# benjiebob/SMALify

Hardware: AMD Instinct MI355X
Metric: fitter iterations/sec (higher is better)
Workload: dtype f32

## Files before the change

### smalify_amd/csrc/kernels_lbs_backward.inc

```

__global__ void __launch_bounds__(256)
vertex_bwd_kernel(ModelDev m, int M, const float* __restrict__ proj, const float* __restrict__ dface,
                  const float* __restrict__ dJ41 ,
                  const float* __restrict__ dverts_ext ,
                  const float* __restrict__ Am, float* __restrict__ dvert ,
                  float* __restrict__ dvp , float* __restrict__ dtr_part ) {
  __shared__ float As[420];
  __shared__ float dJs[123];
  __shared__ float red[16];
  const int Vp = m.Vp;
  PHASE_MARK(pv0);
  int n, vblock;
  xcd_block(Vp / 256, n, vblock);
  if (n >= M) return;
  const int v = vblock * 256 + threadIdx.x;
  constexpr int kPre = 8;
  const int vc = min(v, m.V - 1);
  const int vf0 = m.vf_off[vc], vf1 = (v < m.V) ? m.vf_off[vc + 1] : vf0;
  int vfi[kPre];
#pragma unroll
  for (int q = 0; q < kPre; ++q) vfi[q] = m.vf_idx[min(vf0 + q, max(vf1 - 1, vf0))];
  for (int i = threadIdx.x; i < 420; i += 256) As[i] = Am[(size_t)n * 420 + i];
  for (int i = threadIdx.x; i < 123; i += 256) dJs[i] = dJ41 ? dJ41[(size_t)n * 123 + i] : 0.f;
  __syncthreads();
  int lm = -1;
#pragma unroll
  for (int i = 0; i < 6; ++i) if (v == m.landmarks[i]) lm = i;
  const bool live = v < m.V;
  float g[3] = {0.f, 0.f, 0.f};
  if (live && dface) {
    float gxn = 0.f, gyn = 0.f;
    const float2* df = reinterpret_cast<const float2*>(dface + (size_t)n * m.F * 6);
    float2 gq[kPre];
#pragma unroll
    for (int q = 0; q < kPre; ++q) gq[q] = df[vfi[q]];
#pragma unroll
    for (int q = 0; q < kPre; ++q)
      if (vf0 + q < vf1) { gxn += gq[q].x; gyn += gq[q].y; }
    for (int i = vf0 + kPre; i < vf1; ++i) {
      const float2 g2 = df[m.vf_idx[i]];
      gxn += g2.x;
      gyn += g2.y;
    }
    const float* pv = proj + (size_t)n * 3 * Vp;
    world_to_ndc_bwd(pv[v], pv[Vp + v], pv[2 * Vp + v], gxn, gyn, g[0], g[1], g[2]);
  }
  if (live && dverts_ext) {
#pragma unroll
    for (int a = 0; a < 3; ++a) g[a] += dverts_ext[((size_t)n * 3 + a) * Vp + v];
  }
  {
    const float s0 = wave_sum(live ? g[0] : 0.f), s1 = wave_sum(live ? g[1] : 0.f), s2 = wave_sum(live ? g[2] : 0.f);
    if ((threadIdx.x & 63) == 0) { float* q = &red[(threadIdx.x >> 6) * 4]; q[0] = s0; q[1] = s1; q[2] = s2; }
    __syncthreads();
    if (threadIdx.x < 3)
      dtr_part[((size_t)vblock * M + n) * 3 + threadIdx.x] =
          ((red[threadIdx.x] + red[4 + threadIdx.x]) + red[8 + threadIdx.x]) + red[12 + threadIdx.x];
  }
  float dv[3] = {g[0], g[1], g[2]};
  if (live) {
#pragma unroll 4
    for (int e = 0; e < m.Kj; ++e) {
      const int j = m.jrv_j[e * Vp + v];
      const float c = m.jrv_val[e * Vp + v];
#pragma unroll
      for (int a = 0; a < 3; ++a) dv[a] = fmaf(c, dJs[j * 3 + a], dv[a]);
    }
    if (lm >= 0) {
#pragma unroll
      for (int a = 0; a < 3; ++a) dv[a] += dJs[(35 + lm) * 3 + a];
    }
  }
  float T[9];
#pragma unroll
  for (int e = 0; e < 9; ++e) T[e] = 0.f;
  if (live) {
#pragma unroll 4
    for (int e = 0; e < m.Kw; ++e) {
      const int j = m.w_j[e * Vp + v];
      const float wv = m.w_val[e * Vp + v];
      const float* A = &As[j * 12];
#pragma unroll
      for (int a = 0; a < 3; ++a)
#pragma unroll
        for (int b = 0; b < 3; ++b) T[a * 3 + b] = fmaf(wv, A[a * 4 + b], T[a * 3 + b]);
    }
  }
#pragma unroll
  for (int b = 0; b < 3; ++b) {
    const float o = T[b] * dv[0] + T[3 + b] * dv[1] + T[6 + b] * dv[2];
    if (v < Vp) {
      dvp[((size_t)n * 3 + b) * Vp + v] = live ? o : 0.f;
      dvert[((size_t)n * 3 + b) * Vp + v] = live ? dv[b] : 0.f;
    }
  }
  PHASE_MARK(pv1);
  PHASE_END(PH_VERTEX_BWD, pv0, pv1);
}

__device__ __forceinline__ void
dA_block(const ModelDev& m, int j, int n, const float* __restrict__ dvert, const float* __restrict__ vposed,
         float* __restrict__ dA , float (*part)[32]) {
  const int Vp = m.Vp;
  const float* dv = dvert + (size_t)n * 3 * Vp;
  const float* vp = vposed + (size_t)n * 3 * Vp;
  float acc[16];
#pragma unroll
  for (int e = 0; e < 16; ++e) acc[e] = 0.f;
#pragma unroll 2
  for (int i = m.wc_off[j] + threadIdx.x; i < m.wc_off[j + 1]; i += 256) {
    const int v = m.wc_v[i];
    const float wv = m.wc_val[i];
    const float p[4] = {vp[v], vp[Vp + v], vp[2 * Vp + v], 1.0f};
#pragma unroll
    for (int a = 0; a < 3; ++a) {
      const float d = wv * dv[a * Vp + v];
#pragma unroll
      for (int b = 0; b < 4; ++b) acc[a * 4 + b] = fmaf(d, p[b], acc[a * 4 + b]);
    }
  }
  const int lane = threadIdx.x & 63, w = threadIdx.x >> 6;
  const float tot = wave_sums<16>(acc, lane);
  if ((lane & 3) == 0) part[w][lane >> 2] = tot;
  __syncthreads();
  if (threadIdx.x < 12)
    dA[((size_t)n * 35 + j) * 12 + threadIdx.x] = ((part[0][threadIdx.x] + part[1][threadIdx.x]) + part[2][threadIdx.x]) + part[3][threadIdx.x];
}

constexpr int kAsmElem = 4, kAsmLoss = 16;

__device__ __forceinline__ void
dbeta_block(const ModelDev& m, int M, int nb, int shared, int bx, int by, int bz, int gx, int gzn,
            const float* __restrict__ dvp, float* __restrict__ dbeta_part , float (*part)[32]) {
  const int ncol = 3 * m.Vp;
  const int c = bx * 256 + threadIdx.x;
  float g = 0.f;
  if (c < ncol) {
    if (shared) {
      const int per = (M + gzn - 1) / gzn;
      const int n0 = bz * per, n1 = min(M, n0 + per);
      double gd = 0.0;
#pragma unroll 8
      for (int n = n0; n < n1; ++n) gd += (double)dvp[(size_t)n * ncol + c];
      g = (float)gd;
    } else {
      g = dvp[(size_t)by * ncol + c];
    }
  }
  const size_t pidx = (size_t)by * gzn * gx + (size_t)bz * gx + bx;
  const int lane = threadIdx.x & 63, w = threadIdx.x >> 6;
  for (int b0 = 0; b0 < nb; b0 += 32) {
    float val[32];
    const int cc = min(c, ncol - 1);
#pragma unroll
    for (int b = 0; b < 32; ++b) val[b] = m.sd[(size_t)min(b0 + b, nb - 1) * ncol + cc];
#pragma unroll
    for (int b = 0; b < 32; ++b) val[b] = (c < ncol && b0 + b < nb) ? g * val[b] : 0.f;
    const float tot = wave_sums<32>(val, lane);
    __syncthreads();
    if ((lane & 1) == 0) part[w][lane >> 1] = tot;
    __syncthreads();
    if (threadIdx.x < 32 && b0 + threadIdx.x < nb)
      dbeta_part[pidx * nb + b0 + threadIdx.x] = ((part[0][threadIdx.x] + part[1][threadIdx.x]) + part[2][threadIdx.x]) + part[3][threadIdx.x];
  }
}

constexpr int PBM_SPLITS = 24, PBM_U = 2, PBM_TILES = 4;
static_assert(PBM_SPLITS % 8 == 0, "the blocks of a column split are placed on one XCD (ids in chunks of 8 splits)");
__device__ __forceinline__ void
poseblend_bwd_mfma_block(const ModelDev& m, int M, int tchunk, int kpair, int split, const float* __restrict__ dvp,
                         float* __restrict__ dpf_part , float (*red)[8][64]) {
  const int lane = threadIdx.x & 63, w = threadIdx.x >> 6;
  const int ncol = 3 * m.Vp, nsteps = ncol / 16;
  const int per = (nsteps + PBM_SPLITS * 4 - 1) / (PBM_SPLITS * 4);
  const int s_beg = (split * 4 + w) * per, s_end = min(nsteps, s_beg + per);
  const int nft = (M + 15) / 16, t0 = tchunk * PBM_TILES, nt = min(PBM_TILES, nft - t0);
  const int k0 = kpair * 32;
  const int row = lane & 15, cq = (lane >> 4) * 4;
  const float4* pa[PBM_TILES];
#pragma unroll
  for (int t = 0; t < PBM_TILES; ++t)
    pa[t] = reinterpret_cast<const float4*>(dvp + (size_t)min((t0 + t) * 16 + row, M - 1) * ncol + cq);
  const float4* pb0 = reinterpret_cast<const float4*>(m.pd + (size_t)min(k0 + row, 305) * ncol + cq);
  const float4* pb1 = reinterpret_cast<const float4*>(m.pd + (size_t)min(k0 + 16 + row, 305) * ncol + cq);
  f32x4 acc0[PBM_TILES], acc1[PBM_TILES];
#pragma unroll
  for (int t = 0; t < PBM_TILES; ++t) { acc0[t] = f32x4{0.f, 0.f, 0.f, 0.f}; acc1[t] = acc0[t]; }
  for (int st0 = s_beg; st0 < s_end; st0 += PBM_U) {
    float4 B0[PBM_U], B1[PBM_U], A[PBM_TILES][PBM_U];
#pragma unroll
    for (int u = 0; u < PBM_U; ++u) {
      const int st = min(st0 + u, nsteps - 1);
      B0[u] = pb0[st * 4]; B1[u] = pb1[st * 4];
#pragma unroll
      for (int t = 0; t < PBM_TILES; ++t) {
        A[t][u] = make_float4(0.f, 0.f, 0.f, 0.f);
        if (t < nt && st0 + u < s_end) A[t][u] = pa[t][st * 4];
      }
    }
    __builtin_amdgcn_sched_barrier(0);
#pragma unroll
    for (int u = 0; u < PBM_U; ++u) {
#pragma unroll
      for (int t = 0; t < PBM_TILES; ++t) {
        if (t < nt) {
          acc0[t] = __builtin_amdgcn_mfma_f32_16x16x4f32(A[t][u].x, B0[u].x, acc0[t], 0, 0, 0);
          acc1[t] = __builtin_amdgcn_mfma_f32_16x16x4f32(A[t][u].x, B1[u].x, acc1[t], 0, 0, 0);
          acc0[t] = __builtin_amdgcn_mfma_f32_16x16x4f32(A[t][u].y, B0[u].y, acc0[t], 0, 0, 0);
          acc1[t] = __builtin_amdgcn_mfma_f32_16x16x4f32(A[t][u].y, B1[u].y, acc1[t], 0, 0, 0);
          acc0[t] = __builtin_amdgcn_mfma_f32_16x16x4f32(A[t][u].z, B0[u].z, acc0[t], 0, 0, 0);
          acc1[t] = __builtin_amdgcn_mfma_f32_16x16x4f32(A[t][u].z, B1[u].z, acc1[t], 0, 0, 0);
          acc0[t] = __builtin_amdgcn_mfma_f32_16x16x4f32(A[t][u].w, B0[u].w, acc0[t], 0, 0, 0);
          acc1[t] = __builtin_amdgcn_mfma_f32_16x16x4f32(A[t][u].w, B1[u].w, acc1[t], 0, 0, 0);
        }
      }
    }
    __builtin_amdgcn_sched_barrier(0);
  }
#pragma unroll
  for (int t = 0; t < PBM_TILES; ++t) {
    if (t < nt) {
#pragma unroll
      for (int r = 0; r < 4; ++r) { red[w][r][lane] = acc0[t][r]; red[w][4 + r][lane] = acc1[t][r]; }
      __syncthreads();
#pragma unroll
      for (int q = 0; q < 2; ++q) {
        const int reg = w * 2 + q, r = reg & 3, tile = reg >> 2;
        const float tot = ((red[0][reg][lane] + red[1][reg][lane]) + red[2][reg][lane]) + red[3][reg][lane];
        const int n = (t0 + t) * 16 + 4 * (lane >> 4) + r, k = k0 + tile * 16 + (lane & 15);
        if (n < M && k < 306) dpf_part[((size_t)split * M + n) * 308 + k] = tot;
      }
      __syncthreads();
    }
  }
}

__host__ __device__ inline int mid_pb_ids(int M) { return 10 * PBM_SPLITS * (((M + 15) / 16 + PBM_TILES - 1) / PBM_TILES); }
__host__ __device__ inline int mid_da_ids(int M) { return xcd_grid(35, M); }
__host__ __device__ inline int mid_grid(int M, int nPB) { return (nPB ? mid_pb_ids(M) : 0) + mid_da_ids(M); }
__global__ void __launch_bounds__(256, 4)
lbs_bwd_mid_kernel(ModelDev m, int M, int nPB, const float* __restrict__ dvert, const float* __restrict__ vposed,
                   const float* __restrict__ dvp, float* __restrict__ dA, float* __restrict__ dpf_part) {
  __shared__ float part[4][32];
  __shared__ float tile_red[4][8][64];
  int blk = blockIdx.x;
  if (nPB > 0) {
    const int ids = mid_pb_ids(M);
    if (blk < ids) {
      PHASE_MARK(pm0);
      const int tchunk = blk / (10 * PBM_SPLITS), r = blk - tchunk * (10 * PBM_SPLITS);
      const int chunk = r / 80, q = r - chunk * 80;
      poseblend_bwd_mfma_block(m, M, tchunk, q >> 3, chunk * 8 + (q & 7), dvp, dpf_part, tile_red);
      PHASE_MARK(pm1);
      PHASE_END(PH_MID_PB, pm0, pm1);
      return;
    }
    blk -= ids;
  }
  PHASE_MARK(pd0);
  int n, j;
  xcd_block_of(blk, 35, n, j);
  if (n >= M) return;
  dA_block(m, j, n, dvert, vposed, dA, part);
  PHASE_MARK(pd1); PHASE_END(PH_MID_DA, pd0, pd1);
}

__global__ void __launch_bounds__(256)
chain_bwd_kernel(ModelDev m, int M, const float* __restrict__ theta, const float* __restrict__ Rm,
                 const float* __restrict__ Gm, const float* __restrict__ scm,
                 const float* __restrict__ Jrest, int j_stride, const float* __restrict__ dA,
                 const float* __restrict__ dpf_part, int CS, const float* __restrict__ dth_direct,
                 float* __restrict__ dtheta , float* __restrict__ dls ,
                 float* __restrict__ dJrest , float* __restrict__ dbetaJ ,
                 float* __restrict__ dRs_out ,
                 int nb, int betas_shared, int nDB_x, int nDB_y, int nDB_z, const float* __restrict__ dvp,
                 float* __restrict__ dbeta_part ) {
  PHASE_MARK(pc0);
  if ((int)blockIdx.x >= M) {
    __shared__ float rpart[4][32];
    const int blk = (int)blockIdx.x - M;
    dbeta_block(m, M, nb, betas_shared, blk % nDB_x, (blk / nDB_x) % nDB_y, blk / (nDB_x * nDB_y), nDB_x, nDB_z, dvp, dbeta_part, rpart);
    PHASE_MARK(pcr);
    PHASE_END(PH_CHAIN_RIDER, pc0, pcr);
    return;
  }
  __shared__ float R[35][9], G[35][12], sc[35][3], J[35][3];
  __shared__ float dG[35][12], dR[35][9], dJ[35][3];
  __shared__ float cG[35][12], cJ[35][3], cS[35][3], sOwn[35][3];
  __shared__ float dRp[35][9], djv[35][3];
  __shared__ int sidx[105];
  __shared__ float psum[4][320];
  __shared__ float isc[35][3];
  __shared__ float sJS[105 * 48];
  __shared__ float dAs[35][12];
  __shared__ unsigned char t_lvl_off[36], t_lvl_joint[36], t_child_off[36], t_child_idx[36], t_par[36];
  __shared__ uint2 t_sch[kTreeMaxPass][8];
  const int n = blockIdx.x, l = threadIdx.x;
  const TreeLevels& tl = m.tree;
  if (l < 36) {
    t_lvl_off[l] = tl.lvl_off[l]; t_child_off[l] = tl.child_off[l];
    if (l < 35) { t_lvl_joint[l] = tl.lvl_joint[l]; t_child_idx[l] = tl.child_idx[l]; t_par[l] = (unsigned char)max(m.parents[l], 0); }
  }
  if (l >= 128 && l < 128 + kTreeMaxPass * 8) {
    const int q = l - 128;
    const unsigned char* ch = tl.pass_child[q >> 3][q & 7];
    t_sch[q >> 3][q & 7] = make_uint2((unsigned)tl.pass_joint[q >> 3][q & 7] | ((unsigned)tl.pass_parent[q >> 3][q & 7] << 8) | ((unsigned)tl.pass_nchild[q >> 3][q & 7] << 16),
                                      (unsigned)ch[0] | ((unsigned)ch[1] << 8) | ((unsigned)ch[2] << 16) | ((unsigned)ch[3] << 24));
  }
  const int lth = min(l, 34);
  const float th_pre[3] = {theta[((size_t)n * 35 + lth) * 3], theta[((size_t)n * 35 + lth) * 3 + 1], theta[((size_t)n * 35 + lth) * 3 + 2]};
  float dthd_pre[3] = {0.f, 0.f, 0.f};
  if (dth_direct) {
#pragma unroll
    for (int a = 0; a < 3; ++a) dthd_pre[a] = dth_direct[(size_t)n * 105 + lth * 3 + a];
  }
  const int nlev = tl.nlev;
  const bool js_lds = dbetaJ && m.NBall <= 48;
  const int njs = js_lds ? 105 * m.NBall : 1;
  float js_tmp[20];
  const float* js_src = js_lds ? m.JS : Rm + (size_t)n * 315;
#pragma unroll
  for (int r = 0; r < 20; ++r) js_tmp[r] = js_src[min(l + 256 * r, njs - 1)];
  {
    const int l2 = l + 256;
    const float r0v = Rm[(size_t)n * 315 + l], r1v = Rm[(size_t)n * 315 + min(l2, 314)];
    const float g0v = Gm[(size_t)n * 420 + l], g1v = Gm[(size_t)n * 420 + min(l2, 419)];
    const float a0v = dA[(size_t)n * 420 + l], a1v = dA[(size_t)n * 420 + min(l2, 419)];
    const int lc = min(l, 104);
    const float sv = scm[(size_t)n * 105 + lc], jv = Jrest[(size_t)n * j_stride + lc];
    const int siv = m.scale_idx[lc];
    constexpr int kMaxPer = (PBM_SPLITS + 3) / 4;
    const int per = (CS + 3) / 4, qd = l >> 6, c0 = qd * per, c1 = min(CS, c0 + per);
    const size_t stride = (size_t)M * 308;
    float pv[5][kMaxPer];
    const bool fast = dpf_part != nullptr && per <= kMaxPer;
    if (fast) {
#pragma unroll
      for (int r = 0; r < 5; ++r) {
        const float* src = dpf_part + (size_t)n * 308 + min((l & 63) + 64 * r, 305);
#pragma unroll
        for (int c = 0; c < kMaxPer; ++c) pv[r][c] = src[(size_t)min(c0 + c, CS - 1) * stride];
      }
    }
    if (js_lds) {
#pragma unroll
      for (int r = 0; r < 20; ++r) { const int i = l + 256 * r; if (i < njs) sJS[i] = js_tmp[r]; }
    }
    R[l / 9][l % 9] = r0v;
    if (l2 < 315) R[l2 / 9][l2 % 9] = r1v;
    G[l / 12][l % 12] = g0v; dAs[l / 12][l % 12] = a0v;
    if (l2 < 420) { G[l2 / 12][l2 % 12] = g1v; dAs[l2 / 12][l2 % 12] = a1v; }
    if (l < 105) {
      sc[l / 3][l % 3] = sv; isc[l / 3][l % 3] = 1.0f / sv;
      J[l / 3][l % 3] = jv;
      sOwn[l / 3][l % 3] = 0.f; cS[l / 3][l % 3] = 0.f; cJ[l / 3][l % 3] = 0.f;
      sidx[l] = siv;
    }
    if (dpf_part) {
#pragma unroll
      for (int r = 0; r < 5; ++r) {
        const int el = (l & 63) + 64 * r;
        if (el < 306) {
          float sacc = 0.f;
          if (fast) {
            if (c0 < c1) sacc = pv[r][0];
#pragma unroll
            for (int c = 1; c < kMaxPer; ++c)
              if (c0 + c < c1) sacc += pv[r][c];
          } else {
            const float* src = dpf_part + (size_t)n * 308 + el;
            for (int c = c0; c < c1; ++c) sacc += src[c * stride];
          }
          psum[qd][el] = sacc;
        }
      }
    }
  }
  __syncthreads();
  PHASE_MARK(pc1);
  for (int i = l; i < 315; i += 256)
    dR[i / 9][i % 9] = (i >= 9 && dpf_part) ? ((psum[0][i - 9] + psum[1][i - 9]) + psum[2][i - 9]) + psum[3][i - 9] : 0.f;
  for (int i = l; i < 420; i += 256) {
    const int j = i / 12, e = i % 12, a = e >> 2, b = e & 3;
    const float* da = dAs[j];
    dG[j][e] = (b < 3) ? da[e] - da[a * 4 + 3] * J[j][b] : da[e];
  }
  for (int i = l; i < 105; i += 256) {
    const int j = i / 3, c = i % 3;
    const float* da = dAs[j];
    dJ[j][c] = -(G[j][0 * 4 + c] * da[3] + G[j][1 * 4 + c] * da[7] + G[j][2 * 4 + c] * da[11]);
  }
  __syncthreads();
  PHASE_MARK(pc2);
  const int slot = l / 12, e = l % 12;
  if (l < 64 && tl.fast) {
    const int npass = tl.npass;
    const int slot_c = min(slot, 7);
    uint2 sch_n = t_sch[max(npass - 1, 0)][slot_c];
#pragma unroll 1
    for (int k = npass - 1; k >= 0; --k) {
      const uint2 sch = sch_n;
      sch_n = t_sch[max(k - 1, 0)][slot_c];
      const bool live = (sch.x & 255u) != 255u;
      const int i = live ? (int)(sch.x & 255u) : 0, p = live ? (int)((sch.x >> 8) & 255u) : 0, nch = live ? (int)(sch.x >> 16) : 0;
      const unsigned chil_k = sch.y;
      if (live) {
        float acc = dG[i][e];
        float cv[kTreeMaxChildren];
#pragma unroll
        for (int q = 0; q < kTreeMaxChildren; ++q) cv[q] = cG[(chil_k >> (8 * q)) & 255u][e];
#pragma unroll
        for (int q = 0; q < kTreeMaxChildren; ++q) acc += (q < nch) ? cv[q] : 0.f;
        dG[i][e] = acc;
      }
      __builtin_amdgcn_fence(__ATOMIC_ACQ_REL, "wavefront");
      __builtin_amdgcn_wave_barrier();
      if (live) {
        if (e < 9) {
          const int a = e / 3, b = e % 3;
          dRp[i][e] = G[p][0 * 4 + a] * dG[i][0 * 4 + b] + G[p][1 * 4 + a] * dG[i][1 * 4 + b] + G[p][2 * 4 + a] * dG[i][2 * 4 + b];
        } else {
          const int a = e - 9;
          djv[i][a] = G[p][0 * 4 + a] * dG[i][3] + G[p][1 * 4 + a] * dG[i][7] + G[p][2 * 4 + a] * dG[i][11];
        }
      }
      __builtin_amdgcn_fence(__ATOMIC_ACQ_REL, "wavefront");
      __builtin_amdgcn_wave_barrier();
      if (live) {
        if (e < 9) {
          const int a = e / 3, c = e % 3;
          float acc = dG[i][a * 4 + 3] * (J[i][c] - J[p][c]);
#pragma unroll
          for (int b = 0; b < 3; ++b) acc = fmaf(dG[i][a * 4 + b], R[i][c * 3 + b] * sc[i][b] * isc[p][c], acc);
          cG[i][a * 4 + c] = acc;
          dR[i][a * 3 + c] += dRp[i][a * 3 + c] * sc[i][c] * isc[p][a];
        } else {
          const int a = e - 9;
          cG[i][a * 4 + 3] = dG[i][a * 4 + 3];
          cJ[i][a] = djv[i][a];
          {
            const int b = a;
            float acc = 0.f;
#pragma unroll
            for (int r = 0; r < 3; ++r) acc = fmaf(dRp[i][r * 3 + b], R[i][r * 3 + b] * isc[p][r], acc);
            sOwn[i][b] = acc;
          }
          {
            float acc = 0.f;
#pragma unroll
            for (int b = 0; b < 3; ++b) acc = fmaf(dRp[i][a * 3 + b], R[i][a * 3 + b] * sc[i][b] * isc[p][a], acc);
            cS[i][a] = acc * isc[p][a];
          }
        }
      }
      __builtin_amdgcn_fence(__ATOMIC_ACQ_REL, "wavefront");
      __builtin_amdgcn_wave_barrier();
    }
  } else if (l < 64)
  for (int L = nlev - 1; L >= 1; --L) {
    const int j0 = t_lvl_off[L], nj = t_lvl_off[L + 1] - j0;
    for (int base = 0; base < nj; base += 5) {
      const bool live = (slot < 5) && (base + slot < nj);
      const int i = live ? t_lvl_joint[j0 + base + slot] : 0;
      const int p = live ? t_par[i] : 0;
      if (live) {
        float acc = dG[i][e];
        for (int q = t_child_off[i]; q < t_child_off[i + 1]; ++q) acc += cG[t_child_idx[q]][e];
        dG[i][e] = acc;
      }
      __builtin_amdgcn_fence(__ATOMIC_ACQ_REL, "workgroup");
      __builtin_amdgcn_wave_barrier();
      if (live) {
        if (e < 9) {
          const int a = e / 3, b = e % 3;
          dRp[i][e] = G[p][0 * 4 + a] * dG[i][0 * 4 + b] + G[p][1 * 4 + a] * dG[i][1 * 4 + b] + G[p][2 * 4 + a] * dG[i][2 * 4 + b];
        } else {
          const int a = e - 9;
          djv[i][a] = G[p][0 * 4 + a] * dG[i][3] + G[p][1 * 4 + a] * dG[i][7] + G[p][2 * 4 + a] * dG[i][11];
        }
      }
      __builtin_amdgcn_fence(__ATOMIC_ACQ_REL, "workgroup");
      __builtin_amdgcn_wave_barrier();
      if (live) {
        if (e < 9) {
          const int a = e / 3, c = e % 3;
          float acc = dG[i][a * 4 + 3] * (J[i][c] - J[p][c]);
#pragma unroll
          for (int b = 0; b < 3; ++b) acc = fmaf(dG[i][a * 4 + b], R[i][c * 3 + b] * sc[i][b] * isc[p][c], acc);
          cG[i][a * 4 + c] = acc;
          dR[i][a * 3 + c] += dRp[i][a * 3 + c] * sc[i][c] * isc[p][a];
        } else {
          const int a = e - 9;
          cG[i][a * 4 + 3] = dG[i][a * 4 + 3];
          cJ[i][a] = djv[i][a];
          {
            const int b = a;
            float acc = 0.f;
#pragma unroll
            for (int r = 0; r < 3; ++r) acc = fmaf(dRp[i][r * 3 + b], R[i][r * 3 + b] * isc[p][r], acc);
            sOwn[i][b] = acc;
          }
          {
            float acc = 0.f;
#pragma unroll
            for (int b = 0; b < 3; ++b) acc = fmaf(dRp[i][a * 3 + b], R[i][a * 3 + b] * sc[i][b] * isc[p][a], acc);
            cS[i][a] = acc * isc[p][a];
          }
        }
      }
      __builtin_amdgcn_fence(__ATOMIC_ACQ_REL, "workgroup");
      __builtin_amdgcn_wave_barrier();
    }
  }
  __syncthreads();
  PHASE_MARK(pc3);
  if (l < 12) {
    float acc = dG[0][l];
    for (int q = t_child_off[0]; q < t_child_off[1]; ++q) acc += cG[t_child_idx[q]][l];
    dG[0][l] = acc;
  }
  __syncthreads();
  if (l < 9) dR[0][l] += dG[0][(l / 3) * 4 + (l % 3)];
  for (int i = l; i < 105; i += 256) {
    const int j = i / 3, a = i % 3;
    float aj = dJ[j][a], as = 0.f;
    for (int q = t_child_off[j]; q < t_child_off[j + 1]; ++q) { aj -= cJ[t_child_idx[q]][a]; as -= cS[t_child_idx[q]][a]; }
    if (j > 0) { aj += cJ[j][a]; as += sOwn[j][a]; }
    else aj += dG[0][a * 4 + 3];
    dJ[j][a] = aj;
    sOwn[j][a] = as;
  }
  __syncthreads();
  PHASE_MARK(pc4);
  if (l < 35) {
    const float th[3] = {th_pre[0], th_pre[1], th_pre[2]};
    float g[9], d[3];
#pragma unroll
    for (int q = 0; q < 9; ++q) g[q] = dR[l][q];
    if (dRs_out) {
#pragma unroll
      for (int q = 0; q < 9; ++q) dRs_out[((size_t)n * 35 + l) * 9 + q] = g[q];
    }
    rodrigues_bwd(th, g, d);
#pragma unroll
    for (int a = 0; a < 3; ++a)
      dtheta[(size_t)n * 105 + l * 3 + a] = d[a] + (dth_direct ? dthd_pre[a] : 0.f);
  }
  if (dls) {
    const int w = l >> 6, lane = l & 63;
    for (int sidx_l = w; sidx_l < 6; sidx_l += 4) {
      float v = 0.f;
      if (sidx[lane] == sidx_l) v = sOwn[lane / 3][lane % 3] * sc[lane / 3][lane % 3];
      if (lane + 64 < 105 && sidx[lane + 64] == sidx_l) v += sOwn[(lane + 64) / 3][(lane + 64) % 3] * sc[(lane + 64) / 3][(lane + 64) % 3];
      v = wave_sum(v);
      if (lane == 0) dls[(size_t)n * 6 + sidx_l] = v;
    }
  }
  for (int i = l; i < 105; i += 256) dJrest[(size_t)n * 105 + i] = dJ[i / 3][i % 3];
  if (dbetaJ) {
    const int w = l >> 6, b = l & 63;
    if (b < m.NBall) {
      float acc = 0.f;
      if (js_lds) {
#pragma unroll 9
        for (int r = 0; r < 27; ++r) { const int i = w * 27 + r; if (i < 105) acc = fmaf(dJ[i / 3][i % 3], sJS[i * m.NBall + b], acc); }
      } else {
        for (int i = w * 27; i < min(105, w * 27 + 27); ++i) acc = fmaf(dJ[i / 3][i % 3], m.JS[i * m.NBall + b], acc);
      }
      psum[w][b] = acc;
    }
    __syncthreads();
    if (l < m.NBall) dbetaJ[(size_t)n * m.NBall + l] = ((psum[0][l] + psum[1][l]) + psum[2][l]) + psum[3][l];
  }
  PHASE_MARK(pc5);
  PHASE_ADD(PH_CHAIN, 0, pc0, pc1); PHASE_ADD(PH_CHAIN, 1, pc1, pc2); PHASE_ADD(PH_CHAIN, 2, pc2, pc3); PHASE_ADD(PH_CHAIN, 3, pc3, pc4); PHASE_ADD(PH_CHAIN, 4, pc4, pc5);
  PHASE_END(PH_CHAIN, pc0, pc5);
}

__global__ void __launch_bounds__(256)
assemble_kernel(AssembleArgs a) {
  __shared__ float red[16];
  __shared__ double bsum[12][32];
  __shared__ float part[32][8];
  __shared__ double dpart[32][8];
  __shared__ int is_last;
  const int t = threadIdx.x;
  PHASE_MARK(pa0);
  const int M = a.M;
  const int nbs = a.betas_shared ? 1 : M;
  int role = blockIdx.x;
  const int ph_role = (role < nbs) ? PH_ASM_BETA : PH_ASM_ELEM;
  if (role < nbs) {
    if (a.g_betas) {
      const int s = role;
      const int bl = t % 20, slice = t / 20;
      auto beta_pass = [&](int b0) {
        const int b = b0 + bl;
        if (slice < 12 && b < a.nb) {
          double acc = 0.0;
          const int nlo = a.betas_shared ? 0 : s, nhi = a.betas_shared ? M : s + 1;
          for (int n = nlo + slice; n < nhi; n += 12) acc += (double)a.dbetaJ[(size_t)n * a.NBall + b];
          const int nparts = a.nblk_beta * a.ngrp_beta;
#pragma unroll 8
          for (int blk = slice; blk < nparts; blk += 12) acc += (double)a.dbeta_part[((size_t)s * nparts + blk) * a.nb + b];
          bsum[slice][bl] = acc;
        }
        __syncthreads();
        if (t < 20 && b0 + t < a.nb) {
          double tot = 0.0;
          for (int sl = 0; sl < 12; ++sl) tot += bsum[sl][t];
          if (a.gb_prior && s == 0) tot += (double)a.gb_prior[b0 + t];
          a.g_betas[s * a.nb + b0 + t] = (float)tot;
        }
      };
      beta_pass(0);
      for (int b0 = 20; b0 < a.nb; b0 += 20) {
        __syncthreads();
        beta_pass(b0);
      }
    }
  } else if ((role -= nbs) == 0) {
    if (a.g_ls) {
      if (a.ls_shared) {
        const int e = t & 7, sl = t >> 3;
        double acc = 0.0;
        if (e < 6) for (int n = sl; n < M; n += 32) acc += (double)a.dls[(size_t)n * 6 + e];
        dpart[sl][e] = acc;
        __syncthreads();
        if (t < 6) {
          double tot = 0.0;
          for (int i = 0; i < 32; ++i) tot += dpart[i][t];
          if (a.gls_prior) tot += (double)a.gls_prior[t];
          a.g_ls[t] = (float)tot;
        }
      } else {
        for (int i = t; i < M * 6; i += 256) a.g_ls[i] = a.dls[i];
      }
    }
  } else if ((role -= 1) < kAsmElem) {
    const int gt = role * 256 + t, gs = kAsmElem * 256;
    for (int i = gt; i < M * 3; i += gs) {
      const int n = i / 3, e = i % 3;
      if (a.g_grot) a.g_grot[i] = a.dtheta[(size_t)n * 105 + e] * a.gmask[e];
      if (a.g_trans) {
        double acc = a.dtr_direct ? (double)a.dtr_direct[i] : 0.0;
#pragma unroll 16
        for (int vt = 0; vt < a.nvt; ++vt) acc += (double)a.dtr_part[((size_t)vt * M + n) * 3 + e];
        a.g_trans[i] = (float)acc;
      }
    }
    if (a.g_jrot) {
      const int total = M * 102;
      for (int i0 = gt; i0 < total; i0 += 8 * gs) {
        float v[8];
#pragma unroll
        for (int u = 0; u < 8; ++u) {
          const int i = min(i0 + u * gs, total - 1), n = i / 102, e = i % 102;
          v[u] = a.dtheta[(size_t)n * 105 + 3 + e] * a.rmask[e];
        }
#pragma unroll
        for (int u = 0; u < 8; ++u)
          if (i0 + u * gs < total) a.g_jrot[i0 + u * gs] = v[u];
      }
    }
  } else if (a.losses) {
    role -= kAsmElem;
    float lsil = 0.f;
    if (a.tile_loss) {
      for (int k = role * 256 + t; k < M * a.T; k += kAsmLoss * 256) {
        const int n = k / a.T;
        const int Bn = frame_window_size(n, a.win);
        lsil += a.tile_loss[k] * (a.w_sil / ((float)Bn * (float)a.S * (float)a.S));
      }
    }
    long long qs = 0;
    if (a.qloss) for (int k = role * 256 + t; k < a.nqblk; k += kAsmLoss * 256) qs += a.qloss[k];
    qs = wave_sum_i64(qs);
    __shared__ long long qred[4];
    if ((t & 63) == 0) qred[t >> 6] = qs;
    lsil = block_sum(lsil, red);
    if (t == 0) { a.lpart[role] = lsil; a.qpart[role] = (qred[0] + qred[1]) + (qred[2] + qred[3]); }
  }
  PHASE_MARK(pa1);
  PHASE_END(ph_role, pa0, pa1);
  (void)ph_role;
  if (!a.losses) return;
  __threadfence();
  __syncthreads();
  if (t == 0) is_last = (atomicAdd(a.counter, 1) == (int)gridDim.x - 1);
  __syncthreads();
  if (!is_last) return;
  __threadfence();
  static_assert(kAsmLoss == 16, "butterfly below");
  float lsil = 0.f;
  if (t < 64) {
    const volatile float* lp = a.lpart;
    lsil = (t < kAsmLoss) ? lp[t] : 0.f;
#pragma unroll
    for (int o = 8; o > 0; o >>= 1) lsil += __shfl_xor(lsil, o, 64);
    const volatile long long* qp = a.qpart;
    long long qtot = (t < kAsmLoss) ? qp[t] : 0ll;
    qtot = wave_sum_i64(qtot);
    lsil += (float)((double)qtot * (1.0 / (double)kLossFix));
  }
  {
    const int k = t & 7, sl = t >> 3;
    float acc = 0.f;
    if (a.loss_part) for (int n = sl; n < M; n += 32) acc += a.loss_part[n * 8 + k];
    part[sl][k] = acc;
  }
  __syncthreads();
  if (t < 8) {
    float acc = 0.f;
    if (t == 3) acc = a.loss_betas ? *a.loss_betas : 0.f;
    else if (t == 4) acc = lsil;
    else for (int i = 0; i < 32; ++i) acc += part[i][t];
    a.losses[t] = acc;
  }
  if (t == 8) {
    float acc = 0.f;
    for (int i = 0; i < 32; ++i) acc += part[i][3];
    a.losses[8] = acc;
  }
  if (t == 0) *a.counter = 0;
  PHASE_MARK(pa2);
  PHASE_END(PH_ASM_LAST, pa1, pa2);
}

__global__ void offset_grad_kernel(ModelDev m, int M, const float* __restrict__ dvp ,
                                   const float* __restrict__ dJrest , float* __restrict__ doff ) {
  const int v = blockIdx.x * blockDim.x + threadIdx.x, n = blockIdx.y;
  if (v >= m.V) return;
  float g[3];
#pragma unroll
  for (int c = 0; c < 3; ++c) g[c] = dvp[((size_t)n * 3 + c) * m.Vp + v];
  for (int k = 0; k < m.Kj; ++k) {
    const float w = m.jrv_val[(size_t)k * m.Vp + v];
    const int j = m.jrv_j[(size_t)k * m.Vp + v];
#pragma unroll
    for (int c = 0; c < 3; ++c) g[c] = fmaf(w, dJrest[(size_t)n * 105 + j * 3 + c], g[c]);
  }
  float* o = doff + ((size_t)n * m.V + v) * 3;
  o[0] = g[0]; o[1] = g[1]; o[2] = g[2];
}

struct AdamSegments {
  int nseg;
  int beg[4];
  int off[5];
};
__device__ __forceinline__ void adam_segments_element(const AdamSegments& sg, int j, float* p, const float* g, float* mm,
                                                      float* vv, float step_size, float b1, float b2, float eps,
                                                      float bc2_sqrt, bool fresh) {
  int sgi = 0;
#pragma unroll
  for (int k = 1; k < 4; ++k) sgi += (k < sg.nseg && j >= sg.off[k]) ? 1 : 0;
  const int i = sg.beg[sgi] + (j - sg.off[sgi]);
  const float gi = g[i];
  adam_update(gi, fresh ? 0.f : mm[i], fresh ? 0.f : vv[i], b1, b2, eps, step_size, bc2_sqrt, mm[i], vv[i], p[i]);
}
__global__ void adam_segments_kernel(AdamSegments sg, float* __restrict__ p, const float* __restrict__ g,
                                     float* __restrict__ mm, float* __restrict__ vv,
                                     float step_size, float b1, float b2, float eps, float bc2_sqrt, int fresh) {
  PHASE_MARK(pz0);
  const int j = blockIdx.x * blockDim.x + threadIdx.x;
  if (j >= sg.off[sg.nseg]) return;
  adam_segments_element(sg, j, p, g, mm, vv, step_size, b1, b2, eps, bc2_sqrt, fresh != 0);
  PHASE_MARK(pz1);
  PHASE_END(PH_ADAM, pz0, pz1);
}

__global__ void tick_kernel(int* counter) { *counter += 1; }
__global__ void set_counter_kernel(int* counter, int value) { *counter = value; }
__global__ void adam_segments_graph_kernel(AdamSegments sg, float* __restrict__ p, const float* __restrict__ g,
                                           float* __restrict__ mm, float* __restrict__ vv, const int* __restrict__ step_counter,
                                           float lr, float b1, float b2, float eps) {
  const int j = blockIdx.x * blockDim.x + threadIdx.x;
  if (j >= sg.off[sg.nseg]) return;
  const int t = *step_counter;
  float step_size, bc2_sqrt;
  adam_bias_terms(lr, b1, b2, t, step_size, bc2_sqrt);
  adam_segments_element(sg, j, p, g, mm, vv, step_size, b1, b2, eps, bc2_sqrt, t == 1);
}

__global__ void shard_record_kernel(int ns, const float* __restrict__ shared_grad, int M, const float* __restrict__ grot,
                                    const float* __restrict__ jrot, const float* __restrict__ trans,
                                    const float* __restrict__ gmask, const float* __restrict__ rmask, float* __restrict__ out) {
  const int t = blockIdx.x * blockDim.x + threadIdx.x;
  if (t < ns) { out[t] = shared_grad[t]; return; }
  const int u = t - ns;
  if (u >= 216) return;
  const int which = u / 108, c = u - which * 108;
  const int n = which ? M - 1 : 0;
  float v;
  if (c < 3) v = grot[n * 3 + c] * gmask[c];
  else if (c < 105) v = jrot[n * 102 + (c - 3)] * rmask[c - 3];
  else v = trans[n * 3 + (c - 105)];
  out[t] = v;
}

__global__ void shard_reduce_adam_kernel(int world, int stride, const float* __restrict__ gathered, int ns, int ns_train,
                                         float* __restrict__ p, float* __restrict__ g, float* __restrict__ mm, float* __restrict__ vv,
                                         float step_size, float b1, float b2, float eps, float bc2_sqrt, int fresh) {
  const int i = blockIdx.x * blockDim.x + threadIdx.x;
  if (i >= ns) return;
  float gi = 0.f;
  for (int r = 0; r < world; ++r) gi += gathered[(size_t)r * stride + i];
  g[i] = gi;
  if (i >= ns_train) return;
  adam_update(gi, fresh ? 0.f : mm[i], fresh ? 0.f : vv[i], b1, b2, eps, step_size, bc2_sqrt, mm[i], vv[i], p[i]);
}

__global__ void __launch_bounds__(128)
temporal_kernel(int M, float w_temp, const float* __restrict__ theta, const float* __restrict__ trans,
                float* __restrict__ losses , float* __restrict__ dtheta ,
                float* __restrict__ dtrans ) {
  __shared__ float red[16];
  const int t = threadIdx.x;
  float lj = 0.f, lg = 0.f, lt = 0.f;
  for (int idx = t; idx < M * 108; idx += 128) {
    const int n = idx / 108, e = idx % 108;
    const bool is_tr = e >= 105;
    const int k = is_tr ? e - 105 : e;
    const float D = is_tr ? 3.0f : (k < 3 ? 3.0f : 102.0f);
    const float cur = is_tr ? trans[n * 3 + k] : theta[n * 105 + k];
    float g = 0.f;
    if (n + 1 < M) {
      const float d = cur - (is_tr ? trans[(n + 1) * 3 + k] : theta[(n + 1) * 105 + k]);
      const float term = d * d * (w_temp / D);
      if (is_tr) lt += term; else if (k < 3) lg += term; else lj += term;
      g += d;
    }
    if (n > 0) g += cur - (is_tr ? trans[(n - 1) * 3 + k] : theta[(n - 1) * 105 + k]);
    g *= 2.0f * w_temp / D;
    if (is_tr) dtrans[n * 3 + k] = g; else dtheta[n * 105 + k] = g;
  }
  lj = block_sum(lj, red); lg = block_sum(lg, red); lt = block_sum(lt, red);
  if (t == 0) { losses[0] = lj; losses[1] = lg; losses[2] = lt; }
}

__global__ void split_theta_grad_kernel(int M, const float* __restrict__ dtheta, const float* __restrict__ gmask,
                                        const float* __restrict__ rmask, float* __restrict__ g_grot,
                                        float* __restrict__ g_jrot) {
  const int i = blockIdx.x * blockDim.x + threadIdx.x;
  if (i >= M * 105) return;
  const int n = i / 105, e = i % 105;
  if (e < 3) { if (g_grot) g_grot[n * 3 + e] = dtheta[i] * (gmask ? gmask[e] : 1.f); }
  else if (g_jrot) g_jrot[n * 102 + e - 3] = dtheta[i] * (rmask ? rmask[e - 3] : 1.f);
}

__global__ void project_points_kernel(int count, int S, const float* __restrict__ pts, float* __restrict__ out) {
  const int i = blockIdx.x * blockDim.x + threadIdx.x;
  if (i >= count) return;
  float xn, yn, zv;
  world_to_ndc(pts[i * 3], pts[i * 3 + 1], pts[i * 3 + 2], xn, yn, zv);
  const float half = 0.5f * (float)(S - 1);
  out[i * 2] = half * (1.0f - yn);
  out[i * 2 + 1] = half * (1.0f - xn);
}
__global__ void project_points_bwd_kernel(int count, int S, const float* __restrict__ pts,
                                          const float* __restrict__ dout, float* __restrict__ dpts) {
  const int i = blockIdx.x * blockDim.x + threadIdx.x;
  if (i >= count) return;
  float xn, yn, zv;
  world_to_ndc(pts[i * 3], pts[i * 3 + 1], pts[i * 3 + 2], xn, yn, zv);
  const float half = 0.5f * (float)(S - 1);
  world_to_ndc_bwd(xn, yn, zv, -half * dout[i * 2 + 1], -half * dout[i * 2], dpts[i * 3], dpts[i * 3 + 1], dpts[i * 3 + 2]);
}

__global__ void rodrigues_kernel(int count, const float* __restrict__ th, float* __restrict__ R) {
  const int i = blockIdx.x * blockDim.x + threadIdx.x;
  if (i >= count) return;
  float r[9];
  const float t[3] = {th[i * 3], th[i * 3 + 1], th[i * 3 + 2]};
  rodrigues_fwd(t, r);
#pragma unroll
  for (int e = 0; e < 9; ++e) R[i * 9 + e] = r[e];
}
__global__ void rodrigues_bwd_kernel(int count, const float* __restrict__ th, const float* __restrict__ dR,
                                     float* __restrict__ dth) {
  const int i = blockIdx.x * blockDim.x + threadIdx.x;
  if (i >= count) return;
  const float t[3] = {th[i * 3], th[i * 3 + 1], th[i * 3 + 2]};
  float g[9], d[3];
#pragma unroll
  for (int e = 0; e < 9; ++e) g[e] = dR[i * 9 + e];
  rodrigues_bwd(t, g, d);
  dth[i * 3] = d[0]; dth[i * 3 + 1] = d[1]; dth[i * 3 + 2] = d[2];
}

__global__ void __launch_bounds__(128)
pose_prior_kernel(const float* __restrict__ x, const float* __restrict__ prec, const float* __restrict__ mean,
                  const float* __restrict__ mask, float* __restrict__ out ) {
  __shared__ float xs[105];
  const int n = blockIdx.x, t = threadIdx.x;
  if (t < 105) xs[t] = x[n * 105 + t] - mean[t];
  __syncthreads();
  if (t < 105) {
    float acc = 0.f;
    for (int r = 0; r < 105; ++r) acc = fmaf(xs[r], prec[r * 105 + t], acc);
    acc *= mask[t];
    out[n * 105 + t] = acc * acc;
  }
}
__global__ void __launch_bounds__(128)
pose_prior_bwd_kernel(const float* __restrict__ x, const float* __restrict__ prec, const float* __restrict__ mean,
                      const float* __restrict__ mask, const float* __restrict__ dout, float* __restrict__ dx) {
  __shared__ float xs[105], g[105];
  const int n = blockIdx.x, t = threadIdx.x;
  if (t < 105) xs[t] = x[n * 105 + t] - mean[t];
  __syncthreads();
  if (t < 105) {
    float acc = 0.f;
    for (int r = 0; r < 105; ++r) acc = fmaf(xs[r], prec[r * 105 + t], acc);
    g[t] = 2.0f * acc * mask[t] * mask[t] * dout[n * 105 + t];
  }
  __syncthreads();
  if (t < 105) {
    float acc = 0.f;
    for (int c = 0; c < 105; ++c) acc = fmaf(g[c], prec[t * 105 + c], acc);
    dx[n * 105 + t] = acc;
  }
}
```

### smalify_amd/csrc/kernels_lbs_forward.inc

```


struct HeadArgs {
  int M, Mp, nb, betas_stride, ls_stride, nshape_x, nshape, prior_D, prior_use_ls;
  const float* betas;
  const float* theta_in;
  const float* grot;
  const float* jrot;
  const float* gmask;
  const float* rmask;
  const float* logscale;
  float* theta;
  float* Jrest;
  float* v_shaped;
  float *Rm, *Gm, *scm, *Am, *pfT;
  const float* prior_prec;
  const float* prior_mean;
  float prior_w;
  float *prior_loss, *prior_gb, *prior_gls;
  const float* Rs_in;
  const float* joff;
  int joff_stride;
  const float* voff;
};

__device__ __forceinline__ void
pose_block(const ModelDev& m, const HeadArgs& a, int n) {
  __shared__ float th[105];
  __shared__ float R[35][9];
  __shared__ float sc[35][3], isc[35][3];
  __shared__ __attribute__((aligned(16))) float G[35][12];
  __shared__ float J[35][3];
  __shared__ unsigned char t_lvl_off[36], t_lvl_joint[36], t_par[36];
  __shared__ unsigned char t_pj[kTreeMaxPass][8], t_pp[kTreeMaxPass][8];
  const int l = threadIdx.x, M = a.M;
  PHASE_MARK(ph0);
  const TreeLevels& tl = m.tree;
  if (l < 36) {
    t_lvl_off[l] = tl.lvl_off[l];
    if (l < 35) { t_lvl_joint[l] = tl.lvl_joint[l]; t_par[l] = (unsigned char)max(m.parents[l], 0); }
  }
  if (l >= 128 && l < 128 + kTreeMaxPass * 8) { const int q = l - 128; t_pj[q >> 3][q & 7] = tl.pass_joint[q >> 3][q & 7]; t_pp[q >> 3][q & 7] = tl.pass_parent[q >> 3][q & 7]; }
  const int nlev = tl.nlev;
  if (l < 105) {
    const int lj = max(l - 3, 0);
    const float* tsrc = a.theta_in ? a.theta_in + (size_t)n * 105 + l : ((l < 3) ? a.grot + n * 3 + l : a.jrot + (size_t)n * 102 + lj);
    const float* msrc = a.theta_in ? tsrc : ((l < 3) ? a.gmask + l : a.rmask + lj);
    const int idx = m.scale_idx[l];
    const float tv0 = *tsrc, mv = *msrc;
    float acc = m.Jt[l];
    const float lsv = a.logscale ? a.logscale[(size_t)n * a.ls_stride + max(idx, 0)] : 0.f;
    const float tv = a.theta_in ? tv0 : tv0 * mv;
    th[l] = tv;
    a.theta[(size_t)n * 105 + l] = tv;
    const float* beta = a.betas + (size_t)(a.betas_stride ? n : 0) * a.betas_stride;
#pragma unroll 10
    for (int b = 0; b < a.nb; ++b) acc = fmaf(m.JS[l * m.NBall + b], beta[b], acc);
    if (a.joff) acc += a.joff[(size_t)n * a.joff_stride + l];
    J[l / 3][l % 3] = acc;
    if (a.betas_stride || n == 0) a.Jrest[(size_t)(a.betas_stride ? n : 0) * 105 + l] = acc;
    const float sv = (a.logscale != nullptr && idx >= 0) ? expf(lsv) : 1.0f;
    sc[l / 3][l % 3] = sv; isc[l / 3][l % 3] = 1.0f / sv;
    a.scm[(size_t)n * 105 + l] = sv;
  }
  __syncthreads();
  PHASE_MARK(ph1);
  if (l < 35) {
    const float t3[3] = {th[l * 3], th[l * 3 + 1], th[l * 3 + 2]};
    float r[9];
    if (a.Rs_in) {
#pragma unroll
      for (int e = 0; e < 9; ++e) r[e] = a.Rs_in[((size_t)n * 35 + l) * 9 + e];
    } else {
      rodrigues_fwd(t3, r);
    }
#pragma unroll
    for (int e = 0; e < 9; ++e) { R[l][e] = r[e]; a.Rm[((size_t)n * 35 + l) * 9 + e] = r[e]; }
  }
  __syncthreads();
  PHASE_MARK(ph2);
  for (int idx = l; idx < 306; idx += 256) {
    const int j = idx / 9 + 1, e = idx % 9;
    a.pfT[(size_t)idx * a.Mp + n] = R[j][e] - ((e & 3) == 0 ? 1.0f : 0.0f);
  }
  if (l < 12) {
    const int r = l >> 2, c = l & 3;
    G[0][l] = (c < 3) ? R[0][r * 3 + c] : J[0][r];
  }
  if (l < 64 && tl.fast) {
    const int slot_c = min(l / 12, 7), e = l % 12, r = e >> 2, c = e & 3, cc = min(c, 2);
    const int npass = tl.npass;
    auto fetch = [&](int k, int& ijp, float (&kc)[3]) {
      const int i = t_pj[k][slot_c], p = t_pp[k][slot_c];
      const bool live = i != 255;
      ijp = live ? (i | (p << 8)) : -1;
      const int ii = live ? i : 0;
#pragma unroll
      for (int q = 0; q < 3; ++q) {
        const float rot = R[ii][q * 3 + cc] * sc[ii][cc] * isc[p][q], dj = J[ii][q] - J[p][q];
        kc[q] = (c < 3) ? rot : dj;
      }
    };
    int ijp_n;
    float kc_n[3];
    fetch(0, ijp_n, kc_n);
#pragma unroll 1
    for (int k = 0; k < npass; ++k) {
      const int ijp = ijp_n;
      const float k0 = kc_n[0], k1 = kc_n[1], k2 = kc_n[2];
      fetch(min(k + 1, kTreeMaxPass - 1), ijp_n, kc_n);
      __builtin_amdgcn_fence(__ATOMIC_ACQ_REL, "wavefront");
      __builtin_amdgcn_wave_barrier();
      if (ijp >= 0) {
        const int i = ijp & 255, p = ijp >> 8;
        const float4 g = *reinterpret_cast<const float4*>(&G[p][r * 4]);
        float acc = (c < 3) ? 0.f : g.w;
        acc = fmaf(g.x, k0, acc);
        acc = fmaf(g.y, k1, acc);
        acc = fmaf(g.z, k2, acc);
        G[i][e] = acc;
      }
    }
  } else if (l < 64) {
    const int slot = l / 12, e = l % 12;
    for (int L = 1; L < nlev; ++L) {
      const int j0 = t_lvl_off[L], nj = t_lvl_off[L + 1] - j0;
      for (int base = 0; base < nj; base += 5) {
        __builtin_amdgcn_fence(__ATOMIC_ACQ_REL, "workgroup");
        __builtin_amdgcn_wave_barrier();
        if (slot < 5 && base + slot < nj) {
          const int i = t_lvl_joint[j0 + base + slot], p = t_par[i];
          const int r = e >> 2, c = e & 3;
          float acc;
          if (c < 3) {
            acc = 0.f;
#pragma unroll
            for (int q = 0; q < 3; ++q) acc = fmaf(G[p][r * 4 + q], R[i][q * 3 + c] * sc[i][c] * isc[p][q], acc);
          } else {
            acc = G[p][r * 4 + 3];
#pragma unroll
            for (int q = 0; q < 3; ++q) acc = fmaf(G[p][r * 4 + q], J[i][q] - J[p][q], acc);
          }
          G[i][e] = acc;
        }
      }
    }
  }
  __syncthreads();
  PHASE_MARK(ph3);
  for (int idx = l; idx < 35 * 12; idx += 256) {
    const int j = idx / 12, e = idx % 12, r = e >> 2, c = e & 3;
    float val = G[j][e];
    if (c == 3) {
#pragma unroll
      for (int q = 0; q < 3; ++q) val = fmaf(-G[j][r * 4 + q], J[j][q], val);
    }
    a.Am[(size_t)n * 420 + idx] = val;
    a.Gm[(size_t)n * 420 + idx] = G[j][e];
  }
  (void)M;
  PHASE_MARK(ph4);
  PHASE_ADD(PH_HEAD_POSE, 0, ph0, ph1); PHASE_ADD(PH_HEAD_POSE, 1, ph1, ph2); PHASE_ADD(PH_HEAD_POSE, 2, ph2, ph3); PHASE_ADD(PH_HEAD_POSE, 3, ph3, ph4);
  PHASE_END(PH_HEAD_POSE, ph0, ph4);
}

__global__ void __launch_bounds__(256)
lbs_head_kernel(ModelDev m, HeadArgs a) {
  int blk = blockIdx.x;
  if (blk < a.M) { pose_block(m, a, blk); return; }
  blk -= a.M;
  if (blk < a.nshape) {
    PHASE_MARK(ps0);
    const int s = blk / a.nshape_x;
    const float* beta = a.betas + (size_t)s * a.betas_stride;
    const int v = (blk % a.nshape_x) * 256 + threadIdx.x;
    const int Vp = m.Vp;
    if (v < Vp) {
#pragma unroll
      for (int c = 0; c < 3; ++c) {
        float acc = m.vt[c * Vp + v];
#pragma unroll 10
        for (int b = 0; b < a.nb; ++b) acc = fmaf(beta[b], m.sd[((size_t)b * 3 + c) * Vp + v], acc);
        if (a.voff) acc += a.voff[((size_t)s * 3 + c) * Vp + v];
        a.v_shaped[((size_t)s * 3 + c) * Vp + v] = acc;
      }
    }
    PHASE_MARK(ps1);
    PHASE_END(PH_HEAD_SHAPE, ps0, ps1);
    return;
  }
  if (a.prior_prec && threadIdx.x < 64) {
    __shared__ float x[32], res[32];
    const int t = threadIdx.x, D = a.prior_D;
    if (t < D) x[t] = ((t < 20) ? a.betas[t] : a.logscale[t - 20]) - a.prior_mean[t];
    __builtin_amdgcn_fence(__ATOMIC_ACQ_REL, "workgroup");
    __builtin_amdgcn_wave_barrier();
    float lv = 0.f;
    if (t < D) {
      float acc = 0.f;
      for (int r = 0; r < D; ++r) acc = fmaf(x[r], a.prior_prec[r * D + t], acc);
      res[t] = acc;
      lv = acc * acc;
    }
    __builtin_amdgcn_fence(__ATOMIC_ACQ_REL, "workgroup");
    __builtin_amdgcn_wave_barrier();
    lv = wave_sum(lv);
    if (t == 0) *a.prior_loss = a.prior_w * lv / (float)D;
    if (t < D) {
      float acc = 0.f;
      for (int c = 0; c < D; ++c) acc = fmaf(res[c], a.prior_prec[t * D + c], acc);
      acc *= 2.0f * a.prior_w / (float)D;
      if (t < 20) a.prior_gb[t] = acc; else if (a.prior_use_ls) a.prior_gls[t - 20] = acc;
    }
  }
}

__global__ void build_theta_kernel(int M, const float* __restrict__ grot, const float* __restrict__ jrot,
                                   const float* __restrict__ gmask, const float* __restrict__ rmask,
                                   float* __restrict__ theta) {
  const int i = blockIdx.x * blockDim.x + threadIdx.x;
  if (i >= M * 105) return;
  const int n = i / 105, e = i % 105;
  theta[i] = (e < 3) ? grot[n * 3 + e] * gmask[e] : jrot[n * 102 + (e - 3)] * rmask[e - 3];
}

typedef float f32x4 __attribute__((ext_vector_type(4)));
constexpr int kSkinGroups = 2;
constexpr int kSkinVerts = 16 * kSkinGroups;
constexpr int kSkinThreads = 256 * kSkinGroups;
constexpr int kSkinStage = (16 * 105 + kSkinThreads - 1) / kSkinThreads;
__global__ void __launch_bounds__(kSkinThreads)
skin_mfma_split_kernel(ModelDev m, int M, int Mp, const float* __restrict__ v_shaped, int vs_stride ,
                 const float* __restrict__ pfT, const float* __restrict__ Am, const float* __restrict__ trans,
                 float* __restrict__ vposed, float* __restrict__ verts, float* __restrict__ proj) {
  __shared__ __attribute__((aligned(16))) float As[16][420];
  __shared__ float red[4 * kSkinGroups][12][64];
  const int Vp = m.Vp;
  PHASE_MARK(pk0);
  const int lane = threadIdx.x & 63, wid = threadIdx.x >> 6, w = wid & 3, grp = wid >> 2;
  const int n0 = blockIdx.y * 16;
  const int v = blockIdx.x * kSkinVerts + grp * 16 + (lane & 15);
  const int kq = lane >> 4;
  const int nvalid = min(16, M - n0) * 105;
  float4 a_stage[kSkinStage];
  {
    const float4* src = reinterpret_cast<const float4*>(Am + (size_t)n0 * 420);
#pragma unroll
    for (int r = 0; r < kSkinStage; ++r) a_stage[r] = src[min((int)threadIdx.x + kSkinThreads * r, nvalid - 1)];
  }
  int wj[8];
  float wv[8];
  const int Kw = min(m.Kw, 8);
#pragma unroll
  for (int e = 0; e < 8; ++e) {
    const int ee = max(min(e, Kw - 1), 0);
    wj[e] = m.w_j[ee * Vp + v];
    wv[e] = m.w_val[ee * Vp + v];
  }
  const int f = 4 * kq + w, n = n0 + f, nn = min(n, M - 1);
  float vs_r[3], tr_r[3];
  {
    const float* vs = v_shaped + (size_t)nn * vs_stride;
#pragma unroll
    for (int a = 0; a < 3; ++a) { vs_r[a] = vs[a * Vp + v]; tr_r[a] = trans[nn * 3 + a]; }
  }
  constexpr int U = 20;
  const int st0 = w * U;
  const float* pa = pfT + (size_t)kq * Mp + n0 + (lane & 15);
  const float* pb = m.pd + (size_t)kq * 3 * Vp + v;
  float xa[U], x0[U], x1[U], x2[U];
#pragma unroll
  for (int u = 0; u < U; ++u) {
    const int st = min(st0 + u, 76);
    xa[u] = pa[(size_t)st * 4 * Mp];
    const float* b = pb + (size_t)(min(st * 4 + kq, 305) - kq) * 3 * Vp;
    x0[u] = b[0]; x1[u] = b[Vp]; x2[u] = b[2 * Vp];
  }
  {
    float4* dst = reinterpret_cast<float4*>(&As[0][0]);
#pragma unroll
    for (int r = 0; r < kSkinStage; ++r) {
      const int i4 = threadIdx.x + kSkinThreads * r;
      if (i4 < 16 * 105) dst[i4] = (i4 < nvalid) ? a_stage[r] : make_float4(0.f, 0.f, 0.f, 0.f);
    }
  }
  PHASE_MARK(pk1);
  f32x4 acc0 = {0.f, 0.f, 0.f, 0.f}, acc1 = acc0, acc2 = acc0;
#pragma unroll
  for (int u = 0; u < U; ++u) {
    if (st0 + u < 77) {
      acc0 = __builtin_amdgcn_mfma_f32_16x16x4f32(xa[u], x0[u], acc0, 0, 0, 0);
      acc1 = __builtin_amdgcn_mfma_f32_16x16x4f32(xa[u], x1[u], acc1, 0, 0, 0);
      acc2 = __builtin_amdgcn_mfma_f32_16x16x4f32(xa[u], x2[u], acc2, 0, 0, 0);
    }
  }
#pragma unroll
  for (int r = 0; r < 4; ++r) { red[wid][r][lane] = acc0[r]; red[wid][4 + r][lane] = acc1[r]; red[wid][8 + r][lane] = acc2[r]; }
  __syncthreads();
  PHASE_MARK(pk2);
  if (n < M) {
    float bl[3];
#pragma unroll
    for (int a = 0; a < 3; ++a) bl[a] = ((red[grp * 4][a * 4 + w][lane] + red[grp * 4 + 1][a * 4 + w][lane]) + red[grp * 4 + 2][a * 4 + w][lane]) + red[grp * 4 + 3][a * 4 + w][lane];
    const float vp[3] = {vs_r[0] + bl[0], vs_r[1] + bl[1], vs_r[2] + bl[2]};
#pragma unroll
    for (int a = 0; a < 3; ++a) vposed[((size_t)n * 3 + a) * Vp + v] = vp[a];
    float T[12];
#pragma unroll
    for (int e = 0; e < 12; ++e) T[e] = 0.f;
#pragma unroll
    for (int e = 0; e < 8; ++e) {
      if (e < Kw) {
        const float* A = &As[f][wj[e] * 12];
#pragma unroll
        for (int c = 0; c < 12; ++c) T[c] = fmaf(wv[e], A[c], T[c]);
      }
    }
    for (int e = 8; e < m.Kw; ++e) {
      const int j = m.w_j[e * Vp + v];
      const float wx = m.w_val[e * Vp + v];
      const float* A = &As[f][j * 12];
#pragma unroll
      for (int c = 0; c < 12; ++c) T[c] = fmaf(wx, A[c], T[c]);
    }
    float o[3];
#pragma unroll
    for (int a = 0; a < 3; ++a) {
      o[a] = fmaf(T[a * 4], vp[0], fmaf(T[a * 4 + 1], vp[1], fmaf(T[a * 4 + 2], vp[2], T[a * 4 + 3])));
      verts[((size_t)n * 3 + a) * Vp + v] = o[a];
    }
    float xn, yn, zv;
    world_to_ndc(o[0] + tr_r[0], o[1] + tr_r[1], o[2] + tr_r[2], xn, yn, zv);
    proj[((size_t)n * 3 + 0) * Vp + v] = xn;
    proj[((size_t)n * 3 + 1) * Vp + v] = yn;
    proj[((size_t)n * 3 + 2) * Vp + v] = zv;
  }
  PHASE_MARK(pk3);
  PHASE_ADD(PH_SKIN, 0, pk0, pk1); PHASE_ADD(PH_SKIN, 1, pk1, pk2); PHASE_ADD(PH_SKIN, 2, pk2, pk3);
  PHASE_END(PH_SKIN, pk0, pk3);
}

__global__ void __launch_bounds__(256)
skin_mfma_kernel(ModelDev m, int M, int Mp, const float* __restrict__ v_shaped, int vs_stride ,
                 const float* __restrict__ pfT, const float* __restrict__ Am, const float* __restrict__ trans,
                 float* __restrict__ vposed, float* __restrict__ verts, float* __restrict__ proj) {
  __shared__ __attribute__((aligned(16))) float As[16][420];
  const int Vp = m.Vp;
  PHASE_MARK(pk0);
  const int lane = threadIdx.x & 63, w = threadIdx.x >> 6;
  const int n0 = blockIdx.y * 16;
  const int v = blockIdx.x * 64 + w * 16 + (lane & 15);
  const int kq = lane >> 4;
  const int nvalid = min(16, M - n0) * 105;
  float4 a_stage[7];
  {
    const float4* src = reinterpret_cast<const float4*>(Am + (size_t)n0 * 420);
#pragma unroll
    for (int r = 0; r < 7; ++r) a_stage[r] = src[min((int)threadIdx.x + 256 * r, nvalid - 1)];
  }
  int wj[8];
  float wv[8];
  const int Kw = min(m.Kw, 8);
#pragma unroll
  for (int e = 0; e < 8; ++e) {
    const int ee = max(min(e, Kw - 1), 0);
    wj[e] = m.w_j[ee * Vp + v];
    wv[e] = m.w_val[ee * Vp + v];
  }
  float vs_r[4][3], tr_r[4][3];
#pragma unroll
  for (int r = 0; r < 4; ++r) {
    const int nn = min(n0 + 4 * kq + r, M - 1);
    const float* vs = v_shaped + (size_t)nn * vs_stride;
#pragma unroll
    for (int a = 0; a < 3; ++a) { vs_r[r][a] = vs[a * Vp + v]; tr_r[r][a] = trans[nn * 3 + a]; }
  }
  {
    float4* dst = reinterpret_cast<float4*>(&As[0][0]);
#pragma unroll
    for (int r = 0; r < 7; ++r) {
      const int i4 = threadIdx.x + 256 * r;
      if (i4 < 16 * 105) dst[i4] = (i4 < nvalid) ? a_stage[r] : make_float4(0.f, 0.f, 0.f, 0.f);
    }
  }
  f32x4 acc0 = {0.f, 0.f, 0.f, 0.f}, acc1 = acc0, acc2 = acc0;
  const float* pa = pfT + (size_t)kq * Mp + n0 + (lane & 15);
  const float* pb = m.pd + (size_t)kq * 3 * Vp + v;
  constexpr int U = 11, NBATCH = 7;
  static_assert(U * NBATCH == 77, "306 pose features in steps of 4");
  float xa[U], x0[U], x1[U], x2[U], ya[U], y0[U], y1[U], y2[U];
  auto load_batch = [&](int bt, float* A, float* B0, float* B1, float* B2) {
#pragma unroll
    for (int u = 0; u < U; ++u) {
      const int st = bt * U + u;
      A[u] = pa[(size_t)st * 4 * Mp];
      const float* b = pb + (size_t)(min(st * 4 + kq, 305) - kq) * 3 * Vp;
      B0[u] = b[0]; B1[u] = b[Vp]; B2[u] = b[2 * Vp];
    }
  };
  auto mfma_batch = [&](const float* A, const float* B0, const float* B1, const float* B2) {
#pragma unroll
    for (int u = 0; u < U; ++u) {
      acc0 = __builtin_amdgcn_mfma_f32_16x16x4f32(A[u], B0[u], acc0, 0, 0, 0);
      acc1 = __builtin_amdgcn_mfma_f32_16x16x4f32(A[u], B1[u], acc1, 0, 0, 0);
      acc2 = __builtin_amdgcn_mfma_f32_16x16x4f32(A[u], B2[u], acc2, 0, 0, 0);
    }
  };
  PHASE_MARK(pk1);
  load_batch(0, xa, x0, x1, x2);
  for (int bt = 0; bt < NBATCH - 1; bt += 2) {
    load_batch(bt + 1, ya, y0, y1, y2);
    __builtin_amdgcn_sched_barrier(0);
    mfma_batch(xa, x0, x1, x2);
    __builtin_amdgcn_sched_barrier(0);
    load_batch(bt + 2, xa, x0, x1, x2);
    __builtin_amdgcn_sched_barrier(0);
    mfma_batch(ya, y0, y1, y2);
    __builtin_amdgcn_sched_barrier(0);
  }
  mfma_batch(xa, x0, x1, x2);
  __syncthreads();
  PHASE_MARK(pk2);
#pragma unroll
  for (int r = 0; r < 4; ++r) {
    const int f = 4 * kq + r, n = n0 + f;
    if (n >= M) break;
    const float vp[3] = {vs_r[r][0] + acc0[r], vs_r[r][1] + acc1[r], vs_r[r][2] + acc2[r]};
#pragma unroll
    for (int a = 0; a < 3; ++a) vposed[((size_t)n * 3 + a) * Vp + v] = vp[a];
    float T[12];
#pragma unroll
    for (int e = 0; e < 12; ++e) T[e] = 0.f;
#pragma unroll
    for (int e = 0; e < 8; ++e) {
      if (e < Kw) {
        const float* A = &As[f][wj[e] * 12];
#pragma unroll
        for (int c = 0; c < 12; ++c) T[c] = fmaf(wv[e], A[c], T[c]);
      }
    }
    for (int e = 8; e < m.Kw; ++e) {
      const int j = m.w_j[e * Vp + v];
      const float wx = m.w_val[e * Vp + v];
      const float* A = &As[f][j * 12];
#pragma unroll
      for (int c = 0; c < 12; ++c) T[c] = fmaf(wx, A[c], T[c]);
    }
    float o[3];
#pragma unroll
    for (int a = 0; a < 3; ++a) {
      o[a] = fmaf(T[a * 4], vp[0], fmaf(T[a * 4 + 1], vp[1], fmaf(T[a * 4 + 2], vp[2], T[a * 4 + 3])));
      verts[((size_t)n * 3 + a) * Vp + v] = o[a];
    }
    float xn, yn, zv;
    world_to_ndc(o[0] + tr_r[r][0], o[1] + tr_r[r][1], o[2] + tr_r[r][2], xn, yn, zv);
    proj[((size_t)n * 3 + 0) * Vp + v] = xn;
    proj[((size_t)n * 3 + 1) * Vp + v] = yn;
    proj[((size_t)n * 3 + 2) * Vp + v] = zv;
  }
  PHASE_MARK(pk3);
  PHASE_ADD(PH_SKIN, 0, pk0, pk1); PHASE_ADD(PH_SKIN, 1, pk1, pk2); PHASE_ADD(PH_SKIN, 2, pk2, pk3);
  PHASE_END(PH_SKIN, pk0, pk3);
}

template <int FR>
__global__ void __launch_bounds__(256)
skin_kernel(ModelDev m, int M, int Mp, const float* __restrict__ v_shaped, int vs_stride ,
            const float* __restrict__ pfT, const float* __restrict__ Am, const float* __restrict__ trans,
            float* __restrict__ vposed, float* __restrict__ verts, float* __restrict__ proj) {
  __shared__ float red[4][FR * 3][64];
  __shared__ float As[FR][420];
  const int Vp = m.Vp;
  const int lane = threadIdx.x & 63, w = __builtin_amdgcn_readfirstlane(threadIdx.x >> 6);
  const int v = blockIdx.x * 64 + lane;
  const int n0 = blockIdx.y * FR;
  for (int i = threadIdx.x; i < FR * 420; i += 256) {
    const int f = i / 420;
    As[f][i % 420] = (n0 + f < M) ? Am[(size_t)(n0 + f) * 420 + (i % 420)] : 0.f;
  }
  float acc[FR][3];
#pragma unroll
  for (int f = 0; f < FR; ++f) acc[f][0] = acc[f][1] = acc[f][2] = 0.f;
  const int k0 = (w * 306) / 4, k1 = ((w + 1) * 306) / 4;
  for (int k = k0; k < k1; ++k) {
    const float p0 = m.pd[((size_t)k * 3 + 0) * Vp + v];
    const float p1 = m.pd[((size_t)k * 3 + 1) * Vp + v];
    const float p2 = m.pd[((size_t)k * 3 + 2) * Vp + v];
    const float* pf = pfT + (size_t)k * Mp + n0;
#pragma unroll
    for (int f = 0; f < FR; ++f) {
      const float c = pf[f];
      acc[f][0] = fmaf(c, p0, acc[f][0]);
      acc[f][1] = fmaf(c, p1, acc[f][1]);
      acc[f][2] = fmaf(c, p2, acc[f][2]);
    }
  }
#pragma unroll
  for (int f = 0; f < FR; ++f) {
    red[w][f * 3 + 0][lane] = acc[f][0];
    red[w][f * 3 + 1][lane] = acc[f][1];
    red[w][f * 3 + 2][lane] = acc[f][2];
  }
  __syncthreads();
  for (int f = w; f < FR; f += 4) {
    const int n = n0 + f;
    if (n >= M) break;
    const float* vs = v_shaped + (size_t)n * vs_stride;
    float vp[3];
#pragma unroll
    for (int a = 0; a < 3; ++a) {
      vp[a] = vs[a * Vp + v] + ((red[0][f * 3 + a][lane] + red[1][f * 3 + a][lane]) +
                                (red[2][f * 3 + a][lane] + red[3][f * 3 + a][lane]));
      vposed[((size_t)n * 3 + a) * Vp + v] = vp[a];
    }
    float T[12];
#pragma unroll
    for (int e = 0; e < 12; ++e) T[e] = 0.f;
    for (int e = 0; e < m.Kw; ++e) {
      const int j = m.w_j[e * Vp + v];
      const float wv = m.w_val[e * Vp + v];
      const float* A = &As[f][j * 12];
#pragma unroll
      for (int c = 0; c < 12; ++c) T[c] = fmaf(wv, A[c], T[c]);
    }
    float o[3];
#pragma unroll
    for (int a = 0; a < 3; ++a) {
      o[a] = fmaf(T[a * 4], vp[0], fmaf(T[a * 4 + 1], vp[1], fmaf(T[a * 4 + 2], vp[2], T[a * 4 + 3])));
      verts[((size_t)n * 3 + a) * Vp + v] = o[a];
    }
    float xn, yn, zv;
    world_to_ndc(o[0] + trans[n * 3], o[1] + trans[n * 3 + 1], o[2] + trans[n * 3 + 2], xn, yn, zv);
    proj[((size_t)n * 3 + 0) * Vp + v] = xn;
    proj[((size_t)n * 3 + 1) * Vp + v] = yn;
    proj[((size_t)n * 3 + 2) * Vp + v] = zv;
  }
}

__global__ void project_verts_kernel(int M, int V, int Vp, const float* __restrict__ vin,
                                     float* __restrict__ proj) {
  const int v = blockIdx.x * blockDim.x + threadIdx.x, n = blockIdx.y;
  if (v >= Vp) return;
  float xn = 0.f, yn = 0.f, zv = 1.f;
  if (v < V) {
    const float* p = vin + ((size_t)n * V + v) * 3;
    world_to_ndc(p[0], p[1], p[2], xn, yn, zv);
  }
  proj[((size_t)n * 3 + 0) * Vp + v] = xn;
  proj[((size_t)n * 3 + 1) * Vp + v] = yn;
  proj[((size_t)n * 3 + 2) * Vp + v] = zv;
}

__global__ void planar_to_interleaved_kernel(int M, int V, int Vp, const float* __restrict__ src, int src_stride,
                                             const float* __restrict__ offs, float* __restrict__ dst) {
  const int i = blockIdx.x * blockDim.x + threadIdx.x, n = blockIdx.y;
  if (i >= V * 3) return;
  const int v = i / 3, a = i % 3;
  float val = src[(size_t)n * src_stride + a * Vp + v];
  if (offs) val += offs[n * 3 + a];
  dst[(size_t)n * V * 3 + i] = val;
}

__global__ void interleaved_to_planar_kernel(int M, int V, int Vp, const float* __restrict__ src,
                                             float* __restrict__ dst) {
  const int v = blockIdx.x * blockDim.x + threadIdx.x, n = blockIdx.y;
  if (v >= Vp) return;
#pragma unroll
  for (int a = 0; a < 3; ++a)
    dst[((size_t)n * 3 + a) * Vp + v] = (v < V) ? src[((size_t)n * V + v) * 3 + a] : 0.f;
}

struct Parents35 {
  int p[kJoints];
};

__global__ void global_rigid_kernel(int count, const float* __restrict__ Rs, const float* __restrict__ Js, Parents35 parents,
                                    const float* __restrict__ logscale ,
                                    float* __restrict__ newJ, float* __restrict__ A) {
  const int n = blockIdx.x * blockDim.x + threadIdx.x;
  if (n >= count) return;
  global_rigid_frame(Rs + (size_t)n * 315, Js + (size_t)n * 105, parents.p, logscale ? logscale + (size_t)n * 6 : nullptr,
                     newJ + (size_t)n * 105, A + (size_t)n * 560);
}

__global__ void global_rigid_bwd_kernel(int count, const float* __restrict__ Rs, const float* __restrict__ Js, Parents35 parents,
                                        const float* __restrict__ logscale, const float* __restrict__ dnewJ,
                                        const float* __restrict__ dA, float* __restrict__ scratch, float* __restrict__ dRs,
                                        float* __restrict__ dJs, float* __restrict__ dlogscale) {
  const int n = blockIdx.x * blockDim.x + threadIdx.x;
  if (n >= count) return;
  global_rigid_frame_bwd(Rs + (size_t)n * 315, Js + (size_t)n * 105, parents.p, logscale ? logscale + (size_t)n * 6 : nullptr,
                         dnewJ + (size_t)n * 105, dA + (size_t)n * 560, scratch + (size_t)n * 840, scratch + (size_t)n * 840 + 420,
                         dRs + (size_t)n * 315, dJs + (size_t)n * 105, dlogscale ? dlogscale + (size_t)n * 6 : nullptr);
}

__device__ __forceinline__ void joints_block(const ModelDev& m, const float* __restrict__ verts, float* __restrict__ joints ,
                                             int j, int n, float* red ) {
  const int Vp = m.Vp;
  const float* vx = verts + (size_t)n * 3 * Vp;
  if (j >= 35) {
    if (threadIdx.x < 3) joints[((size_t)n * 41 + j) * 3 + threadIdx.x] = vx[threadIdx.x * Vp + m.landmarks[j - 35]];
    return;
  }
  float a0 = 0.f, a1 = 0.f, a2 = 0.f;
  if (threadIdx.x < 128) {
#pragma unroll 4
    for (int i = m.jr_off[j] + threadIdx.x; i < m.jr_off[j + 1]; i += 128) {
      const int v = m.jr_v[i];
      const float c = m.jr_val[i];
      a0 = fmaf(c, vx[v], a0);
      a1 = fmaf(c, vx[Vp + v], a1);
      a2 = fmaf(c, vx[2 * Vp + v], a2);
    }
  }
  a0 = block_sum(a0, red);
  a1 = block_sum(a1, red);
  a2 = block_sum(a2, red);
  if (threadIdx.x == 0) {
    float* o = joints + ((size_t)n * 41 + j) * 3;
    o[0] = a0; o[1] = a1; o[2] = a2;
  }
}

__global__ void __launch_bounds__(128)
joints_kernel(ModelDev m, const float* __restrict__ verts, float* __restrict__ joints ) {
  __shared__ float red[16];
  joints_block(m, verts, joints, blockIdx.x, blockIdx.y, red);
}

__device__ __forceinline__ void loss_block(const LossArgs& a, int n) {
  __shared__ float th[105], x[105], res[105], dth[105];
  __shared__ float dJ[41 * 3];
  __shared__ float red[16];
  const int t = threadIdx.x;
  const int Bn = frame_window_size(n, a.win);
  for (int i = t; i < 105; i += 128) { th[i] = a.theta[n * 105 + i]; dth[i] = 0.f; }
  for (int i = t; i < 123; i += 128) dJ[i] = 0.f;
  __syncthreads();
  const float tx = a.trans[n * 3], ty = a.trans[n * 3 + 1], tz = a.trans[n * 3 + 2];
  float l_joint = 0.f, l_pose = 0.f, l_splay = 0.f, l_tj = 0.f, l_tg = 0.f, l_tt = 0.f, l_limit = 0.f;
  if (t < 25) {
    const int cj = a.canon[t];
    const float* jp = a.joints + ((size_t)n * 41 + cj) * 3;
    float xn, yn, zv;
    world_to_ndc(jp[0] + tx, jp[1] + ty, jp[2] + tz, xn, yn, zv);
    const float half = 0.5f * (float)(a.S - 1);
    const float row = half * (1.0f - yn), col = half * (1.0f - xn);
    if (a.proj_out) { a.proj_out[(n * 25 + t) * 2] = row; a.proj_out[(n * 25 + t) * 2 + 1] = col; }
    if (a.w_j2d > 0.f && a.vis[n * 25 + t] != 0.f) {
      const float dr = row - a.tj[(n * 25 + t) * 2], dc = col - a.tj[(n * 25 + t) * 2 + 1];
      l_joint = dr * dr + dc * dc;
      const float k = 2.0f * a.w_j2d / (50.0f * (float)Bn);
      float gx, gy, gz;
      world_to_ndc_bwd(xn, yn, zv, -half * k * dc, -half * k * dr, gx, gy, gz);
      atomicAdd(&dJ[cj * 3 + 0], gx);
      atomicAdd(&dJ[cj * 3 + 1], gy);
      atomicAdd(&dJ[cj * 3 + 2], gz);
    }
  }
  if (a.w_pose > 0.f) {
    if (t < 105) x[t] = th[t] - a.pose_mean[t];
    __syncthreads();
    if (t < 105) {
      float acc = 0.f;
#pragma unroll 15
      for (int r = 0; r < 105; ++r) acc = fmaf(x[r], a.pose_prec[r * 105 + t], acc);
      acc *= a.pose_mask[t];
      res[t] = acc * a.pose_mask[t];
      l_pose = acc * acc;
    }
    __syncthreads();
    if (t < 105) {
      float acc = 0.f;
#pragma unroll 15
      for (int c = 0; c < 105; ++c) acc = fmaf(res[c], a.pose_prec[t * 105 + c], acc);
      dth[t] += acc * (2.0f * a.w_pose / (105.0f * (float)Bn));
    }
  }
  if (a.w_limit > 0.f && t >= 3 && t < 105) {
    const float x = th[t], hi = a.lim_max[t - 3], lo = a.lim_min[t - 3];
    l_limit = fmaxf(x - hi, 0.f) + fmaxf(lo - x, 0.f);
    const float slope = (x > hi) ? 1.0f : ((x < lo) ? -1.0f : 0.0f);
    dth[t] += slope * (a.w_limit / (102.0f * (float)Bn));
  }
  if (a.w_splay > 0.f && t >= 3 && t < 105 && ((t % 3) != 1)) {
    l_splay = th[t] * th[t];
    dth[t] += 2.0f * a.w_splay * th[t];
  }
  float dtr = 0.f;
  if (a.w_temp > 0.f && t < 108) {
    const bool is_tr = t >= 105;
    const int e = is_tr ? t - 105 : t;
    const float D = is_tr ? 3.0f : (e < 3 ? 3.0f : 102.0f);
    const float cur = is_tr ? a.trans[n * 3 + e] : th[e];
    float g = 0.f;
    bool has_next = (n + 1 < a.M) || (a.halo_next != nullptr);
    if (has_next) {
      const float nxt = (n + 1 < a.M) ? (is_tr ? a.trans[(n + 1) * 3 + e] : a.theta[(n + 1) * 105 + e])
                                      : a.halo_next[is_tr ? 105 + e : e];
      const float d = cur - nxt;
      const float term = d * d * (a.w_temp / D);
      if (is_tr) l_tt = term; else if (e < 3) l_tg = term; else l_tj = term;
      g += d;
    }
    bool has_prev = (n > 0) || (a.halo_prev != nullptr);
    if (has_prev) {
      const float prv = (n > 0) ? (is_tr ? a.trans[(n - 1) * 3 + e] : a.theta[(n - 1) * 105 + e])
                                : a.halo_prev[is_tr ? 105 + e : e];
      g += cur - prv;
    }
    g *= 2.0f * a.w_temp / D;
    if (is_tr) dtr = g; else dth[e] += g;
  }
  __syncthreads();
  for (int i = t; i < 105; i += 128) a.dth_direct[n * 105 + i] = dth[i];
  for (int i = t; i < 123; i += 128) a.dJ41[n * 123 + i] = dJ[i];
  if (t >= 105 && t < 108) {
    float s = dtr;
    const int e = t - 105;
    for (int j = 0; j < 41; ++j) s += dJ[j * 3 + e];
    a.dtr_direct[n * 3 + e] = s;
  }
  const float nj = 1.0f / (50.0f * (float)Bn), np_ = 1.0f / (105.0f * (float)Bn);
  l_joint = block_sum(l_joint, red);
  l_pose = block_sum(l_pose, red);
  l_splay = block_sum(l_splay, red);
  l_tj = block_sum(l_tj, red);
  l_tg = block_sum(l_tg, red);
  l_tt = block_sum(l_tt, red);
  l_limit = block_sum(l_limit, red);
  if (t == 0) {
    float* o = a.loss_part + n * 8;
    o[0] = a.w_j2d * nj * l_joint;
    o[1] = a.w_pose * np_ * l_pose;
    o[2] = a.w_splay * l_splay;
    o[3] = a.w_limit * l_limit / (102.0f * (float)Bn);
    o[4] = 0.f;
    o[5] = l_tj; o[6] = l_tg; o[7] = l_tt;
  }
}

__global__ void __launch_bounds__(128)
loss_kernel(LossArgs a) { loss_block(a, blockIdx.x); }
```

### smalify_amd/csrc/smalfit_internal.h

```cpp
#pragma once
#include <hip/hip_runtime.h>

#include "smalfit_math.h"

#define SMALFIT_STATUS_BIN_OVERFLOW 1

namespace smalfit {

constexpr int kTreeMaxPass = 16, kTreeMaxChildren = 4;
struct TreeLevels {
  unsigned char nlev;
  unsigned char lvl_off[36];
  unsigned char lvl_joint[35];
  unsigned char child_off[36];
  unsigned char child_idx[35];
  unsigned char fast, npass;
  unsigned char pass_joint[kTreeMaxPass][8];
  unsigned char pass_parent[kTreeMaxPass][8];
  unsigned char pass_nchild[kTreeMaxPass][8];
  unsigned char pass_child[kTreeMaxPass][8][kTreeMaxChildren];
};

struct ModelDev {
  int V, Vp, F, NBall;
  const float* vt;
  const float* sd;
  const float* pd;
  int Kw;
  const int* w_j;
  const float* w_val;
  const int* wc_off;
  const int* wc_v;
  const float* wc_val;
  const int* jr_off;
  const int* jr_v;
  const float* jr_val;
  int Kj;
  const int* jrv_j;
  const float* jrv_val;
  const float* Jt;
  const float* JS;
  const int* parents;
  const int* faces;
  const int* vf_off;
  const int* vf_idx;
  const int* scale_idx;
  int landmarks[6];
  TreeLevels tree;
};

struct WinMap {
  int window;
  int offset;
  int total;
};

struct LossArgs {
  int M, S;
  WinMap win;
  const float* theta;
  const float* trans;
  const float* joints;
  const int* canon;
  const float* tj;
  const float* vis;
  float w_j2d, w_pose, w_splay, w_temp;
  float w_limit;
  const float* lim_min;
  const float* lim_max;
  const float* pose_prec;
  const float* pose_mean;
  const float* pose_mask;
  const float* halo_prev;
  const float* halo_next;
  float* proj_out;
  float* dth_direct;
  float* dJ41;
  float* dtr_direct;
  float* loss_part;
};

struct AssembleArgs {
  int M, S, T, nb, NBall, nblk_beta, nvt;
  WinMap win;
  int betas_shared, ls_shared;
  float w_sil;
  const float* dbeta_part;
  const float* dJrest;
  const float* dbetaJ;
  int ngrp_beta;
  const float* JS;
  const float* gb_prior;
  const float* gls_prior;
  const float* dls;
  const float* dtheta;
  const float* gmask;
  const float* rmask;
  const float* dtr_direct;
  const float* dtr_part;
  const float* loss_part;
  const float* loss_betas;
  const float* tile_loss;
  const long long* qloss;
  int nqblk;
  float* lpart;
  long long* qpart;
  int* counter;
  float* g_betas;
  float* g_ls;
  float* g_grot;
  float* g_jrot;
  float* g_trans;
  float* losses;
};

}
```

### smalify_amd/csrc/smalfit_launch.inc

```
#include <algorithm>
#include <cstdio>
#include <cstring>
#include <string>
#include <vector>

#include "../../include/smalfit.h"

namespace smalfit {

static thread_local std::string g_err;
static constexpr int kBetaGroups = 8;
static constexpr int kSelectBlocks = 1792;
static_assert(kSelectBlocks % (8 * kSelGroups) == 0, "every ticket group of every XCD needs the same number of selection workgroups (a group without one would leave its pixels undone)");
#ifdef SMALFIT_DEV_PROBES
static int g_dbg = 0;
#else
static constexpr int g_dbg = 0;
#endif

static int fail(const std::string& msg) {
  g_err = msg;
  return 1;
}

#define HIP_OK(expr)                                                                         \
  do {                                                                                       \
    hipError_t _e = (expr);                                                                  \
    if (_e != hipSuccess)                                                                    \
      return fail(std::string(#expr) + ": " + hipGetErrorString(_e));                        \
  } while (0)

#define LAUNCH_OK(what)                                                                      \
  do {                                                                                       \
    hipError_t _e = hipGetLastError();                                                       \
    if (_e != hipSuccess) return fail(std::string("launch ") + what + ": " + hipGetErrorString(_e)); \
  } while (0)

static inline size_t align_up(size_t x, size_t a) { return (x + a - 1) / a * a; }

struct Blob {
  std::vector<unsigned char> bytes;
  size_t add(const void* src, size_t n) {
    const size_t off = align_up(bytes.size(), 256);
    bytes.resize(off + n);
    if (src) std::memcpy(bytes.data() + off, src, n);
    return off;
  }
};

static const int kDefaultLandmarks[6] = {1863, 26, 2124, 150, 3055, 1097};
static const int kCanonical[25] = {10, 9, 8, 20, 19, 18, 14, 13, 12, 24, 23, 22, 25,
                                   31, 33, 34, 35, 36, 38, 37, 39, 40, 15, 15, 28};

}

using namespace smalfit;

struct smalfit_model {
  ModelDev dev;
  void* blob = nullptr;
  int V = 0, Vp = 0, F = 0, NBall = 0;
};

struct smalfit_engine {
  smalfit_model* model = nullptr;
  int maxM = 0, Mp = 0, S = 0, Tx = 0, T = 0, cap = 0, CS = PBM_SPLITS, nvt = 0, nblk_beta = 0;
  void* slab = nullptr;
  float *theta, *v_shaped, *Jrest, *Rm, *Gm, *scm, *Am, *pfT, *vposed, *verts, *proj, *joints;
  int2* fbox;
  int* status;
  float4* frec;
  int4* brect;
  unsigned long long* gacc;
  unsigned* bcnt;
  float2* zband;
  float2* blist;
  unsigned char* plist;
  unsigned char* pcount;
  unsigned long long* zbuf = nullptr;
  float* vnorm = nullptr;
  int *qcount, *frect, *queue, *bqueue;
  long long* qloss;
  int nrb = 0;
  float2* gz;
  float* zc;
  float* lpart;
  long long* qpart;
  int* asm_counter;
  float *silbuf, *tile_loss, *dface;
  float *dJ41, *dvert, *dvp, *dext, *dA, *dpf_part, *dbeta_part, *dtheta, *dls, *dJrest;
  float* dbetaJ;
  float *dth_direct, *dtr_direct, *dtr_part, *loss_part, *loss_betas, *gb_prior, *gls_prior;
  float *ones, *zeros;
  int* canon;
  float *pose_prec = nullptr, *pose_mean = nullptr, *pose_mask = nullptr;
  float *lim_min = nullptr, *lim_max = nullptr;
  bool has_joint_limits = false;
  float *shape_prec = nullptr, *shape_mean = nullptr;
  int shape_dim = 0;
  bool has_pose_prior = false;
  bool unclamped_edge_t = false;
  bool use_graph = false;
  hipGraphExec_t graph_exec = nullptr;
  std::vector<unsigned char> graph_key;
  unsigned config_epoch = 0;
  int* step_counter = nullptr;
  bool prof_on = false;
  int prof_iter = 0, prof_cap = 0, prof_stride = 1, prof_tick = 0;
  std::vector<hipEvent_t> prof_ev;
};

namespace smalfit {
struct Section {
  smalfit_engine* e; hipStream_t st; int id; bool on;
  Section(smalfit_engine* e_, hipStream_t st_, int id_) : e(e_), st(st_), id(id_) {
    on = e->prof_on && e->prof_iter < e->prof_cap && (e->prof_tick % e->prof_stride) == 0;
    if (on) (void)hipEventRecord(e->prof_ev[((size_t)e->prof_iter * SMALFIT_NUM_SECTIONS + id) * 2], st);
  }
  ~Section() {
    if (on) (void)hipEventRecord(e->prof_ev[((size_t)e->prof_iter * SMALFIT_NUM_SECTIONS + id) * 2 + 1], st);
  }
};
}

namespace smalfit {
static void launch_raster_bwd(smalfit_engine* e, hipStream_t st, int M) {
  const ModelDev& m = e->model->dev;
  const unsigned grid = (unsigned)xcd_grid((m.F + kBwdFaces - 1) / kBwdFaces, M), block = kBwdLanes * kBwdFaces;
  if (e->unclamped_edge_t)
    raster_bwd_kernel<true><<<grid, block, 0, st>>>(m.F, M, e->S, e->frec, e->fbox, e->zc, e->gz, e->plist, e->pcount, e->dface);
  else
    raster_bwd_kernel<false><<<grid, block, 0, st>>>(m.F, M, e->S, e->frec, e->fbox, e->zc, e->gz, e->plist, e->pcount, e->dface);
}
}

extern "C" {

int smalfit_version(void) { return SMALFIT_ABI_VERSION; }
#ifdef SMALFIT_DEV_PROBES
void smalfit_debug_set(int flags) { g_dbg = flags; }
int smalfit_debug_stats(smalfit_engine* e, int* out8) {
  (void)hipDeviceSynchronize();
  (void)hipMemcpy(out8, e->status, 8 * sizeof(int), hipMemcpyDeviceToHost);
  (void)hipMemset(e->status, 0, 8 * sizeof(int));
  return 0;
}
#endif
#ifdef SMALFIT_WORK_STATS
int smalfit_debug_work_stats(unsigned long long* out32) {
  (void)hipDeviceSynchronize();
  (void)hipMemcpyFromSymbol(out32, HIP_SYMBOL(smalfit::g_work), 32 * sizeof(unsigned long long));
  static const unsigned long long z[32] = {0};
  (void)hipMemcpyToSymbol(HIP_SYMBOL(smalfit::g_work), z, sizeof(z));
  return 0;
}
#endif
#ifdef SMALFIT_PHASES
int smalfit_debug_phase_stats(unsigned long long* out192) {
  (void)hipDeviceSynchronize();
  (void)hipMemcpyFromSymbol(out192, HIP_SYMBOL(smalfit::g_phase), 12 * 16 * sizeof(unsigned long long));
  static const unsigned long long z[12 * 16] = {0};
  (void)hipMemcpyToSymbol(HIP_SYMBOL(smalfit::g_phase), z, sizeof(z));
  return 0;
}
#endif
const char* smalfit_last_error(void) { return g_err.c_str(); }

int smalfit_model_create(const smalfit_model_desc* d, smalfit_model** out) {
  if (!d || !out) return fail("smalfit_model_create: null argument");
  const int V = d->num_verts, F = d->num_faces, NB = d->num_betas;
  if (V <= 0 || F <= 0 || NB <= 0) return fail("smalfit_model_create: bad dimensions");
  for (int i = 1; i < 35; ++i)
    if (!(d->parents[i] >= 0 && d->parents[i] < i)) return fail("smalfit_model_create: parents must satisfy 0 <= parents[i] < i");
  for (int i = 0; i < F * 3; ++i)
    if (d->faces[i] < 0 || d->faces[i] >= V) return fail("smalfit_model_create: face index out of range");
  const int* lms = kDefaultLandmarks;
  for (int i = 0; i < 6; ++i)
    if (lms[i] >= V) return fail("smalfit_model_create: model has fewer vertices than the SMAL landmark ids");
  const int Vp = (int)align_up((size_t)V, 256);
  Blob b;
  std::vector<float> vt((size_t)3 * Vp, 0.f), sd((size_t)NB * 3 * Vp, 0.f), pd((size_t)306 * 3 * Vp, 0.f);
  for (int v = 0; v < V; ++v)
    for (int a = 0; a < 3; ++a) vt[(size_t)a * Vp + v] = d->v_template[v * 3 + a];
  for (int k = 0; k < NB; ++k)
    for (int v = 0; v < V; ++v)
      for (int a = 0; a < 3; ++a) sd[((size_t)k * 3 + a) * Vp + v] = d->shapedirs[(size_t)k * 3 * V + 3 * v + a];
  for (int k = 0; k < 306; ++k)
    for (int v = 0; v < V; ++v)
      for (int a = 0; a < 3; ++a) pd[((size_t)k * 3 + a) * Vp + v] = d->posedirs[(size_t)k * 3 * V + 3 * v + a];
  auto build = [&](const float* dense, int& K, std::vector<int>& ell_j, std::vector<float>& ell_v,
                   std::vector<int>& off, std::vector<int>& cv, std::vector<float>& cval) {
    K = 1;
    for (int v = 0; v < V; ++v) {
      int c = 0;
      for (int j = 0; j < 35; ++j) c += dense[v * 35 + j] != 0.f;
      K = std::max(K, c);
    }
    ell_j.assign((size_t)K * Vp, 0);
    ell_v.assign((size_t)K * Vp, 0.f);
    for (int v = 0; v < V; ++v) {
      int c = 0;
      for (int j = 0; j < 35; ++j)
        if (dense[v * 35 + j] != 0.f) { ell_j[(size_t)c * Vp + v] = j; ell_v[(size_t)c * Vp + v] = dense[v * 35 + j]; ++c; }
    }
    off.assign(36, 0);
    cv.clear(); cval.clear();
    for (int j = 0; j < 35; ++j) {
      for (int v = 0; v < V; ++v)
        if (dense[v * 35 + j] != 0.f) { cv.push_back(v); cval.push_back(dense[v * 35 + j]); }
      off[j + 1] = (int)cv.size();
    }
    if (cv.empty()) { cv.push_back(0); cval.push_back(0.f); }
  };
  int Kw, Kj;
  std::vector<int> w_j, wc_off, wc_v, jrv_j, jr_off, jr_v;
  std::vector<float> w_val, wc_val, jrv_val, jr_val;
  build(d->weights, Kw, w_j, w_val, wc_off, wc_v, wc_val);
  build(d->J_regressor, Kj, jrv_j, jrv_val, jr_off, jr_v, jr_val);
  std::vector<double> Jt64(105, 0.0), JS64((size_t)105 * NB, 0.0);
  for (int j = 0; j < 35; ++j)
    for (int i = jr_off[j]; i < jr_off[j + 1]; ++i) {
      const int v = jr_v[i];
      const double c = jr_val[i];
      for (int a = 0; a < 3; ++a) {
        Jt64[j * 3 + a] += c * d->v_template[v * 3 + a];
        for (int k = 0; k < NB; ++k) JS64[(size_t)(j * 3 + a) * NB + k] += c * d->shapedirs[(size_t)k * 3 * V + 3 * v + a];
      }
    }
  std::vector<float> Jt(105), JS((size_t)105 * NB);
  for (int i = 0; i < 105; ++i) Jt[i] = (float)Jt64[i];
  for (size_t i = 0; i < JS.size(); ++i) JS[i] = (float)JS64[i];
  std::vector<int> faces_int((size_t)F * 3);
  {
    float lo[3] = {1e30f, 1e30f, 1e30f}, hi[3] = {-1e30f, -1e30f, -1e30f};
    std::vector<float> cen((size_t)F * 3);
    for (int f = 0; f < F; ++f)
      for (int a = 0; a < 3; ++a) {
        const float c = (d->v_template[d->faces[f * 3] * 3 + a] + d->v_template[d->faces[f * 3 + 1] * 3 + a] +
                         d->v_template[d->faces[f * 3 + 2] * 3 + a]) / 3.0f;
        cen[(size_t)f * 3 + a] = c;
        lo[a] = std::min(lo[a], c); hi[a] = std::max(hi[a], c);
      }
    std::vector<std::pair<unsigned long long, int>> keyed(F);
    for (int f = 0; f < F; ++f) {
      unsigned long long code = 0;
      for (int a = 0; a < 3; ++a) {
        const float span = hi[a] - lo[a];
        const unsigned q = span > 0.f ? (unsigned)std::min(1023.0f, (cen[(size_t)f * 3 + a] - lo[a]) / span * 1023.0f) : 0u;
        for (int bit = 0; bit < 10; ++bit) code |= (unsigned long long)((q >> bit) & 1u) << (3 * bit + a);
      }
      keyed[f] = {code, f};
    }
    std::stable_sort(keyed.begin(), keyed.end());
    for (int f = 0; f < F; ++f)
      for (int k = 0; k < 3; ++k) faces_int[(size_t)f * 3 + k] = d->faces[keyed[f].second * 3 + k];
  }
  std::vector<int> vf_off(V + 1, 0), vf_idx((size_t)F * 3 + 1, 0);
  for (int i = 0; i < F * 3; ++i) vf_off[faces_int[i] + 1]++;
  for (int v = 0; v < V; ++v) vf_off[v + 1] += vf_off[v];
  {
    std::vector<int> cur(vf_off.begin(), vf_off.end() - 1);
    for (int i = 0; i < F * 3; ++i) vf_idx[cur[faces_int[i]]++] = i;
  }
  std::vector<int> sidx(105, -1);
  auto set = [&](int j, int a, int c) { sidx[j * 3 + a] = c; };
  for (int j = 7; j < 25; ++j) {
    if (j == 15 || j == 16) continue;
    set(j, 2, 0); set(j, 0, 1); set(j, 1, 1);
  }
  for (int j = 25; j < 32; ++j) { set(j, 0, 2); set(j, 1, 3); set(j, 2, 3); }
  for (int j = 33; j < 35; ++j) { set(j, 1, 4); set(j, 2, 5); }

  const size_t o_vt = b.add(vt.data(), vt.size() * 4), o_sd = b.add(sd.data(), sd.size() * 4);
  const size_t o_pd = b.add(pd.data(), pd.size() * 4);
  const size_t o_wj = b.add(w_j.data(), w_j.size() * 4), o_wv = b.add(w_val.data(), w_val.size() * 4);
  const size_t o_wco = b.add(wc_off.data(), 36 * 4), o_wcv = b.add(wc_v.data(), wc_v.size() * 4);
  const size_t o_wcl = b.add(wc_val.data(), wc_val.size() * 4);
  const size_t o_jro = b.add(jr_off.data(), 36 * 4), o_jrv = b.add(jr_v.data(), jr_v.size() * 4);
  const size_t o_jrl = b.add(jr_val.data(), jr_val.size() * 4);
  const size_t o_jvj = b.add(jrv_j.data(), jrv_j.size() * 4), o_jvv = b.add(jrv_val.data(), jrv_val.size() * 4);
  const size_t o_jt = b.add(Jt.data(), 105 * 4), o_js = b.add(JS.data(), JS.size() * 4);
  const size_t o_par = b.add(d->parents, 35 * 4), o_f = b.add(faces_int.data(), (size_t)F * 3 * 4);
  const size_t o_vfo = b.add(vf_off.data(), vf_off.size() * 4), o_vfi = b.add(vf_idx.data(), vf_idx.size() * 4);
  const size_t o_si = b.add(sidx.data(), 105 * 4);

  smalfit_model* m = new smalfit_model();
  if (hipMalloc(&m->blob, b.bytes.size()) != hipSuccess) { delete m; return fail("smalfit_model_create: hipMalloc failed (no HIP device?)"); }
  if (hipMemcpy(m->blob, b.bytes.data(), b.bytes.size(), hipMemcpyHostToDevice) != hipSuccess) {
    (void)hipFree(m->blob); delete m; return fail("smalfit_model_create: hipMemcpy failed");
  }
  unsigned char* base = (unsigned char*)m->blob;
  ModelDev& g = m->dev;
  g.V = V; g.Vp = Vp; g.F = F; g.NBall = NB;
  g.vt = (const float*)(base + o_vt); g.sd = (const float*)(base + o_sd); g.pd = (const float*)(base + o_pd);
  g.Kw = Kw; g.w_j = (const int*)(base + o_wj); g.w_val = (const float*)(base + o_wv);
  g.wc_off = (const int*)(base + o_wco); g.wc_v = (const int*)(base + o_wcv); g.wc_val = (const float*)(base + o_wcl);
  g.jr_off = (const int*)(base + o_jro); g.jr_v = (const int*)(base + o_jrv); g.jr_val = (const float*)(base + o_jrl);
  g.Kj = Kj; g.jrv_j = (const int*)(base + o_jvj); g.jrv_val = (const float*)(base + o_jvv);
  g.Jt = (const float*)(base + o_jt); g.JS = (const float*)(base + o_js);
  g.parents = (const int*)(base + o_par); g.faces = (const int*)(base + o_f);
  g.vf_off = (const int*)(base + o_vfo); g.vf_idx = (const int*)(base + o_vfi);
  g.scale_idx = (const int*)(base + o_si);
  for (int i = 0; i < 6; ++i) g.landmarks[i] = lms[i];
  {
    TreeLevels& tl = g.tree;
    int depth[35] = {0}, maxd = 0;
    for (int i = 1; i < 35; ++i) { depth[i] = depth[d->parents[i]] + 1; maxd = std::max(maxd, depth[i]); }
    tl.nlev = (unsigned char)(maxd + 1);
    int pos = 0;
    for (int L = 0; L <= maxd; ++L) {
      tl.lvl_off[L] = (unsigned char)pos;
      for (int i = 0; i < 35; ++i) if (depth[i] == L) tl.lvl_joint[pos++] = (unsigned char)i;
    }
    for (int L = maxd + 1; L < 36; ++L) tl.lvl_off[L] = (unsigned char)pos;
    pos = 0;
    for (int j = 0; j < 35; ++j) {
      tl.child_off[j] = (unsigned char)pos;
      for (int c = 34; c >= 1; --c) if (d->parents[c] == j) tl.child_idx[pos++] = (unsigned char)c;
    }
    tl.child_off[35] = (unsigned char)pos;
    memset(tl.pass_joint, 255, sizeof(tl.pass_joint));
    memset(tl.pass_parent, 0, sizeof(tl.pass_parent));
    memset(tl.pass_nchild, 0, sizeof(tl.pass_nchild));
    memset(tl.pass_child, 0, sizeof(tl.pass_child));
    int np = 0;
    bool fits = true;
    for (int L = 1; L <= maxd; ++L) {
      const int j0 = tl.lvl_off[L], nj = tl.lvl_off[L + 1] - j0;
      for (int base = 0; base < nj; base += 5, ++np) {
        if (np >= kTreeMaxPass) { fits = false; continue; }
        for (int s = 0; s < 5 && base + s < nj; ++s) {
          const int i = tl.lvl_joint[j0 + base + s];
          tl.pass_joint[np][s] = (unsigned char)i;
          tl.pass_parent[np][s] = (unsigned char)d->parents[i];
          const int nc = tl.child_off[i + 1] - tl.child_off[i];
          if (nc > kTreeMaxChildren) fits = false;
          tl.pass_nchild[np][s] = (unsigned char)std::min(nc, kTreeMaxChildren);
          for (int q = 0; q < std::min(nc, kTreeMaxChildren); ++q) tl.pass_child[np][s][q] = tl.child_idx[tl.child_off[i] + q];
        }
      }
    }
    if (tl.child_off[1] - tl.child_off[0] > 35) fits = false;
    tl.npass = (unsigned char)std::min(np, kTreeMaxPass);
    tl.fast = fits ? 1 : 0;
  }
  m->V = V; m->Vp = Vp; m->F = F; m->NBall = NB;
  *out = m;
  return 0;
}

void smalfit_model_destroy(smalfit_model* m) {
  if (!m) return;
  if (m->blob) (void)hipFree(m->blob);
  delete m;
}

int smalfit_engine_create(smalfit_model* model, int max_frames, int image_size, smalfit_engine** out) {
  if (!model || !out || max_frames <= 0 || image_size <= 0) return fail("smalfit_engine_create: bad argument");
  if (image_size > 1024) return fail("smalfit_engine_create: image_size above 1024 is not supported (float32 pixel walk, see kernels_raster.inc)");
  smalfit_engine* e = new smalfit_engine();
  e->model = model;
  e->maxM = max_frames;
  e->Mp = (int)align_up((size_t)max_frames, 16);
  e->S = image_size;
  e->Tx = (image_size + 15) / 16;
  e->T = e->Tx * e->Tx;
  e->nrb = ((image_size + kResEdge - 1) / kResEdge) * ((image_size + kResEdge - 1) / kResEdge);
  e->nvt = model->Vp / 256;
  e->nblk_beta = (3 * model->Vp + 255) / 256;
  const size_t M = max_frames, Vp = model->Vp, F = model->F, S = image_size, T = e->T;
  size_t off = 0;
  auto carve = [&](size_t bytes) { size_t o = off; off = align_up(off + bytes, 256); return o; };
  struct Item { void** ptr; size_t off; };
  std::vector<Item> items;
#define CARVE(field, count, type) items.push_back({(void**)&e->field, carve((size_t)(count) * sizeof(type))})
  CARVE(theta, M * 105, float);
  CARVE(v_shaped, M * 3 * Vp, float);
  CARVE(Jrest, M * 105, float);
  CARVE(Rm, M * 315, float);
  CARVE(Gm, M * 420, float);
  CARVE(scm, M * 105, float);
  CARVE(Am, M * 420, float);
  CARVE(pfT, (size_t)308 * e->Mp, float);
  CARVE(vposed, M * 3 * Vp, float);
  CARVE(verts, M * 3 * Vp, float);
  CARVE(proj, M * 3 * Vp, float);
  CARVE(joints, M * 123, float);
  CARVE(fbox, M * F, int2);
  CARVE(frec, M * F * kRecVecs, float4);
  CARVE(brect, M * ((F + kRectFaces - 1) / kRectFaces), int4);
  CARVE(plist, M * F * kListCap, unsigned char);
  CARVE(pcount, M * F, unsigned char);
  CARVE(gacc, M * S * S, unsigned long long);
  CARVE(bcnt, M * S * S, unsigned);
  CARVE(zband, M * S * S, float2);
  CARVE(qcount, kQCountInts, int);
  CARVE(frect, M * 4, int);
  CARVE(queue, M * S * S, int);
  CARVE(bqueue, M * S * S, int);
  CARVE(qloss, kSelectBlocks + kBandBlocks, long long);
  CARVE(status, 8, int);
  CARVE(gz, M * S * S, float2);
  CARVE(silbuf, M * S * S, float);
  CARVE(tile_loss, M * (size_t)e->nrb, float);
  CARVE(dface, M * F * 6, float);
  CARVE(dJ41, M * 123, float);
  CARVE(dvert, M * 3 * Vp, float);
  CARVE(dvp, M * 3 * Vp, float);
  CARVE(dext, M * 3 * Vp, float);
  CARVE(dA, M * 420, float);
  CARVE(dpf_part, (size_t)e->CS * M * 308, float);
  CARVE(dbeta_part, (M + kBetaGroups) * (size_t)e->nblk_beta * model->NBall, float);
  CARVE(dtheta, M * 105, float);
  CARVE(dls, M * 6, float);
  CARVE(dJrest, M * 105, float);
  CARVE(dbetaJ, M * (size_t)model->NBall, float);
  CARVE(dth_direct, M * 105, float);
  CARVE(dtr_direct, M * 3, float);
  CARVE(dtr_part, (size_t)e->nvt * M * 3, float);
  CARVE(loss_part, M * 8, float);
  CARVE(loss_betas, 4, float);
  CARVE(lpart, 64, float);
  CARVE(qpart, 64, long long);
  CARVE(zc, M, float);
  CARVE(asm_counter, 4, int);
  CARVE(step_counter, 4, int);
  CARVE(gb_prior, 64, float);
  CARVE(gls_prior, 16, float);
  CARVE(ones, 128, float);
  CARVE(zeros, M * 128, float);
  CARVE(canon, 32, int);
  CARVE(pose_prec, 105 * 105, float);
  CARVE(pose_mean, 105, float);
  CARVE(pose_mask, 105, float);
  CARVE(lim_min, 102, float);
  CARVE(lim_max, 102, float);
  CARVE(shape_prec, 41 * 41, float);
  CARVE(shape_mean, 41, float);
#undef CARVE
  if (hipMalloc(&e->slab, off) != hipSuccess) { delete e; return fail("smalfit_engine_create: hipMalloc of workspace failed"); }
  for (auto& it : items) *it.ptr = (unsigned char*)e->slab + it.off;
  if (hipMemset(e->slab, 0, off) != hipSuccess) { (void)hipFree(e->slab); delete e; return fail("smalfit_engine_create: hipMemset failed"); }
  if (hipMemsetD32((hipDeviceptr_t)e->zband, 0x7f800000, (size_t)M * S * S * 2) != hipSuccess ||
      hipMalloc(&e->blist, (size_t)M * S * S * kBandCap * sizeof(float2)) != hipSuccess) {
    (void)hipFree(e->slab); delete e; return fail("smalfit_engine_create: allocation of the band lists failed");
  }
  std::vector<float> ones(128, 1.0f);
  (void)hipMemcpy(e->ones, ones.data(), 128 * 4, hipMemcpyHostToDevice);
  (void)hipMemcpy(e->canon, kCanonical, 25 * 4, hipMemcpyHostToDevice);
  *out = e;
  return 0;
}

void smalfit_engine_destroy(smalfit_engine* e) {
  if (!e) return;
  for (auto ev : e->prof_ev) (void)hipEventDestroy(ev);
  if (e->graph_exec) (void)hipGraphExecDestroy(e->graph_exec);
  if (e->slab) (void)hipFree(e->slab);
  if (e->blist) (void)hipFree(e->blist);
  if (e->zbuf) (void)hipFree(e->zbuf);
  if (e->vnorm) (void)hipFree(e->vnorm);
  delete e;
}

int smalfit_engine_status(smalfit_engine* e, void* stream, int* bits) {
  if (!e || !bits) return fail("smalfit_engine_status: null argument");
  hipStream_t st = (hipStream_t)stream;
  HIP_OK(hipStreamSynchronize(st));
  HIP_OK(hipMemcpy(bits, e->status, sizeof(int), hipMemcpyDeviceToHost));
  HIP_OK(hipMemset(e->status, 0, sizeof(int)));
  return 0;
}

int smalfit_engine_reset_raster_cache(smalfit_engine* e, void* stream) {
  if (!e) return fail("smalfit_engine_reset_raster_cache: null argument");
  HIP_OK(hipMemsetD32Async((hipDeviceptr_t)e->zband, 0x7f800000, (size_t)e->maxM * e->S * e->S * 2, (hipStream_t)stream));
  return 0;
}

int smalfit_engine_set_pose_prior(smalfit_engine* e, const float* prec, const float* mean, const float* mask) {
  if (!e || !prec || !mean || !mask) return fail("smalfit_engine_set_pose_prior: null argument");
  HIP_OK(hipMemcpy(e->pose_prec, prec, 105 * 105 * 4, hipMemcpyHostToDevice));
  HIP_OK(hipMemcpy(e->pose_mean, mean, 105 * 4, hipMemcpyHostToDevice));
  HIP_OK(hipMemcpy(e->pose_mask, mask, 105 * 4, hipMemcpyHostToDevice));
  e->has_pose_prior = true;
  e->config_epoch++;
  return 0;
}

int smalfit_engine_set_joint_limits(smalfit_engine* e, const float* min_values, const float* max_values) {
  if (!e || !min_values || !max_values) return fail("smalfit_engine_set_joint_limits: null argument");
  for (int i = 0; i < 102; ++i)
    if (!(min_values[i] <= max_values[i])) return fail("smalfit_engine_set_joint_limits: min must not exceed max");
  HIP_OK(hipMemcpy(e->lim_min, min_values, 102 * 4, hipMemcpyHostToDevice));
  HIP_OK(hipMemcpy(e->lim_max, max_values, 102 * 4, hipMemcpyHostToDevice));
  e->has_joint_limits = true;
  e->config_epoch++;
  return 0;
}

int smalfit_engine_clear_joint_limits(smalfit_engine* e) {
  if (!e) return fail("smalfit_engine_clear_joint_limits: null argument");
  e->has_joint_limits = false;
  e->config_epoch++;
  return 0;
}

int smalfit_engine_set_option(smalfit_engine* e, int option, int value) {
  if (!e) return fail("smalfit_engine_set_option: null argument");
  switch (option) {
    case SMALFIT_OPT_UNCLAMPED_EDGE_T:
      if (value != 0 && value != 1) return fail("smalfit_engine_set_option: SMALFIT_OPT_UNCLAMPED_EDGE_T takes 0 or 1");
      e->unclamped_edge_t = value != 0;
      break;
    default:
      return fail("smalfit_engine_set_option: unknown option");
  }
  e->config_epoch++;
  return 0;
}

int smalfit_engine_set_shape_prior(smalfit_engine* e, const float* prec, const float* mean, int dim) {
  if (!e || !prec || !mean || dim <= 0 || dim > 26) return fail("smalfit_engine_set_shape_prior: bad argument (dim must be 1..26)");
  HIP_OK(hipMemcpy(e->shape_prec, prec, (size_t)dim * dim * 4, hipMemcpyHostToDevice));
  HIP_OK(hipMemcpy(e->shape_mean, mean, (size_t)dim * 4, hipMemcpyHostToDevice));
  e->shape_dim = dim;
  e->config_epoch++;
  return 0;
}

}

namespace smalfit {

struct HeadExtras {
  const float *grot = nullptr, *jrot = nullptr, *gmask = nullptr, *rmask = nullptr;
  const float *prior_prec = nullptr, *prior_mean = nullptr;
  int prior_D = 0, prior_use_ls = 0;
  float prior_w = 0.f;
  const float *Rs_in = nullptr, *joff = nullptr, *voff = nullptr;
  int joff_stride = 0;
};

static int run_lbs_forward(smalfit_engine* e, hipStream_t st, int M, const float* betas, int betas_stride,
                           int nb, const float* logscale, int ls_stride, const float* trans,
                           float* joints_out, const HeadExtras* ex = nullptr) {
  const ModelDev& m = e->model->dev;
  const int nbs = betas_stride ? M : 1;
  HeadArgs h;
  std::memset(&h, 0, sizeof(h));
  h.M = M; h.Mp = e->Mp; h.nb = nb; h.betas_stride = betas_stride; h.ls_stride = ls_stride;
  h.nshape_x = m.Vp / 256; h.nshape = h.nshape_x * nbs;
  h.betas = betas; h.logscale = logscale;
  h.theta_in = (ex && ex->grot) ? nullptr : e->theta;
  if (ex) { h.grot = ex->grot; h.jrot = ex->jrot; h.gmask = ex->gmask; h.rmask = ex->rmask;
            h.Rs_in = ex->Rs_in; h.joff = ex->joff; h.joff_stride = ex->joff_stride; h.voff = ex->voff; }
  h.theta = e->theta; h.Jrest = e->Jrest; h.v_shaped = e->v_shaped;
  h.Rm = e->Rm; h.Gm = e->Gm; h.scm = e->scm; h.Am = e->Am; h.pfT = e->pfT;
  const bool prior = ex && ex->prior_prec;
  if (prior) {
    h.prior_prec = ex->prior_prec; h.prior_mean = ex->prior_mean; h.prior_D = ex->prior_D; h.prior_use_ls = ex->prior_use_ls;
    h.prior_w = ex->prior_w; h.prior_loss = e->loss_betas; h.prior_gb = e->gb_prior; h.prior_gls = e->gls_prior;
  }
  lbs_head_kernel<<<M + h.nshape + (prior ? 1 : 0), 256, 0, st>>>(m, h);
  LAUNCH_OK("lbs_head_kernel");
  const int vs_stride = betas_stride ? 3 * m.Vp : 0;
  if (M > 4 && (m.Vp / 64) * ((M + 15) / 16) >= 256)
    skin_mfma_kernel<<<dim3(m.Vp / 64, (M + 15) / 16), 256, 0, st>>>(m, M, e->Mp, e->v_shaped, vs_stride, e->pfT, e->Am, trans,
                                                                    e->vposed, e->verts, e->proj);
  else if (M > 4)
    skin_mfma_split_kernel<<<dim3(m.Vp / kSkinVerts, (M + 15) / 16), kSkinThreads, 0, st>>>(m, M, e->Mp, e->v_shaped, vs_stride, e->pfT, e->Am, trans,
                                                                    e->vposed, e->verts, e->proj);
  else
    skin_kernel<8><<<dim3(m.Vp / 64, (M + 7) / 8), 256, 0, st>>>(m, M, e->Mp, e->v_shaped, vs_stride, e->pfT, e->Am,
                                                                 trans, e->vposed, e->verts, e->proj);
  LAUNCH_OK("skin_kernel");
  if (joints_out) {
    joints_kernel<<<dim3(41, M), 128, 0, st>>>(m, e->verts, joints_out);
    LAUNCH_OK("joints_kernel");
  }
  return 0;
}

static int run_raster_forward(smalfit_engine* e, hipStream_t st, int M, WinMap win, float w_sil,
                              SilTarget tsil, float* sil_out, float2* gz_unused, float* blk_loss,
                              float* joints_out = nullptr, const LossArgs* la = nullptr) {
  (void)gz_unused;
  float2* gz = e->gz;
  const ModelDev& m = e->model->dev;
  {
    Section sec(e, st, SMALFIT_SEC_RASTER_BBOX);
    face_bbox_kernel<<<((M + 7) / 8) * 8 + xcd_grid((m.F + 255) / 256, M) + (joints_out ? 41 * M : 0), 256, 0, st>>>(m, M, e->S, e->proj, e->fbox, e->frec, e->brect, e->zc, e->frect,
                                                                                                 e->qcount, e->verts, joints_out);
    LAUNCH_OK("face_bbox_kernel");
  }
  {
    Section sec(e, st, SMALFIT_SEC_RASTER_SWEEP);
    raster_sweep_kernel<<<xcd_grid((m.F + kSweepFaces - 1) / kSweepFaces, M), 256, 0, st>>>(m.F, M, e->S, e->frec, e->fbox, e->brect, e->zc, e->zband, e->gacc, e->bcnt, e->blist, e->plist, e->pcount);
    LAUNCH_OK("raster_sweep_kernel");
  }
  {
    Section sec(e, st, SMALFIT_SEC_RASTER_RESOLVE);
    LossArgs no_loss;
    std::memset(&no_loss, 0, sizeof(no_loss));
    raster_resolve_kernel<<<xcd_grid(e->nrb, M) + (la ? ((M + 7) / 8) * 8 : 0), 256, 0, st>>>(e->S, M, win, w_sil, e->gacc, e->bcnt, e->frect, e->zband, tsil, sil_out, gz,
                                                                         blk_loss, e->qcount, e->queue, e->bqueue, g_dbg ? e->status : nullptr,
                                                                         la ? *la : no_loss, la ? M : 0);
    LAUNCH_OK("raster_resolve_kernel");
    raster_band_kernel<<<kBandBlocks, 256, 0, st>>>(e->S, M, win, w_sil, e->gacc, e->bcnt, e->blist, tsil, sil_out, gz, e->zband,
                                                    e->qcount, e->queue, e->bqueue, tsil ? e->qloss + kSelectBlocks : nullptr);
    LAUNCH_OK("raster_band_kernel");
  }
  Section sec(e, st, SMALFIT_SEC_RASTER_SELECT);
  raster_select_kernel<<<kSelectBlocks, 64 * kSelWaves, 0, st>>>(m.F, e->S, M, win, w_sil, e->frec, e->zc, e->brect, e->fbox, e->qcount, e->queue,
                                                      tsil, sil_out, gz, e->zband, e->pcount, tsil ? e->qloss : nullptr, g_dbg);
  LAUNCH_OK("raster_select_kernel");
  return 0;
}

static int run_lbs_backward(smalfit_engine* e, hipStream_t st, int M, int nb, int betas_shared,
                            const float* dface, const float* dJ41, const float* dext, bool need_pose,
                            bool need_beta, bool need_ls, const float* dth_direct, int j_stride, float* dRs_out = nullptr) {
  const ModelDev& m = e->model->dev;
  vertex_bwd_kernel<<<xcd_grid(m.Vp / 256, M), 256, 0, st>>>(m, M, e->proj, dface, dJ41, dext, e->Am, e->dvert, e->dvp, e->dtr_part);
  LAUNCH_OK("vertex_bwd_kernel");
  {
    const int nPB = need_pose ? mid_pb_ids(M) : 0;
    const int dbx = need_beta ? e->nblk_beta : 0, dby = betas_shared ? 1 : M, dbz = betas_shared ? kBetaGroups : 1;
    lbs_bwd_mid_kernel<<<mid_grid(M, nPB), 256, 0, st>>>(m, M, nPB, e->dvert, e->vposed, e->dvp, e->dA, e->dpf_part);
    LAUNCH_OK("lbs_bwd_mid_kernel");
    chain_bwd_kernel<<<M + dbx * dby * dbz, 256, 0, st>>>(m, M, e->theta, e->Rm, e->Gm, e->scm, e->Jrest, j_stride, e->dA,
                                                   need_pose ? e->dpf_part : nullptr, e->CS, dth_direct, e->dtheta,
                                                   need_ls ? e->dls : nullptr, e->dJrest, need_beta ? e->dbetaJ : nullptr, dRs_out,
                                                   nb, betas_shared, dbx, dby, dbz, e->dvp, e->dbeta_part);
  }
  LAUNCH_OK("chain_bwd_kernel");
  return 0;
}

}

extern "C" {

int smalfit_fit_eval(smalfit_engine* e, void* stream, const smalfit_fit_args* a) {
  if (!e || !a) return fail("smalfit_fit_eval: null argument");
  if (a->struct_size != (unsigned)sizeof(smalfit_fit_args))
    return fail("smalfit_fit_eval: smalfit_fit_args.struct_size does not match this library (built against another smalfit.h?)");
  const int M = a->num_frames;
  if (M <= 0 || M > e->maxM) return fail("smalfit_fit_eval: num_frames exceeds the engine's max_frames");
  if (a->window <= 0) return fail("smalfit_fit_eval: window must be positive");
  if (a->frame_offset < 0) return fail("smalfit_fit_eval: frame_offset must be >= 0");
  if (a->total_frames != 0 && a->total_frames < a->frame_offset + M) return fail("smalfit_fit_eval: total_frames is smaller than frame_offset + num_frames");
  const WinMap win{a->window, a->frame_offset, a->total_frames > 0 ? a->total_frames : a->frame_offset + M};
  if (!a->betas || !a->global_rotation || !a->joint_rotations || !a->trans || !a->losses)
    return fail("smalfit_fit_eval: missing parameter / losses pointer");
  if (a->w_j2d > 0.f && (!a->target_joints || !a->target_visibility)) return fail("smalfit_fit_eval: keypoint targets missing");
  if (a->w_sil > 0.f && !a->target_sil && !a->target_sil_u8) return fail("smalfit_fit_eval: target_sil missing with w_sil > 0");
  if (a->w_pose > 0.f && !e->has_pose_prior) return fail("smalfit_fit_eval: pose prior not set");
  if (a->w_betas > 0.f && e->shape_dim <= 0) return fail("smalfit_fit_eval: shape prior not set");
  if (a->logscale_mode != 0 && !a->log_beta_scales) return fail("smalfit_fit_eval: log_beta_scales missing");
  hipStream_t st = (hipStream_t)stream;
  const ModelDev& m = e->model->dev;
  const float* gmask = a->global_mask ? a->global_mask : e->ones;
  const float* rmask = a->rotation_mask ? a->rotation_mask : e->ones;
  const float* ls = a->logscale_mode ? a->log_beta_scales : nullptr;
  const int ls_stride = a->logscale_mode == 2 ? 6 : 0;
  const int nb = 20;

  const bool sil_on = a->w_sil > 0.f;
  const bool fused_loss = sil_on || a->sil_out;
  const bool shape_prior = a->w_betas > 0.f;
  const int D = a->shape_prior_dim > 0 ? a->shape_prior_dim : e->shape_dim;
  const bool prior_uses_ls = shape_prior && D > 20;
  if (shape_prior && prior_uses_ls && a->logscale_mode != 1)
    return fail("smalfit_fit_eval: a 26-dim shape prior needs shared log_beta_scales");
  {
    Section sec(e, st, SMALFIT_SEC_LBS_FWD);
    HeadExtras ex;
    ex.grot = a->global_rotation; ex.jrot = a->joint_rotations; ex.gmask = gmask; ex.rmask = rmask;
    if (shape_prior) {
      ex.prior_prec = e->shape_prec; ex.prior_mean = e->shape_mean; ex.prior_D = D; ex.prior_use_ls = prior_uses_ls ? 1 : 0;
      const int w0 = (win.offset + win.window - 1) / win.window, w1 = (win.offset + M + win.window - 1) / win.window;
      ex.prior_w = a->w_betas * (float)(w1 - w0);
    }
    if (run_lbs_forward(e, st, M, a->betas, 0, nb, ls, ls_stride, a->trans, fused_loss ? nullptr : e->joints, &ex)) return 1;
  }

  LossArgs la;
  la.M = M; la.S = e->S; la.win = win;
  la.theta = e->theta; la.trans = a->trans; la.joints = e->joints; la.canon = e->canon;
  la.tj = a->target_joints; la.vis = a->target_visibility;
  la.w_j2d = a->w_j2d; la.w_pose = a->w_pose; la.w_splay = a->w_splay; la.w_temp = a->temporal ? a->w_temp : 0.f;
  la.w_limit = e->has_joint_limits ? a->w_limit : 0.f; la.lim_min = e->lim_min; la.lim_max = e->lim_max;
  la.pose_prec = e->pose_prec; la.pose_mean = e->pose_mean; la.pose_mask = e->pose_mask;
  la.halo_prev = a->temporal ? a->halo_prev : nullptr;
  la.halo_next = a->temporal ? a->halo_next : nullptr;
  la.proj_out = a->proj_out;
  la.dth_direct = e->dth_direct; la.dJ41 = e->dJ41; la.dtr_direct = e->dtr_direct; la.loss_part = e->loss_part;
  if (!fused_loss) {
    loss_kernel<<<M, 128, 0, st>>>(la);
    LAUNCH_OK("loss_kernel");
  } else {
    SilTarget tsil{nullptr, nullptr};
    if (sil_on) { if (a->target_sil_u8) tsil.b = a->target_sil_u8; else tsil.f = a->target_sil; }
    if (run_raster_forward(e, st, M, win, a->w_sil, tsil, a->sil_out,
                           sil_on ? e->gz : nullptr, sil_on ? e->tile_loss : nullptr, e->joints, &la)) return 1;
  }
  if (sil_on) {
    Section sec(e, st, SMALFIT_SEC_RASTER_BWD);
    launch_raster_bwd(e, st, M);
    LAUNCH_OK("raster_bwd_kernel");
  }
  if (a->verts_out) {
    planar_to_interleaved_kernel<<<dim3((m.V * 3 + 255) / 256, M), 256, 0, st>>>(M, m.V, m.Vp, e->verts, 3 * m.Vp, a->trans, a->verts_out);
    LAUNCH_OK("planar_to_interleaved_kernel");
  }

  const bool need_pose = a->g_joint_rotations != nullptr;
  const bool need_beta = a->g_betas != nullptr;
  const bool need_ls = a->g_log_beta_scales != nullptr && a->logscale_mode != 0;
  {
    Section sec(e, st, SMALFIT_SEC_LBS_BWD);
    if (run_lbs_backward(e, st, M, nb, 1, sil_on ? e->dface : nullptr, e->dJ41, nullptr, need_pose, need_beta, need_ls,
                         e->dth_direct, 0)) return 1;
  }

  AssembleArgs g;
  g.M = M; g.S = e->S; g.T = e->nrb; g.win = win; g.nb = nb; g.NBall = m.NBall;
  g.nblk_beta = e->nblk_beta; g.nvt = e->nvt; g.betas_shared = 1; g.ls_shared = a->logscale_mode == 1;
  g.w_sil = a->w_sil;
  g.dbeta_part = e->dbeta_part; g.dJrest = e->dJrest; g.JS = m.JS; g.dbetaJ = e->dbetaJ; g.ngrp_beta = kBetaGroups;
  g.gb_prior = shape_prior ? e->gb_prior : nullptr;
  g.gls_prior = prior_uses_ls ? e->gls_prior : nullptr;
  g.dls = e->dls; g.dtheta = e->dtheta; g.gmask = gmask; g.rmask = rmask;
  g.dtr_direct = e->dtr_direct; g.dtr_part = e->dtr_part; g.loss_part = e->loss_part;
  g.loss_betas = shape_prior ? e->loss_betas : nullptr;
  g.tile_loss = sil_on ? e->tile_loss : nullptr;
  g.qloss = sil_on ? e->qloss : nullptr;
  g.nqblk = kSelectBlocks + kBandBlocks;
  g.g_betas = need_beta ? a->g_betas : nullptr;
  g.g_ls = need_ls ? a->g_log_beta_scales : nullptr;
  g.g_grot = a->g_global_rotation; g.g_jrot = a->g_joint_rotations; g.g_trans = a->g_trans;
  g.losses = a->losses;
  g.lpart = e->lpart; g.qpart = e->qpart; g.counter = e->asm_counter;
  assemble_kernel<<<1 + 1 + kAsmElem + kAsmLoss, 256, 0, st>>>(g);
  LAUNCH_OK("assemble_kernel");
  if (e->prof_on) {
    if (e->prof_iter < e->prof_cap && (e->prof_tick % e->prof_stride) == 0) e->prof_iter++;
    e->prof_tick++;
  }
  return 0;
}

int smalfit_engine_profile_begin(smalfit_engine* e, int max_evals, int stride) {
  if (!e || max_evals <= 0 || stride <= 0) return fail("smalfit_engine_profile_begin: bad argument");
  for (auto ev : e->prof_ev) (void)hipEventDestroy(ev);
  e->prof_ev.assign((size_t)max_evals * SMALFIT_NUM_SECTIONS * 2, nullptr);
  for (auto& ev : e->prof_ev) HIP_OK(hipEventCreate(&ev));
  e->prof_cap = max_evals;
  e->prof_iter = 0;
  e->prof_stride = stride;
  e->prof_tick = 0;
  e->prof_on = true;
  return 0;
}

int smalfit_engine_profile_end(smalfit_engine* e, void* stream, float* ms_total, int* counts) {
  if (!e || !ms_total || !counts) return fail("smalfit_engine_profile_end: null argument");
  HIP_OK(hipStreamSynchronize((hipStream_t)stream));
  e->prof_on = false;
  for (int sct = 0; sct < SMALFIT_NUM_SECTIONS; ++sct) { ms_total[sct] = 0.f; counts[sct] = 0; }
  for (int it = 0; it < e->prof_iter; ++it)
    for (int sct = 0; sct < SMALFIT_NUM_SECTIONS; ++sct) {
      float ms = 0.f;
      hipEvent_t a = e->prof_ev[((size_t)it * SMALFIT_NUM_SECTIONS + sct) * 2];
      hipEvent_t b = e->prof_ev[((size_t)it * SMALFIT_NUM_SECTIONS + sct) * 2 + 1];
      if (hipEventElapsedTime(&ms, a, b) == hipSuccess) { ms_total[sct] += ms; counts[sct]++; }
    }
  (void)hipGetLastError();
  for (auto ev : e->prof_ev) (void)hipEventDestroy(ev);
  e->prof_ev.clear();
  e->prof_cap = e->prof_iter = 0;
  return 0;
}

namespace smalfit {
static int stage_vertex_offset(smalfit_engine* e, hipStream_t st, int M, const float* v_offset, HeadExtras& ex) {
  const ModelDev& m = e->model->dev;
  interleaved_to_planar_kernel<<<dim3(m.Vp / 256, M), 256, 0, st>>>(M, m.V, m.Vp, v_offset, e->dext);
  LAUNCH_OK("interleaved_to_planar_kernel");
  joints_kernel<<<dim3(41, M), 128, 0, st>>>(m, e->dext, e->dJ41);
  LAUNCH_OK("joints_kernel");
  ex.voff = e->dext; ex.joff = e->dJ41; ex.joff_stride = 123;
  return 0;
}
static int check_lbs_args(smalfit_engine* e, const smalfit_lbs_args* a, const char* who) {
  if (!e || !a) return fail(std::string(who) + ": null argument");
  if (a->num_frames <= 0 || a->num_frames > e->maxM) return fail(std::string(who) + ": num_frames exceeds the engine's max_frames");
  if (a->num_betas <= 0 || a->num_betas > e->model->dev.NBall) return fail(std::string(who) + ": num_betas out of range");
  if (!a->beta) return fail(std::string(who) + ": beta missing");
  if ((a->theta == nullptr) == (a->Rs == nullptr)) return fail(std::string(who) + ": give exactly one of theta (axis-angle) and Rs (rotation matrices)");
  return 0;
}
static int lbs_forward_common(smalfit_engine* e, hipStream_t st, const smalfit_lbs_args* a, float* joints_out) {
  const int M = a->num_frames, nb = a->num_betas;
  HeadExtras ex;
  if (a->theta) HIP_OK(hipMemcpyAsync(e->theta, a->theta, (size_t)M * 105 * 4, hipMemcpyDeviceToDevice, st));
  else HIP_OK(hipMemsetAsync(e->theta, 0, (size_t)M * 105 * 4, st));
  ex.Rs_in = a->Rs;
  if (a->v_offset && stage_vertex_offset(e, st, M, a->v_offset, ex)) return 1;
  return run_lbs_forward(e, st, M, a->beta, nb, nb, a->logscale, 6, e->zeros, joints_out, &ex);
}
}

int smalfit_lbs_forward_ex(smalfit_engine* e, void* stream, const smalfit_lbs_args* a) {
  if (check_lbs_args(e, a, "smalfit_lbs_forward_ex")) return 1;
  if (!a->verts || !a->joints) return fail("smalfit_lbs_forward_ex: verts / joints outputs missing");
  const ModelDev& m = e->model->dev;
  const int M = a->num_frames;
  hipStream_t st = (hipStream_t)stream;
  if (lbs_forward_common(e, st, a, a->joints)) return 1;
  const dim3 grid((m.V * 3 + 255) / 256, M);
  planar_to_interleaved_kernel<<<grid, 256, 0, st>>>(M, m.V, m.Vp, e->verts, 3 * m.Vp, nullptr, a->verts);
  if (a->v_shaped) planar_to_interleaved_kernel<<<grid, 256, 0, st>>>(M, m.V, m.Vp, e->v_shaped, 3 * m.Vp, nullptr, a->v_shaped);
  LAUNCH_OK("planar_to_interleaved_kernel");
  if (a->Rs_out) HIP_OK(hipMemcpyAsync(a->Rs_out, e->Rm, (size_t)M * 315 * 4, hipMemcpyDeviceToDevice, st));
  return 0;
}

int smalfit_lbs_backward_ex(smalfit_engine* e, void* stream, const smalfit_lbs_args* a) {
  if (check_lbs_args(e, a, "smalfit_lbs_backward_ex")) return 1;
  const ModelDev& m = e->model->dev;
  const int M = a->num_frames, nb = a->num_betas;
  hipStream_t st = (hipStream_t)stream;
  if (lbs_forward_common(e, st, a, e->joints)) return 1;
  const float* dext = nullptr;
  if (a->dverts) {
    interleaved_to_planar_kernel<<<dim3(m.Vp / 256, M), 256, 0, st>>>(M, m.V, m.Vp, a->dverts, e->dext);
    LAUNCH_OK("interleaved_to_planar_kernel");
    dext = e->dext;
  }
  const float* dj = a->djoints;
  if (a->v_offset) {
    if (dj) HIP_OK(hipMemcpyAsync(e->dJ41, dj, (size_t)M * 123 * 4, hipMemcpyDeviceToDevice, st));
    else HIP_OK(hipMemsetAsync(e->dJ41, 0, (size_t)M * 123 * 4, st));
    dj = e->dJ41;
  }
  if (run_lbs_backward(e, st, M, nb, 0, nullptr, dj, dext, true, a->dbeta != nullptr || a->dv_offset != nullptr,
                       a->logscale != nullptr && a->dlogscale != nullptr, nullptr, 105, a->Rs ? a->dRs : nullptr)) return 1;
  if (a->dtheta && a->theta) HIP_OK(hipMemcpyAsync(a->dtheta, e->dtheta, (size_t)M * 105 * 4, hipMemcpyDeviceToDevice, st));
  if (a->dlogscale) {
    if (a->logscale) HIP_OK(hipMemcpyAsync(a->dlogscale, e->dls, (size_t)M * 6 * 4, hipMemcpyDeviceToDevice, st));
    else HIP_OK(hipMemsetAsync(a->dlogscale, 0, (size_t)M * 6 * 4, st));
  }
  if (a->dbeta) {
    AssembleArgs g;
    std::memset(&g, 0, sizeof(g));
    g.M = M; g.nb = nb; g.NBall = m.NBall; g.nblk_beta = e->nblk_beta; g.betas_shared = 0;
    g.dbeta_part = e->dbeta_part; g.dJrest = e->dJrest; g.JS = m.JS; g.dbetaJ = e->dbetaJ; g.ngrp_beta = 1; g.g_betas = a->dbeta;
    g.win = WinMap{1, 0, M};
    assemble_kernel<<<M, 256, 0, st>>>(g);
    LAUNCH_OK("assemble_kernel");
  }
  if (a->dv_offset) {
    offset_grad_kernel<<<dim3((m.V + 255) / 256, M), 256, 0, st>>>(m, M, e->dvp, e->dJrest, a->dv_offset);
    LAUNCH_OK("offset_grad_kernel");
  }
  return 0;
}

int smalfit_lbs_forward(smalfit_engine* e, void* stream, int M, int nb, const float* beta, const float* theta,
                        const float* logscale, float* verts, float* joints, float* Rs, float* v_shaped) {
  if (!theta) return fail("smalfit_lbs_forward: null argument");
  smalfit_lbs_args a;
  std::memset(&a, 0, sizeof(a));
  a.num_frames = M; a.num_betas = nb; a.beta = beta; a.theta = theta; a.logscale = logscale;
  a.verts = verts; a.joints = joints; a.Rs_out = Rs; a.v_shaped = v_shaped;
  return smalfit_lbs_forward_ex(e, stream, &a);
}

int smalfit_lbs_backward(smalfit_engine* e, void* stream, int M, int nb, const float* beta, const float* theta,
                         const float* logscale, const float* dverts, const float* djoints, float* dbeta,
                         float* dtheta, float* dlogscale) {
  if (!theta) return fail("smalfit_lbs_backward: null argument");
  smalfit_lbs_args a;
  std::memset(&a, 0, sizeof(a));
  a.num_frames = M; a.num_betas = nb; a.beta = beta; a.theta = theta; a.logscale = logscale;
  a.dverts = dverts; a.djoints = djoints; a.dbeta = dbeta; a.dtheta = dtheta; a.dlogscale = dlogscale;
  return smalfit_lbs_backward_ex(e, stream, &a);
}

int smalfit_rodrigues(void* stream, int count, const float* theta, float* R) {
  if (count <= 0 || !theta || !R) return fail("smalfit_rodrigues: bad argument");
  rodrigues_kernel<<<(count + 255) / 256, 256, 0, (hipStream_t)stream>>>(count, theta, R);
  LAUNCH_OK("rodrigues_kernel");
  return 0;
}

int smalfit_global_rigid_transformation(void* stream, int count, const float* Rs, const float* Js, const int* parents,
                                        const float* logscale, float* new_J, float* A) {
  if (count <= 0 || !Rs || !Js || !parents || !new_J || !A) return fail("smalfit_global_rigid_transformation: bad argument");
  Parents35 par;
  par.p[0] = -1;
  for (int i = 1; i < 35; ++i) {
    if (!(parents[i] >= 0 && parents[i] < i)) return fail("smalfit_global_rigid_transformation: parents must satisfy 0 <= parents[i] < i");
    par.p[i] = parents[i];
  }
  global_rigid_kernel<<<(count + 63) / 64, 64, 0, (hipStream_t)stream>>>(count, Rs, Js, par, logscale, new_J, A);
  LAUNCH_OK("global_rigid_kernel");
  return 0;
}

int smalfit_global_rigid_transformation_backward(void* stream, int count, const float* Rs, const float* Js, const int* parents,
                                                 const float* logscale, const float* d_new_J, const float* d_A,
                                                 float* scratch, float* dRs, float* dJs, float* dlogscale) {
  if (count <= 0 || !Rs || !Js || !parents || !d_new_J || !d_A || !scratch || !dRs || !dJs)
    return fail("smalfit_global_rigid_transformation_backward: bad argument");
  Parents35 par;
  par.p[0] = -1;
  for (int i = 1; i < 35; ++i) {
    if (!(parents[i] >= 0 && parents[i] < i)) return fail("smalfit_global_rigid_transformation_backward: parents must satisfy 0 <= parents[i] < i");
    par.p[i] = parents[i];
  }
  global_rigid_bwd_kernel<<<(count + 63) / 64, 64, 0, (hipStream_t)stream>>>(count, Rs, Js, par, logscale, d_new_J, d_A, scratch, dRs, dJs,
                                                                            logscale ? dlogscale : nullptr);
  LAUNCH_OK("global_rigid_bwd_kernel");
  return 0;
}

int smalfit_rodrigues_backward(void* stream, int count, const float* theta, const float* dR, float* dtheta) {
  if (count <= 0 || !theta || !dR || !dtheta) return fail("smalfit_rodrigues_backward: bad argument");
  rodrigues_bwd_kernel<<<(count + 255) / 256, 256, 0, (hipStream_t)stream>>>(count, theta, dR, dtheta);
  LAUNCH_OK("rodrigues_bwd_kernel");
  return 0;
}

int smalfit_render_forward(smalfit_engine* e, void* stream, int M, const float* verts, const float* points, int P,
                           float* sil, float* proj_points) {
  if (!e || !verts) return fail("smalfit_render_forward: null argument");
  if (M <= 0 || M > e->maxM) return fail("smalfit_render_forward: M exceeds the engine's max_frames");
  hipStream_t st = (hipStream_t)stream;
  const ModelDev& m = e->model->dev;
  if (sil) {
    project_verts_kernel<<<dim3(m.Vp / 256, M), 256, 0, st>>>(M, m.V, m.Vp, verts, e->proj);
    LAUNCH_OK("project_verts_kernel");
    if (run_raster_forward(e, st, M, WinMap{1, 0, M}, 0.f, SilTarget{nullptr, nullptr}, sil, nullptr, nullptr)) return 1;
  }
  if (points && proj_points && P > 0) {
    project_points_kernel<<<(M * P + 255) / 256, 256, 0, st>>>(M * P, e->S, points, proj_points);
    LAUNCH_OK("project_points_kernel");
  }
  return 0;
}

}

namespace smalfit {
__global__ void raster_vertex_grad_kernel(ModelDev m, const float* __restrict__ proj, const float* __restrict__ dface,
                                          float* __restrict__ dverts) {
  const int v = blockIdx.x * blockDim.x + threadIdx.x, n = blockIdx.y;
  if (v >= m.V) return;
  float gxn = 0.f, gyn = 0.f;
  const float* df = dface + (size_t)n * m.F * 6;
  for (int i = m.vf_off[v]; i < m.vf_off[v + 1]; ++i) {
    gxn += df[m.vf_idx[i] * 2];
    gyn += df[m.vf_idx[i] * 2 + 1];
  }
  const float* pv = proj + (size_t)n * 3 * m.Vp;
  float g[3];
  world_to_ndc_bwd(pv[v], pv[m.Vp + v], pv[2 * m.Vp + v], gxn, gyn, g[0], g[1], g[2]);
  float* o = dverts + ((size_t)n * m.V + v) * 3;
  o[0] = g[0]; o[1] = g[1]; o[2] = g[2];
}
}

extern "C" {

int smalfit_render_color(smalfit_engine* e, void* stream, int M, const float* verts, const float* rgb, float* image) {
  if (!e || !verts || !rgb || !image) return fail("smalfit_render_color: null argument");
  if (M <= 0 || M > e->maxM) return fail("smalfit_render_color: M exceeds the engine's max_frames");
  hipStream_t st = (hipStream_t)stream;
  const ModelDev& m = e->model->dev;
  const size_t npx = (size_t)e->S * e->S;
  if (!e->zbuf && hipMalloc(&e->zbuf, (size_t)e->maxM * npx * sizeof(unsigned long long)) != hipSuccess)
    return fail("smalfit_render_color: hipMalloc of the z-buffer failed");
  if (!e->vnorm && hipMalloc(&e->vnorm, (size_t)e->maxM * 3 * m.Vp * sizeof(float)) != hipSuccess)
    return fail("smalfit_render_color: hipMalloc of the vertex normals failed");
  interleaved_to_planar_kernel<<<dim3(m.Vp / 256, M), 256, 0, st>>>(M, m.V, m.Vp, verts, e->verts);
  project_verts_kernel<<<dim3(m.Vp / 256, M), 256, 0, st>>>(M, m.V, m.Vp, verts, e->proj);
  vnormal_kernel<<<dim3(m.Vp / 256, M), 256, 0, st>>>(m, M, e->verts, e->vnorm);
  HIP_OK(hipMemsetAsync(e->zbuf, 0xff, (size_t)M * npx * sizeof(unsigned long long), st));
  color_zbuf_kernel<<<dim3((m.F + 15) / 16, M), 256, 0, st>>>(m, e->S, e->proj, e->zbuf);
  color_shade_kernel<<<dim3((unsigned)((npx + 255) / 256), M), 256, 0, st>>>(m, e->S, e->proj, e->verts, e->vnorm, e->zbuf, rgb[0], rgb[1],
                                                                            rgb[2], image);
  LAUNCH_OK("colour render kernels");
  return 0;
}

int smalfit_render_backward(smalfit_engine* e, void* stream, int M, const float* verts, const float* sil,
                            const float* dsil, float* dverts) {
  if (!e || !verts || !sil || !dsil || !dverts) return fail("smalfit_render_backward: null argument");
  if (M <= 0 || M > e->maxM) return fail("smalfit_render_backward: M exceeds the engine's max_frames");
  hipStream_t st = (hipStream_t)stream;
  const ModelDev& m = e->model->dev;
  project_verts_kernel<<<dim3(m.Vp / 256, M), 256, 0, st>>>(M, m.V, m.Vp, verts, e->proj);
  if (run_raster_forward(e, st, M, WinMap{1, 0, M}, 0.f, SilTarget{nullptr, nullptr}, e->silbuf, e->gz, nullptr)) return 1;
  const size_t total = (size_t)M * e->S * e->S;
  gpix_from_dsil_kernel<<<(unsigned)((total + 255) / 256), 256, 0, st>>>(total, sil, dsil, e->gz);
  launch_raster_bwd(e, st, M);
  raster_vertex_grad_kernel<<<dim3((m.V + 255) / 256, M), 256, 0, st>>>(m, e->proj, e->dface, dverts);
  LAUNCH_OK("render_backward kernels");
  return 0;
}

int smalfit_project_points_backward(void* stream, int count, int image_size, const float* points, const float* dproj,
                                    float* dpoints) {
  if (count <= 0 || !points || !dproj || !dpoints) return fail("smalfit_project_points_backward: bad argument");
  project_points_bwd_kernel<<<(count + 255) / 256, 256, 0, (hipStream_t)stream>>>(count, image_size, points, dproj, dpoints);
  LAUNCH_OK("project_points_bwd_kernel");
  return 0;
}

int smalfit_pose_prior(smalfit_engine* e, void* stream, int N, const float* x, float* out) {
  if (!e || !x || !out || N <= 0) return fail("smalfit_pose_prior: bad argument");
  if (!e->has_pose_prior) return fail("smalfit_pose_prior: pose prior not set");
  pose_prior_kernel<<<N, 128, 0, (hipStream_t)stream>>>(x, e->pose_prec, e->pose_mean, e->pose_mask, out);
  LAUNCH_OK("pose_prior_kernel");
  return 0;
}

int smalfit_pose_prior_backward(smalfit_engine* e, void* stream, int N, const float* x, const float* dout, float* dx) {
  if (!e || !x || !dout || !dx || N <= 0) return fail("smalfit_pose_prior_backward: bad argument");
  if (!e->has_pose_prior) return fail("smalfit_pose_prior_backward: pose prior not set");
  pose_prior_bwd_kernel<<<N, 128, 0, (hipStream_t)stream>>>(x, e->pose_prec, e->pose_mean, e->pose_mask, dout, dx);
  LAUNCH_OK("pose_prior_bwd_kernel");
  return 0;
}

int smalfit_temporal(smalfit_engine* e, void* stream, int N, float w_temp, const float* global_rotation,
                     const float* joint_rotations, const float* trans, const float* global_mask,
                     const float* rotation_mask, float* losses, float* g_global_rotation, float* g_joint_rotations,
                     float* g_trans) {
  if (!e || !global_rotation || !joint_rotations || !trans || !losses) return fail("smalfit_temporal: null argument");
  if (N <= 0 || N > e->maxM) return fail("smalfit_temporal: N exceeds the engine's max_frames");
  hipStream_t st = (hipStream_t)stream;
  const float* gmask = global_mask ? global_mask : e->ones;
  const float* rmask = rotation_mask ? rotation_mask : e->ones;
  build_theta_kernel<<<(N * 105 + 255) / 256, 256, 0, st>>>(N, global_rotation, joint_rotations, gmask, rmask, e->theta);
  temporal_kernel<<<1, 128, 0, st>>>(N, w_temp, e->theta, trans, losses, e->dtheta, g_trans ? g_trans : e->dtr_direct);
  split_theta_grad_kernel<<<(N * 105 + 255) / 256, 256, 0, st>>>(N, e->dtheta, gmask, rmask, g_global_rotation, g_joint_rotations);
  LAUNCH_OK("temporal kernels");
  return 0;
}

namespace smalfit {
static int pack_adam_segments(const smalfit_adam_args* o, AdamSegments& sg) {
  if (!o->param || !o->grad || !o->exp_avg || !o->exp_avg_sq) return fail("smalfit adam: null buffer");
  if (o->num_segments < 0 || o->num_segments > 4) return fail("smalfit adam: at most 4 segments");
  std::memset(&sg, 0, sizeof(sg));
  sg.nseg = o->num_segments;
  int total = 0;
  for (int k = 0; k < sg.nseg; ++k) {
    if (o->seg_begin[k] < 0 || o->seg_end[k] < o->seg_begin[k]) return fail("smalfit adam: bad segment");
    sg.beg[k] = o->seg_begin[k];
    sg.off[k] = total;
    total += o->seg_end[k] - o->seg_begin[k];
  }
  for (int k = sg.nseg; k <= 4; ++k) sg.off[k] = total;
  return 0;
}

static int launch_adam_segments(hipStream_t st, const AdamSegments& sg, const smalfit_adam_args* o, int t, bool fresh) {
  const int total = sg.off[sg.nseg];
  if (total == 0) return 0;
  float step_size, bc2_sqrt;
  adam_bias_terms(o->lr, o->beta1, o->beta2, t, step_size, bc2_sqrt);
  adam_segments_kernel<<<(total + 255) / 256, 256, 0, st>>>(sg, o->param, o->grad, o->exp_avg, o->exp_avg_sq, step_size,
                                                           o->beta1, o->beta2, o->eps, bc2_sqrt, fresh ? 1 : 0);
  LAUNCH_OK("adam_segments_kernel");
  return 0;
}

static int launch_adam_next_step(hipStream_t st, const smalfit_adam_args* o) {
  AdamSegments sg;
  if (pack_adam_segments(o, sg)) return 1;
  return launch_adam_segments(st, sg, o, o->step + 1, o->step == 0);
}
}

int smalfit_adam_segments(void* stream, const smalfit_adam_args* o) {
  if (!o) return fail("smalfit_adam_segments: null argument");
  if (o->step < 0) return fail("smalfit_adam_segments: step must be >= 0");
  return launch_adam_next_step((hipStream_t)stream, o);
}

int smalfit_engine_set_graph(smalfit_engine* e, int enable) {
  if (!e) return fail("smalfit_engine_set_graph: null argument");
  e->use_graph = enable != 0;
  if (!e->use_graph && e->graph_exec) { (void)hipGraphExecDestroy(e->graph_exec); e->graph_exec = nullptr; e->graph_key.clear(); }
  return 0;
}

namespace smalfit {
static int launch_adam_graph_node(smalfit_engine* e, hipStream_t st, const AdamSegments& sg, const smalfit_adam_args* o) {
  const int total = sg.off[sg.nseg];
  if (total == 0) return 0;
  adam_segments_graph_kernel<<<(total + 255) / 256, 256, 0, st>>>(sg, o->param, o->grad, o->exp_avg, o->exp_avg_sq, e->step_counter,
                                                                 o->lr, o->beta1, o->beta2, o->eps);
  LAUNCH_OK("adam_segments_graph_kernel");
  return 0;
}
}

int smalfit_fit_run(smalfit_engine* e, void* stream, const smalfit_fit_args* a, const smalfit_adam_args* o, int iterations) {
  if (!e || !a || !o) return fail("smalfit_fit_run: null argument");
  if (iterations <= 0) return fail("smalfit_fit_run: iterations must be positive");
  if (o->step < 0) return fail("smalfit_fit_run: step must be >= 0");
  AdamSegments sg;
  if (pack_adam_segments(o, sg)) return 1;
  hipStream_t st = (hipStream_t)stream;
  if (e->use_graph && !e->prof_on && iterations >= 2 && st != nullptr) {
    smalfit_adam_args okey = *o;
    okey.step = 0;
    const unsigned cfg[2] = {e->config_epoch, (unsigned)g_dbg};
    std::vector<unsigned char> key(sizeof(*a) + sizeof(okey) + sizeof(st) + sizeof(cfg));
    std::memcpy(key.data(), a, sizeof(*a));
    std::memcpy(key.data() + sizeof(*a), &okey, sizeof(okey));
    std::memcpy(key.data() + sizeof(*a) + sizeof(okey), &st, sizeof(st));
    std::memcpy(key.data() + sizeof(*a) + sizeof(okey) + sizeof(st), cfg, sizeof(cfg));
    if (!e->graph_exec || key != e->graph_key) {
      if (e->graph_exec) { (void)hipGraphExecDestroy(e->graph_exec); e->graph_exec = nullptr; }
      hipGraph_t graph = nullptr;
      HIP_OK(hipStreamBeginCapture(st, hipStreamCaptureModeThreadLocal));
      tick_kernel<<<1, 1, 0, st>>>(e->step_counter);
      int rc = smalfit_fit_eval(e, stream, a);
      if (!rc) rc = launch_adam_graph_node(e, st, sg, o);
      const hipError_t ce = hipStreamEndCapture(st, &graph);
      if (rc) { if (graph) (void)hipGraphDestroy(graph); return 1; }
      if (ce != hipSuccess) return fail(std::string("hipStreamEndCapture: ") + hipGetErrorString(ce));
      const hipError_t ie = hipGraphInstantiate(&e->graph_exec, graph, nullptr, nullptr, 0);
      (void)hipGraphDestroy(graph);
      if (ie != hipSuccess) { e->graph_exec = nullptr; return fail(std::string("hipGraphInstantiate: ") + hipGetErrorString(ie)); }
      e->graph_key = key;
    }
    set_counter_kernel<<<1, 1, 0, st>>>(e->step_counter, o->step);
    LAUNCH_OK("set_counter_kernel");
    for (int it = 0; it < iterations; ++it) HIP_OK(hipGraphLaunch(e->graph_exec, st));
    return 0;
  }
  for (int it = 0; it < iterations; ++it) {
    const int t = o->step + it + 1;
    if (smalfit_fit_eval(e, stream, a)) return 1;
    if (launch_adam_segments(st, sg, o, t, t == 1)) return 1;
  }
  return 0;
}

int smalfit_shard_record(void* stream, int num_shared, const float* shared_grad, int num_frames, const float* global_rotation,
                         const float* joint_rotations, const float* trans, const float* global_mask,
                         const float* rotation_mask, float* record) {
  if (num_shared < 0 || !shared_grad || num_frames <= 0 || !global_rotation || !joint_rotations || !trans || !global_mask ||
      !rotation_mask || !record) return fail("smalfit_shard_record: bad argument");
  shard_record_kernel<<<(num_shared + 216 + 255) / 256, 256, 0, (hipStream_t)stream>>>(num_shared, shared_grad, num_frames, global_rotation,
                                                                                    joint_rotations, trans, global_mask, rotation_mask, record);
  LAUNCH_OK("shard_record_kernel");
  return 0;
}

int smalfit_shard_local_step(smalfit_engine* e, void* stream, const smalfit_fit_args* a, const smalfit_adam_args* o, int num_shared,
                             const float* shared_grad, float* record) {
  if (!e || !a || !o || !record || !shared_grad) return fail("smalfit_shard_local_step: null argument");
  if (o->step < 0) return fail("smalfit_shard_local_step: step must be >= 0");
  if (smalfit_fit_eval(e, stream, a)) return 1;
  if (launch_adam_next_step((hipStream_t)stream, o)) return 1;
  return smalfit_shard_record(stream, num_shared, shared_grad, a->num_frames, a->global_rotation, a->joint_rotations, a->trans,
                              a->global_mask ? a->global_mask : e->ones, a->rotation_mask ? a->rotation_mask : e->ones, record);
}

int smalfit_shard_reduce_step(void* stream, int world_size, int record_stride, const float* gathered, int num_shared,
                              int num_trainable, const smalfit_adam_args* o) {
  if (world_size <= 0 || record_stride < num_shared || !gathered || num_shared <= 0 || num_trainable < 0 || num_trainable > num_shared || !o)
    return fail("smalfit_shard_reduce_step: bad argument");
  if (!o->param || !o->grad || !o->exp_avg || !o->exp_avg_sq || o->step < 0) return fail("smalfit_shard_reduce_step: bad optimiser state");
  float step_size, bc2_sqrt;
  adam_bias_terms(o->lr, o->beta1, o->beta2, o->step + 1, step_size, bc2_sqrt);
  shard_reduce_adam_kernel<<<(num_shared + 255) / 256, 256, 0, (hipStream_t)stream>>>(world_size, record_stride, gathered, num_shared, num_trainable,
                                                                                   o->param, o->grad, o->exp_avg, o->exp_avg_sq, step_size,
                                                                                   o->beta1, o->beta2, o->eps, bc2_sqrt, o->step == 0 ? 1 : 0);
  LAUNCH_OK("shard_reduce_adam_kernel");
  return 0;
}

int smalfit_rccl_allgather(void* ctx, const float* send, float* recv, int count, void* stream) {
  const smalfit_rccl_ctx* c = (const smalfit_rccl_ctx*)ctx;
  if (!c || !c->comm || !c->nccl_all_gather) return fail("smalfit_rccl_allgather: no communicator / ncclAllGather address");
  typedef int (*all_gather_t)(const void*, void*, size_t, int, void*, hipStream_t);
  const int kNcclFloat32 = 7;
  const int rc = ((all_gather_t)c->nccl_all_gather)(send, recv, (size_t)count, kNcclFloat32, c->comm, (hipStream_t)stream);
  if (rc != 0) return fail("smalfit_rccl_allgather: ncclAllGather returned " + std::to_string(rc));
  return 0;
}

int smalfit_shard_run(smalfit_engine* e, void* stream, const smalfit_fit_args* a, const smalfit_adam_args* ol,
                      const smalfit_adam_args* os, const smalfit_shard_args* sh, int iterations) {
  if (!e || !a || !ol || !os || !sh) return fail("smalfit_shard_run: null argument");
  if (sh->struct_size != (unsigned)sizeof(smalfit_shard_args))
    return fail("smalfit_shard_run: smalfit_shard_args.struct_size does not match this library (built against another smalfit.h?)");
  if (iterations <= 0) return fail("smalfit_shard_run: iterations must be positive");
  if (sh->world_size <= 0 || sh->rank < 0 || sh->rank >= sh->world_size) return fail("smalfit_shard_run: bad rank / world_size");
  if (sh->num_shared <= 0 || sh->num_trainable_shared < 0 || sh->num_trainable_shared > sh->num_shared) return fail("smalfit_shard_run: bad num_shared / num_trainable_shared");
  if (!sh->shared_grad || !sh->record || !sh->gathered || !sh->allgather) return fail("smalfit_shard_run: missing buffer / collective");
  if (ol->step < 0 || os->step != ol->step) return fail("smalfit_shard_run: adam_local and adam_shared must carry the same step >= 0");
  const int stride = sh->num_shared + 216;
  for (int it = 0; it < iterations; ++it) {
    smalfit_adam_args l = *ol, s = *os;
    l.step = s.step = ol->step + it;
    if (smalfit_shard_local_step(e, stream, a, &l, sh->num_shared, sh->shared_grad, sh->record)) return 1;
    if (sh->allgather(sh->allgather_ctx, sh->record, sh->gathered, stride, stream)) {
      if (g_err.empty() || g_err.find("allgather") == std::string::npos) return fail("smalfit_shard_run: the caller's all-gather reported an error");
      return 1;
    }
    if (smalfit_shard_reduce_step(stream, sh->world_size, stride, sh->gathered, sh->num_shared, sh->num_trainable_shared, &s)) return 1;
  }
  return 0;
}

int smalfit_adam_step(void* stream, int count, float* param, const float* grad, float* exp_avg, float* exp_avg_sq,
                      float lr, float beta1, float beta2, float eps, int t) {
  if (count <= 0 || !param || !grad || !exp_avg || !exp_avg_sq || t <= 0) return fail("smalfit_adam_step: bad argument");
  smalfit_adam_args o{};
  o.param = param; o.grad = const_cast<float*>(grad); o.exp_avg = exp_avg; o.exp_avg_sq = exp_avg_sq;
  o.num_segments = 1; o.seg_begin[0] = 0; o.seg_end[0] = count;
  o.lr = lr; o.beta1 = beta1; o.beta2 = beta2; o.eps = eps;
  AdamSegments sg;
  if (pack_adam_segments(&o, sg)) return 1;
  return launch_adam_segments((hipStream_t)stream, sg, &o, t, false);
}

}
```

### smalify_amd/csrc/smalfit_math.h

```cpp
#pragma once
#include <math.h>

#if defined(__HIPCC__)
#define SMALFIT_HD __host__ __device__ __forceinline__
#else
#define SMALFIT_HD inline
#endif

namespace smalfit {

SMALFIT_HD float recip(float x) {
#if defined(__HIP_DEVICE_COMPILE__)
  return __builtin_amdgcn_rcpf(x);
#else
  return 1.0f / x;
#endif
}

constexpr int kJoints = 35;
constexpr int kPoseFeat = 306;
constexpr int kModelJoints = 41;
constexpr int kKeypoints = 25;
constexpr int kLogScales = 6;

constexpr float kCamDist = 2.7f;
constexpr float kCamScale = 1.7320508075688772f;
constexpr float kSigma = 1e-4f;
constexpr float kBlur = 9.21024036697585e-4f;
constexpr float kBlurSqrt = 0.030348377826444f;
constexpr float kEps = 1e-8f;
constexpr int kFacesPerPixel = 100;

SMALFIT_HD void rodrigues_fwd(const float th[3], float R[9]) {
  const float ux = th[0] + 1e-8f, uy = th[1] + 1e-8f, uz = th[2] + 1e-8f;
  const float a = sqrtf(ux * ux + uy * uy + uz * uz);
  const float ia = 1.0f / a;
  const float rx = th[0] * ia, ry = th[1] * ia, rz = th[2] * ia;
  const float c = cosf(a), s = sinf(a), k = 1.0f - c;
  R[0] = c + k * rx * rx;      R[1] = k * rx * ry - s * rz; R[2] = k * rx * rz + s * ry;
  R[3] = k * ry * rx + s * rz; R[4] = c + k * ry * ry;      R[5] = k * ry * rz - s * rx;
  R[6] = k * rz * rx - s * ry; R[7] = k * rz * ry + s * rx; R[8] = c + k * rz * rz;
}

SMALFIT_HD void rodrigues_bwd(const float th[3], const float G[9], float dth[3]) {
  const float ux = th[0] + 1e-8f, uy = th[1] + 1e-8f, uz = th[2] + 1e-8f;
  const float a = sqrtf(ux * ux + uy * uy + uz * uz);
  const float ia = 1.0f / a;
  const float r[3] = {th[0] * ia, th[1] * ia, th[2] * ia};
  const float c = cosf(a), s = sinf(a), k = 1.0f - c;
  float Gr[3], GTr[3];
  for (int i = 0; i < 3; ++i) {
    Gr[i] = G[3 * i] * r[0] + G[3 * i + 1] * r[1] + G[3 * i + 2] * r[2];
    GTr[i] = G[i] * r[0] + G[3 + i] * r[1] + G[6 + i] * r[2];
  }
  const float rGr = r[0] * Gr[0] + r[1] * Gr[1] + r[2] * Gr[2];
  const float trG = G[0] + G[4] + G[8];
  const float kv[3] = {G[7] - G[5], G[2] - G[6], G[3] - G[1]};
  const float dc = trG - rGr;
  const float ds = r[0] * kv[0] + r[1] * kv[1] + r[2] * kv[2];
  float dr[3];
  for (int i = 0; i < 3; ++i) dr[i] = k * (Gr[i] + GTr[i]) + s * kv[i];
  const float da = -s * dc + c * ds - (dr[0] * r[0] + dr[1] * r[1] + dr[2] * r[2]) * ia;
  dth[0] = dr[0] * ia + da * ux * ia;
  dth[1] = dr[1] * ia + da * uy * ia;
  dth[2] = dr[2] * ia + da * uz * ia;
}

SMALFIT_HD void mat3_mul(const float A[9], const float B[9], float C[9]) {
  for (int i = 0; i < 3; ++i)
    for (int j = 0; j < 3; ++j)
      C[3 * i + j] = A[3 * i] * B[j] + A[3 * i + 1] * B[3 + j] + A[3 * i + 2] * B[6 + j];
}
SMALFIT_HD void mat3_vec(const float A[9], const float v[3], float o[3]) {
  for (int i = 0; i < 3; ++i) o[i] = A[3 * i] * v[0] + A[3 * i + 1] * v[1] + A[3 * i + 2] * v[2];
}
SMALFIT_HD void mat3T_vec(const float A[9], const float v[3], float o[3]) {
  for (int i = 0; i < 3; ++i) o[i] = A[i] * v[0] + A[3 + i] * v[1] + A[6 + i] * v[2];
}

SMALFIT_HD int limb_scale_index(int j, int a) {
  if (j >= 7 && j < 25 && j != 15 && j != 16) return a == 2 ? 0 : 1;
  if (j >= 25 && j < 32) return a == 0 ? 2 : 3;
  if (j == 33 || j == 34) return a == 1 ? 4 : (a == 2 ? 5 : -1);
  return -1;
}

SMALFIT_HD void global_rigid_frame(const float* Rs, const float* Js, const int* parents, const float* logscale,
                                   float* newJ, float* A) {
  float es[6], ies[6];
  for (int k = 0; k < 6; ++k) {
    es[k] = logscale != nullptr ? expf(logscale[k]) : 1.0f;
    ies[k] = 1.0f / es[k];
  }
  for (int i = 0; i < kJoints; ++i) {
    float* G = A + 16 * i;
    if (i == 0) {
      for (int r = 0; r < 3; ++r) {
        for (int c = 0; c < 3; ++c) G[r * 4 + c] = Rs[r * 3 + c];
        G[r * 4 + 3] = Js[r];
      }
    } else {
      const int p = parents[i];
      const float* Gp = A + 16 * p;
      for (int r = 0; r < 3; ++r) {
        for (int c = 0; c < 3; ++c) {
          const int si = limb_scale_index(i, c);
          const float sc = si >= 0 ? es[si] : 1.0f;
          float acc = 0.f;
          for (int q = 0; q < 3; ++q) {
            const int sp = limb_scale_index(p, q);
            const float isc = sp >= 0 ? ies[sp] : 1.0f;
            acc = fmaf(Gp[r * 4 + q], Rs[9 * i + q * 3 + c] * sc * isc, acc);
          }
          G[r * 4 + c] = acc;
        }
        float acc = Gp[r * 4 + 3];
        for (int q = 0; q < 3; ++q) acc = fmaf(Gp[r * 4 + q], Js[3 * i + q] - Js[3 * p + q], acc);
        G[r * 4 + 3] = acc;
      }
    }
    G[12] = 0.f; G[13] = 0.f; G[14] = 0.f; G[15] = 1.0f;
  }
  for (int i = 0; i < kJoints; ++i) {
    float* G = A + 16 * i;
    for (int r = 0; r < 3; ++r) {
      newJ[3 * i + r] = G[r * 4 + 3];
      float val = G[r * 4 + 3];
      for (int q = 0; q < 3; ++q) val = fmaf(-G[r * 4 + q], Js[3 * i + q], val);
      G[r * 4 + 3] = val;
    }
  }
}

SMALFIT_HD void global_rigid_frame_bwd(const float* Rs, const float* Js, const int* parents, const float* logscale,
                                       const float* dnewJ, const float* dA, float* G ,
                                       float* dG , float* dRs, float* dJs, float* dlogscale) {
  float es[6], ies[6], des[6];
  for (int k = 0; k < 6; ++k) {
    es[k] = logscale != nullptr ? expf(logscale[k]) : 1.0f;
    ies[k] = 1.0f / es[k];
    des[k] = 0.f;
  }
  auto sc = [&](int j, int a) { const int si = limb_scale_index(j, a); return si >= 0 ? es[si] : 1.0f; };
  auto isc = [&](int j, int a) { const int si = limb_scale_index(j, a); return si >= 0 ? ies[si] : 1.0f; };
  for (int i = 0; i < kJoints; ++i) {
    float* g = G + 12 * i;
    if (i == 0) {
      for (int r = 0; r < 3; ++r) { for (int c = 0; c < 3; ++c) g[r * 4 + c] = Rs[r * 3 + c]; g[r * 4 + 3] = Js[r]; }
    } else {
      const int p = parents[i];
      const float* gp = G + 12 * p;
      for (int r = 0; r < 3; ++r) {
        for (int c = 0; c < 3; ++c) {
          float acc = 0.f;
          for (int q = 0; q < 3; ++q) acc = fmaf(gp[r * 4 + q], Rs[9 * i + q * 3 + c] * sc(i, c) * isc(p, q), acc);
          g[r * 4 + c] = acc;
        }
        float acc = gp[r * 4 + 3];
        for (int q = 0; q < 3; ++q) acc = fmaf(gp[r * 4 + q], Js[3 * i + q] - Js[3 * p + q], acc);
        g[r * 4 + 3] = acc;
      }
    }
  }
  for (int i = 0; i < kJoints; ++i) {
    const float* da = dA + 16 * i;
    const float* g = G + 12 * i;
    float* dg = dG + 12 * i;
    for (int r = 0; r < 3; ++r) {
      for (int q = 0; q < 3; ++q) dg[r * 4 + q] = da[r * 4 + q] - da[r * 4 + 3] * Js[3 * i + q];
      dg[r * 4 + 3] = da[r * 4 + 3] + dnewJ[3 * i + r];
    }
    for (int q = 0; q < 3; ++q) {
      float acc = 0.f;
      for (int r = 0; r < 3; ++r) acc = fmaf(-g[r * 4 + q], da[r * 4 + 3], acc);
      dJs[3 * i + q] = acc;
    }
  }
  for (int i = kJoints - 1; i >= 1; --i) {
    const int p = parents[i];
    const float* gp = G + 12 * p;
    const float* dg = dG + 12 * i;
    float* dgp = dG + 12 * p;
    float dRp[9], dj[3];
    for (int q = 0; q < 3; ++q) {
      for (int c = 0; c < 3; ++c) dRp[q * 3 + c] = gp[0 * 4 + q] * dg[0 * 4 + c] + gp[1 * 4 + q] * dg[1 * 4 + c] + gp[2 * 4 + q] * dg[2 * 4 + c];
      dj[q] = gp[0 * 4 + q] * dg[3] + gp[1 * 4 + q] * dg[7] + gp[2 * 4 + q] * dg[11];
    }
    for (int r = 0; r < 3; ++r) {
      for (int q = 0; q < 3; ++q) {
        float acc = dg[r * 4 + 3] * (Js[3 * i + q] - Js[3 * p + q]);
        for (int c = 0; c < 3; ++c) acc = fmaf(dg[r * 4 + c], Rs[9 * i + q * 3 + c] * sc(i, c) * isc(p, q), acc);
        dgp[r * 4 + q] += acc;
      }
      dgp[r * 4 + 3] += dg[r * 4 + 3];
    }
    for (int q = 0; q < 3; ++q) { dJs[3 * i + q] += dj[q]; dJs[3 * p + q] -= dj[q]; }
    for (int q = 0; q < 3; ++q)
      for (int c = 0; c < 3; ++c) {
        const float rp = Rs[9 * i + q * 3 + c];
        dRs[9 * i + q * 3 + c] = dRp[q * 3 + c] * sc(i, c) * isc(p, q);
        const int si = limb_scale_index(i, c), sp = limb_scale_index(p, q);
        if (si >= 0) des[si] += dRp[q * 3 + c] * rp * isc(p, q);
        if (sp >= 0) des[sp] -= dRp[q * 3 + c] * rp * sc(i, c) * isc(p, q) * isc(p, q);
      }
  }
  for (int r = 0; r < 3; ++r) {
    for (int c = 0; c < 3; ++c) dRs[r * 3 + c] = dG[r * 4 + c];
    dJs[r] += dG[r * 4 + 3];
  }
  if (logscale != nullptr && dlogscale != nullptr)
    for (int k = 0; k < 6; ++k) dlogscale[k] = des[k] * es[k];
}

SMALFIT_HD void world_to_ndc(float x, float y, float z, float& xn, float& yn, float& zv) {
  zv = kCamDist - z;
  const float iz = kCamScale / zv;
  xn = -x * iz;
  yn = y * iz;
}
SMALFIT_HD void world_to_ndc_bwd(float xn, float yn, float zv, float gxn, float gyn,
                                 float& gx, float& gy, float& gz) {
  const float iz = 1.0f / zv;
  gx = -kCamScale * iz * gxn;
  gy = kCamScale * iz * gyn;
  gz = (xn * gxn + yn * gyn) * iz;
}

struct FaceRec {
  float ax, ay, e1x, e1y;
  float e2x, e2y, e3x, e3y;
  float il1, il2, il3, area;
  float t01, t02, t03, inv_den;
  float pz0, gzx, gzy, pad;
};

SMALFIT_HD float face_depth(const FaceRec& r, float dx, float dy) { return fmaf(r.gzy, dy, fmaf(r.gzx, dx, r.pz0)); }

SMALFIT_HD bool make_face_rec(float ax, float ay, float az, float bx, float by, float bz,
                              float cx, float cy, float cz, FaceRec& r) {
  r.ax = ax; r.ay = ay;
  r.e1x = bx - ax; r.e1y = by - ay;
  r.e2x = cx - ax; r.e2y = cy - ay;
  r.e3x = cx - bx; r.e3y = cy - by;
  const float l1 = r.e1x * r.e1x + r.e1y * r.e1y;
  const float l2 = r.e2x * r.e2x + r.e2y * r.e2y;
  const float l3 = r.e3x * r.e3x + r.e3y * r.e3y;
  r.il1 = l1 > kEps ? recip(l1) : 0.0f;  r.t01 = l1 > kEps ? 0.0f : 1.0f;
  r.il2 = l2 > kEps ? recip(l2) : 0.0f;  r.t02 = l2 > kEps ? 0.0f : 1.0f;
  r.il3 = l3 > kEps ? recip(l3) : 0.0f;  r.t03 = l3 > kEps ? 0.0f : 1.0f;
  r.area = r.e2x * r.e1y - r.e2y * r.e1x;
  r.inv_den = recip(r.area + kEps);
  const float da = cz - az, db = az - bz;
  r.gzx = r.inv_den * (da * r.e1y + db * r.e2y);
  r.gzy = -r.inv_den * (da * r.e1x + db * r.e2x);
  r.pz0 = r.inv_den * az * r.area;
  r.pad = 0.0f;
  const float zmax = fmaxf(az, fmaxf(bz, cz));
  return (fabsf(r.area) > kEps) && (zmax >= 0.0f);
}

SMALFIT_HD float face_pixel_depth(const FaceRec& r, float px, float py) { return face_depth(r, px - r.ax, py - r.ay); }

struct PixEval {
  float d;
  float pz;
  float qx, qy;
  float tc;
  int edge;
  bool inside;
};

SMALFIT_HD bool face_pixel_eval(const FaceRec& r, float px, float py, PixEval& o) {
  const float dx = px - r.ax, dy = py - r.ay;
  const float c1 = fmaf(dx, r.e1y, -(dy * r.e1x));
  const float c2 = fmaf(dx, r.e2y, -(dy * r.e2x));
  const float w2 = c1 * r.inv_den;
  const float w1 = -c2 * r.inv_den;
  const float w0 = ((c2 - c1) + r.area) * r.inv_den;
  o.inside = (w0 > 0.0f) && (w1 > 0.0f) && (w2 > 0.0f);
  const float pz = face_depth(r, dx, dy);
  o.pz = pz;
  const float t1 = fminf(fmaxf(fmaf(fmaf(dy, r.e1y, dx * r.e1x), r.il1, r.t01), 0.0f), 1.0f);
  const float q1x = fmaf(-t1, r.e1x, dx), q1y = fmaf(-t1, r.e1y, dy);
  const float d1 = fmaf(q1y, q1y, q1x * q1x);
  const float t2 = fminf(fmaxf(fmaf(fmaf(dy, r.e2y, dx * r.e2x), r.il2, r.t02), 0.0f), 1.0f);
  const float q2x = fmaf(-t2, r.e2x, dx), q2y = fmaf(-t2, r.e2y, dy);
  const float d2 = fmaf(q2y, q2y, q2x * q2x);
  const float ex = dx - r.e1x, ey = dy - r.e1y;
  const float t3 = fminf(fmaxf(fmaf(fmaf(ey, r.e3y, ex * r.e3x), r.il3, r.t03), 0.0f), 1.0f);
  const float q3x = fmaf(-t3, r.e3x, ex), q3y = fmaf(-t3, r.e3y, ey);
  const float d3 = fmaf(q3y, q3y, q3x * q3x);
  float dist = d1; o.qx = q1x; o.qy = q1y; o.tc = t1; o.edge = 0;
  if (d2 < dist) { dist = d2; o.qx = q2x; o.qy = q2y; o.tc = t2; o.edge = 1; }
  if (d3 < dist) { dist = d3; o.qx = q3x; o.qy = q3y; o.tc = t3; o.edge = 2; }
  o.d = o.inside ? -dist : dist;
  return (pz >= 0.0f) && (o.inside || dist < kBlur);
}

SMALFIT_HD bool face_pixel_candidate(const FaceRec& r, float px, float py, float& d_out) {
  const float dx = px - r.ax, dy = py - r.ay;
  const float c1 = fmaf(dx, r.e1y, -(dy * r.e1x));
  const float c2 = fmaf(dx, r.e2y, -(dy * r.e2x));
  const float w2 = c1 * r.inv_den;
  const float w1 = -c2 * r.inv_den;
  const float w0 = ((c2 - c1) + r.area) * r.inv_den;
  const bool inside = fminf(w0, fminf(w1, w2)) > 0.0f;
  const float pz = face_depth(r, dx, dy);
  const float t1 = fminf(fmaxf(fmaf(fmaf(dy, r.e1y, dx * r.e1x), r.il1, r.t01), 0.0f), 1.0f);
  const float q1x = fmaf(-t1, r.e1x, dx), q1y = fmaf(-t1, r.e1y, dy);
  const float d1 = fmaf(q1y, q1y, q1x * q1x);
  const float t2 = fminf(fmaxf(fmaf(fmaf(dy, r.e2y, dx * r.e2x), r.il2, r.t02), 0.0f), 1.0f);
  const float q2x = fmaf(-t2, r.e2x, dx), q2y = fmaf(-t2, r.e2y, dy);
  const float d2 = fmaf(q2y, q2y, q2x * q2x);
  const float ex = dx - r.e1x, ey = dy - r.e1y;
  const float t3 = fminf(fmaxf(fmaf(fmaf(ey, r.e3y, ex * r.e3x), r.il3, r.t03), 0.0f), 1.0f);
  const float q3x = fmaf(-t3, r.e3x, ex), q3y = fmaf(-t3, r.e3y, ey);
  const float d3 = fmaf(q3y, q3y, q3x * q3x);
  const float dist = fminf(d1, fminf(d2, d3));
  d_out = inside ? -dist : dist;
  return (pz >= 0.0f) && (inside || dist < kBlur);
}

SMALFIT_HD float one_minus_prob(float d) { return recip(1.0f + expf(-d * (1.0f / kSigma))); }
SMALFIT_HD float prob(float d) { return recip(1.0f + expf(d * (1.0f / kSigma))); }

SMALFIT_HD float log2_one_minus_prob(float d) {
  const float x2 = d * (1.4426950408889634f / kSigma);
  const float ls2 = fminf(x2, 0.0f) - log2f(1.0f + exp2f(-fabsf(x2)));
  return fmaxf(ls2, -256.0f);
}

SMALFIT_HD float pix_to_ndc(int i, float inv_s) { return fmaf((float)i, -2.0f * inv_s, 1.0f - inv_s); }

SMALFIT_HD void adam_bias_terms(float lr, float beta1, float beta2, int t, float& step_size, float& bc2_sqrt) {
  const double bc1 = 1.0 - pow((double)beta1, (double)t), bc2 = 1.0 - pow((double)beta2, (double)t);
  step_size = (float)((double)lr / bc1);
  bc2_sqrt = (float)sqrt(bc2);
}

SMALFIT_HD void adam_update(float g, float m0, float v0, float b1, float b2, float eps, float step_size, float bc2_sqrt,
                            float& m, float& v, float& p) {
  const float mi = b1 * m0 + (1.0f - b1) * g;
  const float vi = b2 * v0 + (1.0f - b2) * g * g;
  m = mi;
  v = vi;
  const float denom = sqrtf(vi) / bc2_sqrt + eps;
  p = p - step_size * (mi / denom);
}

}
```

Measured before the change: 2901.

## Fold gradient assembly and Adam step into next iteration's LBS head kernel

On the multi-iteration, non-graph fit path, the assemble kernel and the separate Adam launch for each iteration are replaced by a pending step. The next iteration's LBS head kernel reduces the gradients, applies Adam and uses the updated parameters directly. Shared beta and log-scale state is double-buffered in a small device slot, and a restore kernel is added for the two-iteration edge case. Assemble-side loads are software-prefetched into registers, and adam_update is rewritten with explicit fma so results match across the host-side and in-kernel paths. This removes kernel launches and global round-trips per iteration, at the cost of redundant per-block reductions of the shared gradients and considerable complexity.

```diff
diff --git a/smalify_amd/csrc/kernels_lbs_backward.inc b/smalify_amd/csrc/kernels_lbs_backward.inc
--- a/smalify_amd/csrc/kernels_lbs_backward.inc
+++ b/smalify_amd/csrc/kernels_lbs_backward.inc
@@ -593,46 +593,25 @@
   if (role < nbs) {
     if (a.g_betas) {
       const int s = role;
-      const int bl = t % 20, slice = t / 20;
-      auto beta_pass = [&](int b0) {
-        const int b = b0 + bl;
-        if (slice < 12 && b < a.nb) {
-          double acc = 0.0;
-          const int nlo = a.betas_shared ? 0 : s, nhi = a.betas_shared ? M : s + 1;
-          for (int n = nlo + slice; n < nhi; n += 12) acc += (double)a.dbetaJ[(size_t)n * a.NBall + b];
-          const int nparts = a.nblk_beta * a.ngrp_beta;
-#pragma unroll 8
-          for (int blk = slice; blk < nparts; blk += 12) acc += (double)a.dbeta_part[((size_t)s * nparts + blk) * a.nb + b];
-          bsum[slice][bl] = acc;
-        }
+      for (int b0 = 0; b0 < a.nb; b0 += 20) {
+        if (b0) __syncthreads();
+        BetaOperands bo;
+        asm_beta_fetch(a, s, b0, bo);
+        asm_beta_slices(a, s, b0, bo, bsum);
         __syncthreads();
-        if (t < 20 && b0 + t < a.nb) {
-          double tot = 0.0;
-          for (int sl = 0; sl < 12; ++sl) tot += bsum[sl][t];
-          if (a.gb_prior && s == 0) tot += (double)a.gb_prior[b0 + t];
-          a.g_betas[s * a.nb + b0 + t] = (float)tot;
-        }
-      };
-      beta_pass(0);
-      for (int b0 = 20; b0 < a.nb; b0 += 20) {
-        __syncthreads();
-        beta_pass(b0);
+        const float tot = asm_beta_total(a, s, b0, bo, bsum);
+        if (t < 20 && b0 + t < a.nb) a.g_betas[s * a.nb + b0 + t] = tot;
       }
     }
   } else if ((role -= nbs) == 0) {
     if (a.g_ls) {
       if (a.ls_shared) {
-        const int e = t & 7, sl = t >> 3;
-        double acc = 0.0;
-        if (e < 6) for (int n = sl; n < M; n += 32) acc += (double)a.dls[(size_t)n * 6 + e];
-        dpart[sl][e] = acc;
+        LsOperands lo;
+        asm_ls_fetch(a, lo);
+        asm_ls_slices(a, lo, dpart);
         __syncthreads();
-        if (t < 6) {
-          double tot = 0.0;
-          for (int i = 0; i < 32; ++i) tot += dpart[i][t];
-          if (a.gls_prior) tot += (double)a.gls_prior[t];
-          a.g_ls[t] = (float)tot;
-        }
+        const float tot = asm_ls_total(a, lo, dpart);
+        if (t < 6) a.g_ls[t] = tot;
       } else {
         for (int i = t; i < M * 6; i += 256) a.g_ls[i] = a.dls[i];
       }
@@ -641,13 +620,8 @@
     const int gt = role * 256 + t, gs = kAsmElem * 256;
     for (int i = gt; i < M * 3; i += gs) {
       const int n = i / 3, e = i % 3;
-      if (a.g_grot) a.g_grot[i] = a.dtheta[(size_t)n * 105 + e] * a.gmask[e];
-      if (a.g_trans) {
-        double acc = a.dtr_direct ? (double)a.dtr_direct[i] : 0.0;
-#pragma unroll 16
-        for (int vt = 0; vt < a.nvt; ++vt) acc += (double)a.dtr_part[((size_t)vt * M + n) * 3 + e];
-        a.g_trans[i] = (float)acc;
-      }
+      if (a.g_grot) a.g_grot[i] = asm_grot_elem(a, n, e);
+      if (a.g_trans) a.g_trans[i] = asm_trans_elem(a, n, e);
     }
     if (a.g_jrot) {
       const int total = M * 102;
@@ -656,7 +630,7 @@
 #pragma unroll
         for (int u = 0; u < 8; ++u) {
           const int i = min(i0 + u * gs, total - 1), n = i / 102, e = i % 102;
-          v[u] = a.dtheta[(size_t)n * 105 + 3 + e] * a.rmask[e];
+          v[u] = asm_jrot_elem(a, n, e);
         }
 #pragma unroll
         for (int u = 0; u < 8; ++u)
@@ -781,6 +755,16 @@
   float step_size, bc2_sqrt;
   adam_bias_terms(lr, b1, b2, t, step_size, bc2_sqrt);
   adam_segments_element(sg, j, p, g, mm, vv, step_size, b1, b2, eps, bc2_sqrt, t == 1);
+}
+
+__global__ void shared_state_restore_kernel(const float* __restrict__ slot, float* __restrict__ p, float* __restrict__ mm, float* __restrict__ vv,
+                                            int nbeta, int off_beta, int nls, int off_ls) {
+  const int t = threadIdx.x;
+  int i = -1, j = t;
+  if (t < nbeta) i = off_beta + t;
+  else if (t >= 20 && t < 20 + nls) i = off_ls + (t - 20);
+  if (i < 0) return;
+  p[i] = slot[j]; mm[i] = slot[32 + j]; vv[i] = slot[64 + j];
 }
 
 __global__ void shard_record_kernel(int ns, const float* __restrict__ shared_grad, int M, const float* __restrict__ grot,
diff --git a/smalify_amd/csrc/kernels_lbs_forward.inc b/smalify_amd/csrc/kernels_lbs_forward.inc
--- a/smalify_amd/csrc/kernels_lbs_forward.inc
+++ b/smalify_amd/csrc/kernels_lbs_forward.inc
@@ -1,3 +1,97 @@
+
+constexpr int kAsmFr = 8, kAsmPa = 32, kAsmLs = 4;
+struct BetaOperands { float fv[kAsmFr], pv[kAsmPa], prior; };
+__device__ __forceinline__ void asm_beta_fetch(const AssembleArgs& a, int s, int b0, BetaOperands& o) {
+  const int t = threadIdx.x, slice = min(t / 20, 11), b = min(b0 + t % 20, a.nb - 1);
+  const int nlo = a.betas_shared ? 0 : s, nhi = a.betas_shared ? a.M : s + 1, nparts = a.nblk_beta * a.ngrp_beta;
+  const float* pj = a.dbetaJ + b;
+  const float* pp = a.dbeta_part + (size_t)s * nparts * a.nb + b;
+#pragma unroll
+  for (int u = 0; u < kAsmFr; ++u) o.fv[u] = pj[(size_t)min(nlo + slice + 12 * u, nhi - 1) * a.NBall];
+#pragma unroll
+  for (int u = 0; u < kAsmPa; ++u) o.pv[u] = pp[(size_t)min(slice + 12 * u, nparts - 1) * a.nb];
+  o.prior = (a.gb_prior && s == 0) ? a.gb_prior[min(b0 + min(t, 19), a.nb - 1)] : 0.f;
+}
+__device__ __forceinline__ void asm_beta_slices(const AssembleArgs& a, int s, int b0, BetaOperands& o, double (*bsum)[32]) {
+  const int t = threadIdx.x, bl = t % 20, slice = t / 20, b = b0 + bl;
+  if (slice < 12 && b < a.nb) {
+    const int nlo = a.betas_shared ? 0 : s, nhi = a.betas_shared ? a.M : s + 1, nparts = a.nblk_beta * a.ngrp_beta;
+    const float* pj = a.dbetaJ + b;
+    const float* pp = a.dbeta_part + (size_t)s * nparts * a.nb + b;
+    double acc = 0.0;
+    for (int n0 = nlo + slice; n0 < nhi; n0 += 12 * kAsmFr) {
+#pragma unroll
+      for (int u = 0; u < kAsmFr; ++u)
+        if (n0 + 12 * u < nhi) acc += (double)o.fv[u];
+      if (n0 + 12 * kAsmFr < nhi) {
+#pragma unroll
+        for (int u = 0; u < kAsmFr; ++u) o.fv[u] = pj[(size_t)min(n0 + 12 * (kAsmFr + u), nhi - 1) * a.NBall];
+      }
+    }
+    for (int k0 = slice; k0 < nparts; k0 += 12 * kAsmPa) {
+#pragma unroll
+      for (int u = 0; u < kAsmPa; ++u)
+        if (k0 + 12 * u < nparts) acc += (double)o.pv[u];
+      if (k0 + 12 * kAsmPa < nparts) {
+#pragma unroll
+        for (int u = 0; u < kAsmPa; ++u) o.pv[u] = pp[(size_t)min(k0 + 12 * (kAsmPa + u), nparts - 1) * a.nb];
+      }
+    }
+    bsum[slice][bl] = acc;
+  }
+}
+__device__ __forceinline__ float asm_beta_total(const AssembleArgs& a, int s, int b0, const BetaOperands& o, double (*bsum)[32]) {
+  const int t = threadIdx.x;
+  double tot = 0.0;
+  if (t < 20 && b0 + t < a.nb) {
+    for (int sl = 0; sl < 12; ++sl) tot += bsum[sl][t];
+    if (a.gb_prior && s == 0) tot += (double)o.prior;
+  }
+  return (float)tot;
+}
+struct LsOperands { float lv[kAsmLs], prior; };
+__device__ __forceinline__ void asm_ls_fetch(const AssembleArgs& a, LsOperands& o) {
+  const int t = threadIdx.x, e = min(t & 7, 5), sl = t >> 3;
+#pragma unroll
+  for (int u = 0; u < kAsmLs; ++u) o.lv[u] = a.dls[(size_t)min(sl + 32 * u, a.M - 1) * 6 + e];
+  o.prior = a.gls_prior ? a.gls_prior[min(t, 5)] : 0.f;
+}
+__device__ __forceinline__ void asm_ls_slices(const AssembleArgs& a, LsOperands& o, double (*dpart)[8]) {
+  const int t = threadIdx.x, e = t & 7, sl = t >> 3;
+  double acc = 0.0;
+  if (e < 6)
+    for (int n0 = sl; n0 < a.M; n0 += 32 * kAsmLs) {
+#pragma unroll
+      for (int u = 0; u < kAsmLs; ++u)
+        if (n0 + 32 * u < a.M) acc += (double)o.lv[u];
+      if (n0 + 32 * kAsmLs < a.M) {
+#pragma unroll
+        for (int u = 0; u < kAsmLs; ++u) o.lv[u] = a.dls[(size_t)min(n0 + 32 * (kAsmLs + u), a.M - 1) * 6 + e];
+      }
+    }
+  dpart[sl][e] = acc;
+}
+__device__ __forceinline__ float asm_ls_total(const AssembleArgs& a, const LsOperands& o, double (*dpart)[8]) {
+  const int t = threadIdx.x;
+  double tot = 0.0;
+  if (t < 6) {
+    for (int i = 0; i < 32; ++i) tot += dpart[i][t];
+    if (a.gls_prior) tot += (double)o.prior;
+  }
+  return (float)tot;
+}
+__device__ __forceinline__ float asm_theta_elem(const AssembleArgs& a, int n, int l) {
+  const float* mk = (l < 3) ? a.gmask + l : a.rmask + max(l - 3, 0);
+  return a.dtheta[(size_t)n * 105 + l] * *mk;
+}
+__device__ __forceinline__ float asm_grot_elem(const AssembleArgs& a, int n, int e) { return asm_theta_elem(a, n, e); }
+__device__ __forceinline__ float asm_jrot_elem(const AssembleArgs& a, int n, int e) { return asm_theta_elem(a, n, 3 + e); }
+__device__ __forceinline__ float asm_trans_elem(const AssembleArgs& a, int n, int e) {
+  double acc = a.dtr_direct ? (double)a.dtr_direct[n * 3 + e] : 0.0;
+#pragma unroll 16
+  for (int vt = 0; vt < a.nvt; ++vt) acc += (double)a.dtr_part[((size_t)vt * a.M + n) * 3 + e];
+  return (float)acc;
+}
 
 
 struct HeadArgs {
@@ -23,8 +117,82 @@
   const float* voff;
 };
 
+constexpr int kPendingNb = 20;
+struct HeadShared {
+  float beta[kPendingNb], ls[8], grot[4];
+  double bsum[12][32], dpart[32][8];
+};
+struct AdamOperands { float p, m, v; };
+__device__ __forceinline__ AdamOperands pending_load(const PendingStep& p, const PendingTensor& T, int i) {
+  return AdamOperands{T.p_in[i], p.fresh ? 0.f : T.m_in[i], p.fresh ? 0.f : T.v_in[i]};
+}
+__device__ __forceinline__ float pending_adam(const PendingStep& p, const PendingTensor& T, int i, const AdamOperands& o, float gi, bool store) {
+  float mi, vi, pv = o.p;
+  adam_update(gi, o.m, o.v, p.b1, p.b2, p.eps, p.step_size, p.bc2_sqrt, mi, vi, pv);
+  if (store) { T.m[i] = mi; T.v[i] = vi; T.p[i] = pv; T.g[i] = gi; }
+  return pv;
+}
+struct SharedOperands { AdamOperands beta, ls; BetaOperands bo; LsOperands lo; };
+__device__ __forceinline__ void pending_shared_fetch(const PendingStep& p, const HeadArgs& a, int n, SharedOperands& o) {
+  const int t = threadIdx.x;
+  o.beta = pending_load(p, p.betas, min(t, 19));
+  if (p.betas.train) asm_beta_fetch(p.g, 0, 0, o.bo);
+  if (a.logscale) {
+    if (p.g.ls_shared) o.ls = pending_load(p, p.ls, min(t, 5));
+    else if (!p.ls.train) o.ls.p = a.logscale[(size_t)n * a.ls_stride + min(t, 5)];
+    if (p.ls.train && p.g.ls_shared) asm_ls_fetch(p.g, o.lo);
+  }
+}
+__device__ __forceinline__ void pending_shared_slices(const PendingStep& p, SharedOperands& o, HeadShared& sh) {
+  if (p.betas.train) asm_beta_slices(p.g, 0, 0, o.bo, sh.bsum);
+  if (p.ls.train && p.g.ls_shared) asm_ls_slices(p.g, o.lo, sh.dpart);
+}
+__device__ __forceinline__ void pending_shared_step(const PendingStep& p, const HeadArgs& a, const SharedOperands& o, HeadShared& sh) {
+  const int t = threadIdx.x;
+  const bool store = blockIdx.x == 0;
+  if (p.betas.train) {
+    const float gi = asm_beta_total(p.g, 0, 0, o.bo, sh.bsum);
+    if (t < 20) sh.beta[t] = pending_adam(p, p.betas, t, o.beta, gi, store);
+  } else if (t < 20) {
+    sh.beta[t] = o.beta.p;
+  }
+  if (a.logscale && (p.g.ls_shared || !p.ls.train)) {
+    if (p.ls.train) {
+      const float gi = asm_ls_total(p.g, o.lo, sh.dpart);
+      if (t < 6) sh.ls[t] = pending_adam(p, p.ls, t, o.ls, gi, store);
+    } else if (t < 6) {
+      sh.ls[t] = o.ls.p;
+    }
+  }
+}
+struct ThetaOperands { AdamOperands ao; float gi; };
+__device__ __forceinline__ void pending_jrot_fetch(const PendingStep& p, int n, ThetaOperands& o) {
+  const int l = max(min((int)threadIdx.x, 104), 3);
+  o.ao = pending_load(p, p.jrot, n * 102 + (l - 3));
+  o.gi = asm_theta_elem(p.g, n, l);
+}
+__device__ __forceinline__ float pending_jrot_step(const PendingStep& p, int n, const ThetaOperands& o) {
+  const int l = threadIdx.x;
+  if (l >= 3 && l < 105 && p.jrot.train) return pending_adam(p, p.jrot, n * 102 + (l - 3), o.ao, o.gi, true);
+  return o.ao.p;
+}
+__device__ __forceinline__ void pending_frame_extras(const PendingStep& p, int n, HeadShared& sh) {
+  const int l = threadIdx.x;
+  if (l >= 128 && l < 131) {
+    const int i = n * 3 + (l - 128);
+    if (p.trans.train) pending_adam(p, p.trans, i, pending_load(p, p.trans, i), asm_trans_elem(p.g, n, l - 128), true);
+  } else if (l >= 224 && l < 227) {
+    const int i = n * 3 + (l - 224);
+    const AdamOperands ao = pending_load(p, p.grot, i);
+    sh.grot[l - 224] = p.grot.train ? pending_adam(p, p.grot, i, ao, asm_theta_elem(p.g, n, l - 224), true) : ao.p;
+  } else if (l >= 192 && l < 198) {
+    if (p.ls.train && !p.g.ls_shared) { const int i = n * 6 + (l - 192); sh.ls[l - 192] = pending_adam(p, p.ls, i, pending_load(p, p.ls, i), p.g.dls[i], true); }
+  }
+}
+
+template <bool kPending>
 __device__ __forceinline__ void
-pose_block(const ModelDev& m, const HeadArgs& a, int n) {
+pose_block(const ModelDev& m, const HeadArgs& a, int n, const PendingStep* pend, HeadShared* sh) {
   __shared__ float th[105];
   __shared__ float R[35][9];
   __shared__ float sc[35][3], isc[35][3];
@@ -41,20 +209,56 @@
   }
   if (l >= 128 && l < 128 + kTreeMaxPass * 8) { const int q = l - 128; t_pj[q >> 3][q & 7] = tl.pass_joint[q >> 3][q & 7]; t_pp[q >> 3][q & 7] = tl.pass_parent[q >> 3][q & 7]; }
   const int nlev = tl.nlev;
+  float tv_pend = 0.f, js_pre[kPendingNb], jt_pre = 0.f, mv_pre = 0.f;
+  int idx_pre = 0;
+  if constexpr (kPending) {
+    const int lc = min(l, 104);
+    idx_pre = m.scale_idx[lc]; jt_pre = m.Jt[lc];
+    mv_pre = (lc < 3) ? a.gmask[lc] : a.rmask[max(lc - 3, 0)];
+#pragma unroll
+    for (int b = 0; b < kPendingNb; ++b) js_pre[b] = m.JS[lc * m.NBall + b];
+    SharedOperands so;
+    ThetaOperands to;
+    pending_shared_fetch(*pend, a, n, so);
+    pending_jrot_fetch(*pend, n, to);
+    pending_frame_extras(*pend, n, *sh);
+    tv_pend = pending_jrot_step(*pend, n, to);
+    pending_shared_slices(*pend, so, *sh);
+    PHASE_MARK(pp1);
+    __syncthreads();
+    pending_shared_step(*pend, a, so, *sh);
+    PHASE_MARK(pp2);
+    __syncthreads();
+    if (l < 3) tv_pend = sh->grot[l];
+    PHASE_MARK(pp3);
+    PHASE_ADD(PH_HEAD_POSE, 4, ph0, pp1); PHASE_ADD(PH_HEAD_POSE, 5, pp1, pp2); PHASE_ADD(PH_HEAD_POSE, 6, pp2, pp3);
+  }
   if (l < 105) {
     const int lj = max(l - 3, 0);
     const float* tsrc = a.theta_in ? a.theta_in + (size_t)n * 105 + l : ((l < 3) ? a.grot + n * 3 + l : a.jrot + (size_t)n * 102 + lj);
     const float* msrc = a.theta_in ? tsrc : ((l < 3) ? a.gmask + l : a.rmask + lj);
-    const int idx = m.scale_idx[l];
-    const float tv0 = *tsrc, mv = *msrc;
-    float acc = m.Jt[l];
-    const float lsv = a.logscale ? a.logscale[(size_t)n * a.ls_stride + max(idx, 0)] : 0.f;
+    int idx;
+    float tv0, mv, lsv, acc;
+    if constexpr (kPending) {
+      idx = idx_pre; tv0 = tv_pend; mv = mv_pre; acc = jt_pre;
+      lsv = a.logscale ? sh->ls[max(idx, 0)] : 0.f;
+    } else {
+      idx = m.scale_idx[l];
+      tv0 = *tsrc; mv = *msrc;
+      acc = m.Jt[l];
+      lsv = a.logscale ? a.logscale[(size_t)n * a.ls_stride + max(idx, 0)] : 0.f;
+    }
     const float tv = a.theta_in ? tv0 : tv0 * mv;
     th[l] = tv;
     a.theta[(size_t)n * 105 + l] = tv;
-    const float* beta = a.betas + (size_t)(a.betas_stride ? n : 0) * a.betas_stride;
+    if constexpr (kPending) {
+#pragma unroll
+      for (int b = 0; b < kPendingNb; ++b) acc = fmaf(js_pre[b], sh->beta[b], acc);
+    } else {
+      const float* beta = a.betas + (size_t)(a.betas_stride ? n : 0) * a.betas_stride;
 #pragma unroll 10
-    for (int b = 0; b < a.nb; ++b) acc = fmaf(m.JS[l * m.NBall + b], beta[b], acc);
+      for (int b = 0; b < a.nb; ++b) acc = fmaf(m.JS[l * m.NBall + b], beta[b], acc);
+    }
     if (a.joff) acc += a.joff[(size_t)n * a.joff_stride + l];
     J[l / 3][l % 3] = acc;
     if (a.betas_stride || n == 0) a.Jrest[(size_t)(a.betas_stride ? n : 0) * 105 + l] = acc;
@@ -163,11 +367,73 @@
   PHASE_END(PH_HEAD_POSE, ph0, ph4);
 }
 
-__global__ void __launch_bounds__(256)
-lbs_head_kernel(ModelDev m, HeadArgs a) {
+template <bool kPending>
+__device__ __forceinline__ void
+head_block(const ModelDev& m, const HeadArgs& a, const PendingStep* pend, HeadShared* sh) {
   int blk = blockIdx.x;
-  if (blk < a.M) { pose_block(m, a, blk); return; }
+  if (blk < a.M) { pose_block<kPending>(m, a, blk, pend, sh); return; }
   blk -= a.M;
+  if constexpr (kPending) {
+    const int Vp = m.Vp, v = min(blk, a.nshape_x - 1) * 256 + threadIdx.x, t = threadIdx.x, D = a.prior_D;
+    const bool shape = blk < a.nshape;
+    float vt_pre[3], sd_pre[3][kPendingNb], pcol[26], prow[26];
+    if (shape) {
+#pragma unroll
+      for (int c = 0; c < 3; ++c) {
+        vt_pre[c] = m.vt[c * Vp + v];
+#pragma unroll
+        for (int b = 0; b < kPendingNb; ++b) sd_pre[c][b] = m.sd[((size_t)b * 3 + c) * Vp + v];
+      }
+    } else if (a.prior_prec) {
+      const int tc = min(t, D - 1);
+#pragma unroll
+      for (int r = 0; r < 26; ++r) { const int rc = min(r, D - 1); pcol[r] = a.prior_prec[rc * D + tc]; prow[r] = a.prior_prec[tc * D + rc]; }
+    }
+    const float pmean = (!shape && a.prior_prec) ? a.prior_mean[min(t, D - 1)] : 0.f;
+    SharedOperands so;
+    pending_shared_fetch(*pend, a, 0, so);
+    pending_shared_slices(*pend, so, *sh);
+    __syncthreads();
+    pending_shared_step(*pend, a, so, *sh);
+    __syncthreads();
+    if (shape) {
+#pragma unroll
+      for (int c = 0; c < 3; ++c) {
+        float acc = vt_pre[c];
+#pragma unroll
+        for (int b = 0; b < kPendingNb; ++b) acc = fmaf(sh->beta[b], sd_pre[c][b], acc);
+        if (a.voff) acc += a.voff[(size_t)c * Vp + v];
+        a.v_shaped[(size_t)c * Vp + v] = acc;
+      }
+      return;
+    }
+    if (a.prior_prec && t < 64) {
+      __shared__ float x[32], res[32];
+      if (t < D) x[t] = ((t < 20) ? sh->beta[t] : sh->ls[t - 20]) - pmean;
+      __builtin_amdgcn_fence(__ATOMIC_ACQ_REL, "workgroup");
+      __builtin_amdgcn_wave_barrier();
+      float lv = 0.f;
+      if (t < D) {
+        float acc = 0.f;
+#pragma unroll
+        for (int r = 0; r < 26; ++r) if (r < D) acc = fmaf(x[r], pcol[r], acc);
+        res[t] = acc;
+        lv = acc * acc;
+      }
+      __builtin_amdgcn_fence(__ATOMIC_ACQ_REL, "workgroup");
+      __builtin_amdgcn_wave_barrier();
+      lv = wave_sum(lv);
+      if (t == 0) *a.prior_loss = a.prior_w * lv / (float)D;
+      if (t < D) {
+        float acc = 0.f;
+#pragma unroll
+        for (int c = 0; c < 26; ++c) if (c < D) acc = fmaf(res[c], prow[c], acc);
+        acc *= 2.0f * a.prior_w / (float)D;
+        if (t < 20) a.prior_gb[t] = acc; else if (a.prior_use_ls) a.prior_gls[t - 20] = acc;
+      }
+    }
+    return;
+  }
   if (blk < a.nshape) {
     PHASE_MARK(ps0);
     const int s = blk / a.nshape_x;
@@ -212,6 +478,15 @@
       if (t < 20) a.prior_gb[t] = acc; else if (a.prior_use_ls) a.prior_gls[t - 20] = acc;
     }
   }
+}
+
+__global__ void __launch_bounds__(256)
+lbs_head_kernel(ModelDev m, HeadArgs a) { head_block<false>(m, a, nullptr, nullptr); }
+
+__global__ void __launch_bounds__(256)
+lbs_head_step_kernel(ModelDev m, HeadArgs a, PendingStep p) {
+  __shared__ HeadShared sh;
+  head_block<true>(m, a, &p, &sh);
 }
 
 __global__ void build_theta_kernel(int M, const float* __restrict__ grot, const float* __restrict__ jrot,
diff --git a/smalify_amd/csrc/smalfit_internal.h b/smalify_amd/csrc/smalfit_internal.h
--- a/smalify_amd/csrc/smalfit_internal.h
+++ b/smalify_amd/csrc/smalfit_internal.h
@@ -114,4 +114,16 @@
   float* losses;
 };
 
+struct PendingTensor {
+  int train;
+  const float *p_in, *m_in, *v_in;
+  float *p, *m, *v, *g;
+};
+struct PendingStep {
+  AssembleArgs g;
+  PendingTensor betas, ls, grot, jrot, trans;
+  float step_size, b1, b2, eps, bc2_sqrt;
+  int fresh;
+};
+
 }
diff --git a/smalify_amd/csrc/smalfit_launch.inc b/smalify_amd/csrc/smalfit_launch.inc
--- a/smalify_amd/csrc/smalfit_launch.inc
+++ b/smalify_amd/csrc/smalfit_launch.inc
@@ -87,6 +87,7 @@
   float* lpart;
   long long* qpart;
   int* asm_counter;
+  float* shstate;
   float *silbuf, *tile_loss, *dface;
   float *dJ41, *dvert, *dvp, *dext, *dA, *dpf_part, *dbeta_part, *dtheta, *dls, *dJrest;
   float* dbetaJ;
@@ -424,6 +425,7 @@
   CARVE(qpart, 64, long long);
   CARVE(zc, M, float);
   CARVE(asm_counter, 4, int);
+  CARVE(shstate, 2 * 3 * 32, float);
   CARVE(step_counter, 4, int);
   CARVE(gb_prior, 64, float);
   CARVE(gls_prior, 16, float);
@@ -540,7 +542,10 @@
   float prior_w = 0.f;
   const float *Rs_in = nullptr, *joff = nullptr, *voff = nullptr;
   int joff_stride = 0;
+  const PendingStep* pending = nullptr;
+  int prior_slot = 0;
 };
+static constexpr int kPriorSlotB = 32, kPriorSlotLs = 8;
 
 static int run_lbs_forward(smalfit_engine* e, hipStream_t st, int M, const float* betas, int betas_stride,
                            int nb, const float* logscale, int ls_stride, const float* trans,
@@ -560,9 +565,11 @@
   const bool prior = ex && ex->prior_prec;
   if (prior) {
     h.prior_prec = ex->prior_prec; h.prior_mean = ex->prior_mean; h.prior_D = ex->prior_D; h.prior_use_ls = ex->prior_use_ls;
-    h.prior_w = ex->prior_w; h.prior_loss = e->loss_betas; h.prior_gb = e->gb_prior; h.prior_gls = e->gls_prior;
-  }
-  lbs_head_kernel<<<M + h.nshape + (prior ? 1 : 0), 256, 0, st>>>(m, h);
+    h.prior_w = ex->prior_w; h.prior_loss = e->loss_betas;
+    h.prior_gb = e->gb_prior + ex->prior_slot * kPriorSlotB; h.prior_gls = e->gls_prior + ex->prior_slot * kPriorSlotLs;
+  }
+  if (ex && ex->pending) lbs_head_step_kernel<<<M + h.nshape + (prior ? 1 : 0), 256, 0, st>>>(m, h, *ex->pending);
+  else lbs_head_kernel<<<M + h.nshape + (prior ? 1 : 0), 256, 0, st>>>(m, h);
   LAUNCH_OK("lbs_head_kernel");
   const int vs_stride = betas_stride ? 3 * m.Vp : 0;
   if (M > 4 && (m.Vp / 64) * ((M + 15) / 16) >= 256)
@@ -640,9 +647,15 @@
 
 }
 
-extern "C" {
-
-int smalfit_fit_eval(smalfit_engine* e, void* stream, const smalfit_fit_args* a) {
+namespace smalfit {
+struct EvalFold {
+  const PendingStep* pending = nullptr;
+  int prior_slot = 0;
+  bool assemble = true;
+  AssembleArgs* args_out = nullptr;
+};
+
+static int fit_eval_impl(smalfit_engine* e, void* stream, const smalfit_fit_args* a, const EvalFold& fold) {
   if (!e || !a) return fail("smalfit_fit_eval: null argument");
   if (a->struct_size != (unsigned)sizeof(smalfit_fit_args))
     return fail("smalfit_fit_eval: smalfit_fit_args.struct_size does not match this library (built against another smalfit.h?)");
@@ -678,6 +691,7 @@
     Section sec(e, st, SMALFIT_SEC_LBS_FWD);
     HeadExtras ex;
     ex.grot = a->global_rotation; ex.jrot = a->joint_rotations; ex.gmask = gmask; ex.rmask = rmask;
+    ex.pending = fold.pending; ex.prior_slot = fold.prior_slot;
     if (shape_prior) {
       ex.prior_prec = e->shape_prec; ex.prior_mean = e->shape_mean; ex.prior_D = D; ex.prior_use_ls = prior_uses_ls ? 1 : 0;
       const int w0 = (win.offset + win.window - 1) / win.window, w1 = (win.offset + M + win.window - 1) / win.window;
@@ -730,8 +744,8 @@
   g.nblk_beta = e->nblk_beta; g.nvt = e->nvt; g.betas_shared = 1; g.ls_shared = a->logscale_mode == 1;
   g.w_sil = a->w_sil;
   g.dbeta_part = e->dbeta_part; g.dJrest = e->dJrest; g.JS = m.JS; g.dbetaJ = e->dbetaJ; g.ngrp_beta = kBetaGroups;
-  g.gb_prior = shape_prior ? e->gb_prior : nullptr;
-  g.gls_prior = prior_uses_ls ? e->gls_prior : nullptr;
+  g.gb_prior = shape_prior ? e->gb_prior + fold.prior_slot * kPriorSlotB : nullptr;
+  g.gls_prior = prior_uses_ls ? e->gls_prior + fold.prior_slot * kPriorSlotLs : nullptr;
   g.dls = e->dls; g.dtheta = e->dtheta; g.gmask = gmask; g.rmask = rmask;
   g.dtr_direct = e->dtr_direct; g.dtr_part = e->dtr_part; g.loss_part = e->loss_part;
   g.loss_betas = shape_prior ? e->loss_betas : nullptr;
@@ -743,14 +757,22 @@
   g.g_grot = a->g_global_rotation; g.g_jrot = a->g_joint_rotations; g.g_trans = a->g_trans;
   g.losses = a->losses;
   g.lpart = e->lpart; g.qpart = e->qpart; g.counter = e->asm_counter;
-  assemble_kernel<<<1 + 1 + kAsmElem + kAsmLoss, 256, 0, st>>>(g);
-  LAUNCH_OK("assemble_kernel");
+  if (fold.args_out) *fold.args_out = g;
+  if (fold.assemble) {
+    assemble_kernel<<<1 + 1 + kAsmElem + kAsmLoss, 256, 0, st>>>(g);
+    LAUNCH_OK("assemble_kernel");
+  }
   if (e->prof_on) {
     if (e->prof_iter < e->prof_cap && (e->prof_tick % e->prof_stride) == 0) e->prof_iter++;
     e->prof_tick++;
   }
   return 0;
 }
+}
+
+extern "C" {
+
+int smalfit_fit_eval(smalfit_engine* e, void* stream, const smalfit_fit_args* a) { return fit_eval_impl(e, stream, a, EvalFold{}); }
 
 int smalfit_engine_profile_begin(smalfit_engine* e, int max_evals, int stride) {
   if (!e || max_evals <= 0 || stride <= 0) return fail("smalfit_engine_profile_begin: bad argument");
@@ -1102,6 +1124,40 @@
 }
 
 namespace smalfit {
+struct FoldPlan {
+  bool train[5];
+  int off[5];
+};
+static bool plan_fold(const smalfit_fit_args* a, const smalfit_adam_args* o, const AdamSegments& sg, FoldPlan& plan) {
+  const int M = a->num_frames;
+  if (M <= 0 || !a->betas || !a->global_rotation || !a->joint_rotations || !a->trans) return false;
+  const float* ptr[5] = {a->betas, a->logscale_mode ? a->log_beta_scales : nullptr, a->global_rotation, a->joint_rotations, a->trans};
+  const float* gptr[5] = {a->g_betas, a->g_log_beta_scales, a->g_global_rotation, a->g_joint_rotations, a->g_trans};
+  const long long cnt[5] = {20, a->logscale_mode == 1 ? 6 : (long long)M * 6, (long long)M * 3, (long long)M * 102, (long long)M * 3};
+  long long lo[5], covered = 0;
+  for (int k = 0; k < 5; ++k) {
+    plan.train[k] = false; plan.off[k] = 0; lo[k] = 0;
+    if (!ptr[k]) continue;
+    const long long bytes = (long long)((const char*)ptr[k] - (const char*)o->param);
+    if (bytes % 4) return false;
+    lo[k] = bytes / 4;
+    bool inside = false, touches = false;
+    for (int q = 0; q < sg.nseg; ++q) {
+      const long long b = sg.beg[q], en = b + (sg.off[q + 1] - sg.off[q]);
+      if (b <= lo[k] && lo[k] + cnt[k] <= en) inside = true;
+      else if (lo[k] < en && b < lo[k] + cnt[k]) touches = true;
+    }
+    if (touches) return false;
+    if (!inside) continue;
+    if (gptr[k] != o->grad + lo[k]) return false;
+    for (int j = 0; j < k; ++j)
+      if (plan.train[j] && lo[j] < lo[k] + cnt[k] && lo[k] < lo[j] + cnt[j]) return false;
+    plan.train[k] = true; plan.off[k] = (int)lo[k];
+    covered += cnt[k];
+  }
+  return covered > 0 && covered == sg.off[sg.nseg];
+}
+
 static int launch_adam_graph_node(smalfit_engine* e, hipStream_t st, const AdamSegments& sg, const smalfit_adam_args* o) {
   const int total = sg.off[sg.nseg];
   if (total == 0) return 0;
@@ -1148,6 +1204,47 @@
     for (int it = 0; it < iterations; ++it) HIP_OK(hipGraphLaunch(e->graph_exec, st));
     return 0;
   }
+  FoldPlan plan;
+  if (iterations >= 2 && !e->prof_on && plan_fold(a, o, sg, plan)) {
+    const bool ls_shared = a->logscale_mode == 1, shared_trained = plan.train[0] || (plan.train[1] && ls_shared);
+    PendingStep ps;
+    for (int it = 0; it < iterations; ++it) {
+      const bool last = it == iterations - 1;
+      EvalFold fold;
+      AssembleArgs g;
+      fold.pending = it ? &ps : nullptr; fold.prior_slot = it & 1; fold.assemble = last; fold.args_out = &g;
+      if (fit_eval_impl(e, stream, a, fold)) return 1;
+      if (last) break;
+      std::memset(&ps, 0, sizeof(ps));
+      ps.g = g;
+      const int t = o->step + it + 1;
+      adam_bias_terms(o->lr, o->beta1, o->beta2, t, ps.step_size, ps.bc2_sqrt);
+      ps.b1 = o->beta1; ps.b2 = o->beta2; ps.eps = o->eps; ps.fresh = t == 1 ? 1 : 0;
+      PendingTensor* pt[5] = {&ps.betas, &ps.ls, &ps.grot, &ps.jrot, &ps.trans};
+      const float* tensor[5] = {a->betas, a->logscale_mode ? a->log_beta_scales : nullptr, a->global_rotation, a->joint_rotations, a->trans};
+      for (int k = 0; k < 5; ++k) {
+        PendingTensor& T = *pt[k];
+        if (!plan.train[k]) { T.p_in = T.m_in = T.v_in = tensor[k]; continue; }
+        const int off = plan.off[k];
+        T.train = 1;
+        T.p_in = T.p = o->param + off; T.m_in = T.m = o->exp_avg + off; T.v_in = T.v = o->exp_avg_sq + off; T.g = o->grad + off;
+        if (k == 0 || (k == 1 && ls_shared)) {
+          const int at = k == 0 ? 0 : 20;
+          float* dst = e->shstate + ((it + 1) & 1) * 96 + at;
+          const float* src = e->shstate + (it & 1) * 96 + at;
+          if (it) { T.p_in = src; T.m_in = src + 32; T.v_in = src + 64; }
+          if (!(it && it + 2 == iterations)) { T.p = dst; T.m = dst + 32; T.v = dst + 64; }
+        }
+      }
+    }
+    if (shared_trained && iterations == 2) {
+      shared_state_restore_kernel<<<1, 64, 0, st>>>(e->shstate + ((iterations - 1) & 1) * 96, o->param, o->exp_avg, o->exp_avg_sq,
+                                                   plan.train[0] ? 20 : 0, plan.off[0], (plan.train[1] && ls_shared) ? 6 : 0, plan.off[1]);
+      LAUNCH_OK("shared_state_restore_kernel");
+    }
+    const int t = o->step + iterations;
+    return launch_adam_segments(st, sg, o, t, t == 1);
+  }
   for (int it = 0; it < iterations; ++it) {
     const int t = o->step + it + 1;
     if (smalfit_fit_eval(e, stream, a)) return 1;
diff --git a/smalify_amd/csrc/smalfit_math.h b/smalify_amd/csrc/smalfit_math.h
--- a/smalify_amd/csrc/smalfit_math.h
+++ b/smalify_amd/csrc/smalfit_math.h
@@ -340,12 +340,13 @@
 
 SMALFIT_HD void adam_update(float g, float m0, float v0, float b1, float b2, float eps, float step_size, float bc2_sqrt,
                             float& m, float& v, float& p) {
-  const float mi = b1 * m0 + (1.0f - b1) * g;
-  const float vi = b2 * v0 + (1.0f - b2) * g * g;
+#pragma clang fp contract(off)
+  const float mi = fmaf(1.0f - b1, g, b1 * m0);
+  const float vi = fmaf((1.0f - b2) * g, g, b2 * v0);
   m = mi;
   v = vi;
   const float denom = sqrtf(vi) / bc2_sqrt + eps;
-  p = p - step_size * (mi / denom);
-}
-
-}
+  p = fmaf(-step_size, mi / denom, p);
+}
+
+}
```

After: 2958 (median of 6 runs). +2.0%, better.
